# mcgillmrl/prob_mbrl

Measured on AMD Instinct MI355X. Metric: particle_rollouts_per_sec, higher is better.
Workload: dtype f32 via split fp16 (fwd, 2 pieces) / bf16 (adjoint, 2 pieces) MFMA, fp32 accumulate

## Files before the change

include/pmbrl.h:

```cpp
#ifndef PMBRL_H
#define PMBRL_H

#include <stddef.h>
#include <stdint.h>

#ifdef __cplusplus
extern "C" {
#endif

#define PMBRL_MAX_LAYERS 8
#define PMBRL_MAX_ANGLE 8
#define PMBRL_MAX_TIP 8
#define PMBRL_MAX_DIM 64

#define PMBRL_FLAG_MM_STATES 1
#define PMBRL_FLAG_MM_REWARDS 2
#define PMBRL_FLAG_INFER_NS 4
#define PMBRL_FLAG_FORCE_GENERIC 16
#define PMBRL_FLAG_NO_SHAPED 32
#define PMBRL_FLAG_POL_MASKS_PER_STEP 64
#define PMBRL_FLAG_DYN_MASKS_PER_STEP 128
#define PMBRL_FLAG_GMM_EXACT_NOISE_GRAD 256
#define PMBRL_MAX_COMP 8
#define PMBRL_FLAG_ZMM_PER_STEP 8
// ... 18 lines not shown

typedef struct pmbrl_reward {
  int32_t kind;
  int32_t expand;
  int32_t n_angle;
  int32_t angle_dims[PMBRL_MAX_ANGLE];
  int32_t k;
  float C[PMBRL_MAX_TIP * PMBRL_MAX_DIM];
  float tip_target[PMBRL_MAX_TIP];
  float norm;
  float w;
  float Q[PMBRL_MAX_TIP * PMBRL_MAX_TIP];
  float R[PMBRL_MAX_DIM * PMBRL_MAX_DIM];
} pmbrl_reward;

typedef struct pmbrl_config {
  int32_t B, D, U, H;
  int32_t B_global, row_offset;
  int32_t flags;
  int32_t mm_groups;
  float max_log_std_pol;
  float max_log_std_dyn;
  pmbrl_mlp pol;
  pmbrl_mlp dyn;
  pmbrl_reward reward;
  int32_t rows_per_wg_hint;
  int32_t precision;
  int32_t n_pol_angle;
  int32_t pol_angle_dims[PMBRL_MAX_ANGLE];
  int32_t n_dyn_angle;
  int32_t dyn_angle_dims[PMBRL_MAX_ANGLE];
  int32_t dyn_components;
  int32_t mm_span_rows, mm_span_offset;
  int32_t mm_span_ranks, mm_span_rank;
  int32_t pol_act, dyn_act;
} pmbrl_config;


typedef struct pmbrl_plan pmbrl_plan;

enum {
  PMBRL_INFO_ROWS_PER_WG = 0,
  PMBRL_INFO_N_WG = 1,
  PMBRL_INFO_ROW_TILES = 2,
  PMBRL_INFO_LDS_BYTES = 3,
  PMBRL_INFO_N_POL_PARAMS = 4,
  PMBRL_INFO_N_DYN_PARAMS = 5,
  PMBRL_INFO_DW_SPLITS = 6,
  PMBRL_INFO_MM_MODE = 7,
  PMBRL_INFO_LD = 8,
  PMBRL_INFO_DW_BLOCKS = 9,
  PMBRL_INFO_FAST = 10,
  PMBRL_INFO_STAGES = 11,
  PMBRL_INFO_MM_GRID = 12,
  PMBRL_INFO_PRECISION = 13,
  PMBRL_INFO_DW_PIPE = 14,
  PMBRL_INFO_MM_PARTS = 15,
  PMBRL_INFO_REG = 16,
  PMBRL_INFO_REPLAY = 17,
  PMBRL_INFO_INPLACE = 18,
  PMBRL_INFO_REG_FWD_CALLS = 19,
  PMBRL_INFO_REG_BWD_CALLS = 20,
  PMBRL_INFO_TAIL_CALLS = 21,
  PMBRL_INFO_COUNT = 22
};

const char* pmbrl_last_error(void);
int pmbrl_version(void);
const char* pmbrl_build_id(void);

typedef struct pmbrl_graph pmbrl_graph;
int pmbrl_graph_capture_begin(void* stream);
int pmbrl_graph_capture_end(void* stream, pmbrl_graph** graph_out);
int pmbrl_graph_launch(pmbrl_graph* graph, void* stream);
int pmbrl_graph_num_nodes(pmbrl_graph* graph, int64_t* n_out);
void pmbrl_graph_destroy(pmbrl_graph* graph);

int pmbrl_plan_create(const pmbrl_config* cfg, int device, pmbrl_plan** out);
void pmbrl_plan_destroy(pmbrl_plan* plan);
size_t pmbrl_plan_workspace_bytes(const pmbrl_plan* plan);
int pmbrl_plan_info(const pmbrl_plan* plan, int32_t* info );
#define PMBRL_SWEEP_REG 4
int pmbrl_plan_sweep_kernel(const pmbrl_plan* plan, int variant, int adjoint, const char** name);

int pmbrl_pack_mask(void* stream, const float* mask_d, int32_t B, int32_t h,
                    int32_t src_ld, uint16_t* bits_d);

int pmbrl_draw_masks(void* stream, int32_t kind, uint64_t seed, uint64_t offset, const float* param_d,
                     int32_t param_len, float temp, int32_t rows, int32_t h, const float* u_d, const float* v_d,
                     uint16_t* bits_d, int32_t aux_row0, int32_t aux_rows, float* u_out_d, float* hard_out_d,
                     float* probs_out_d);

typedef struct pmbrl_inputs {
  const float* x0_d;
  const float* pol_params_d;
  const float* dyn_params_d;
  const float* mx_d;
  const float* iSx_d;
  const float* my_d;
  const float* Sy_d;
  const float* pol_scale_d;
  const float* pol_bias_d;
  const uint16_t* pol_mask_bits_d[PMBRL_MAX_LAYERS];
  const uint16_t* dyn_mask_bits_d[PMBRL_MAX_LAYERS];
  const float* z_pol_d;
  const float* z_dyn_d;
  int64_t z_pol_step_stride;
  int64_t z_dyn_step_stride;
  const float* z_mm_d;
  const float* z_rr_d;
  const float* z_pi_d;
  const float* u_cat_d;
} pmbrl_inputs;

int pmbrl_rollout_fwd(pmbrl_plan* plan, void* stream, void* workspace_d,
                      const pmbrl_inputs* in, float* states_d, float* actions_d,
                      float* rewards_d, int32_t* status_d);

int pmbrl_rollout_bwd(pmbrl_plan* plan, void* stream, void* workspace_d,
                      const pmbrl_inputs* in, const float* states_d,
                      const float* actions_d, const float* rewards_d,
                      const float* grad_rewards_d, const float* grad_states_d,
                      const float* grad_actions_d, float* grad_pol_flat_d,
                      float* grad_x0_d, float* action_grad_norms_d, int32_t* status_d);

int pmbrl_weighted_sum(void* stream, const float* a_d, const float* w_d,
                       int64_t n, float* out_d);
int pmbrl_weighted_sum_steps(void* stream, const float* a_d, const float* w_d,
                             int64_t n_per_step, int32_t n_steps, const int32_t* status_d,
                             float* out_d);

int pmbrl_clip_adam(void* stream, float* params_d, float* grads_d,
                    float* exp_avg_d, float* exp_avg_sq_d, int64_t n,
                    int64_t step, double lr, double beta1, double beta2, double eps,
                    double max_norm, float* norm_out_d);

int pmbrl_clip_adam_guarded(void* stream, float* params_d, float* grads_d,
                            float* exp_avg_d, float* exp_avg_sq_d, int64_t n,
                            int64_t* step_d, double lr, double beta1, double beta2,
                            double eps, double max_norm, float* norm_out_d,
                            const int32_t* status_d, int32_t expect);

typedef struct pmbrl_adam {
  float* params_d;
  float* exp_avg_d;
  float* exp_avg_sq_d;
  int64_t* step_d;
  double lr, beta1, beta2, eps, max_norm;
  float* norm_out_d;
  int32_t expect_steps;
  float* loss_out_d;
} pmbrl_adam;
int pmbrl_plan_set_loss(pmbrl_plan* plan, const float* loss_weights_d, float* loss_out_d);
int pmbrl_rollout_bwd_adam(pmbrl_plan* plan, void* stream, void* workspace_d, const pmbrl_inputs* in,
                           const float* states_d, const float* actions_d, const float* rewards_d,
                           const float* grad_rewards_d, const float* grad_states_d, const float* grad_actions_d,
                           float* grad_pol_flat_d, float* grad_x0_d, float* action_grad_norms_d, int32_t* status_d,
                           const pmbrl_adam* opt);

#define PMBRL_COMM_ID_BYTES 128
typedef struct pmbrl_comm pmbrl_comm;
int pmbrl_comm_unique_id(void* id_out );
int pmbrl_comm_init(const void* id , int32_t rank, int32_t nranks,
                    int32_t device, pmbrl_comm** out);
int pmbrl_allreduce_sum(pmbrl_comm* comm, void* stream, float* buf_d, int64_t n);
int pmbrl_comm_count(pmbrl_comm* comm, int32_t* nranks_out);
// ... 114 lines not shown
```

prob_mbrl_amd/_lib.py:

```python
import ctypes as C
import os

_HERE = os.path.dirname(os.path.abspath(__file__))
LIB_PATH = os.environ.get('PMBRL_LIB_PATH', os.path.join(_HERE, 'csrc', 'libpmbrl_hip.so'))

MAX_LAYERS = 8
MAX_ANGLE = 8
MAX_TIP = 8
MAX_DIM = 64
FLAG_MM_STATES, FLAG_MM_REWARDS, FLAG_INFER_NS, FLAG_ZMM_PER_STEP = 1, 2, 4, 8
FLAG_FORCE_GENERIC = 16
FLAG_NO_SHAPED = 32
FLAG_POL_MASKS_PER_STEP, FLAG_DYN_MASKS_PER_STEP = 64, 128
FLAG_GMM_EXACT_NOISE_GRAD = 256
MAX_COMP = 8
REWARD_EXP, REWARD_NEG, REWARD_LEARNED = 0, 1, 2
PREC_F32, PREC_SPLIT, PREC_SPLIT_F16 = 0, 1, 2
ACT_RELU, ACT_TANH, ACT_SILU = 0, 1, 2
DROP_BY_TEMPERATURE, DROP_BERNOULLI = 0, 1
(INFO_ROWS_PER_WG, INFO_N_WG, INFO_ROW_TILES, INFO_LDS_BYTES, INFO_N_POL_PARAMS, INFO_N_DYN_PARAMS, INFO_DW_SPLITS,
 INFO_MM_MODE, INFO_LD, INFO_DW_BLOCKS, INFO_FAST, INFO_STAGES, INFO_MM_GRID, INFO_PRECISION, INFO_DW_PIPE, INFO_MM_PARTS,
 INFO_REG, INFO_REPLAY, INFO_INPLACE, INFO_REG_FWD_CALLS, INFO_REG_BWD_CALLS, INFO_TAIL_CALLS, INFO_COUNT) = range(23)
SWEEP_VARIANTS = ('lean', 'ext', 'mm', 'mmg', 'reg')
TIMER_COUNT = 8
TIMER_NAMES = ['pack', 'fwd', 'bwd', 'dw', 'dw_reduce', 'reward']


class MLP(C.Structure):
    _fields_ = [('n_layers', C.c_int32),
                ('dims', C.c_int32 * (MAX_LAYERS + 1)),
                ('keep', C.c_float * MAX_LAYERS)]


class MlpCall(C.Structure):
    _fields_ = [('B', C.c_int32), ('net', MLP), ('max_log_std', C.c_float), ('act', C.c_int32)]


class BnnConfig(C.Structure):
    _fields_ = [('M', C.c_int32), ('N', C.c_int32), ('net', MLP), ('max_log_std', C.c_float),
                ('temperature', C.c_float * MAX_LAYERS), ('reg_scale', C.c_float * MAX_LAYERS),
                ('drop_reg', C.c_float * MAX_LAYERS), ('reg_weight', C.c_float), ('loss_kind', C.c_int32),
                ('n_components', C.c_int32), ('act', C.c_int32),
                ('drop_kind', C.c_int32 * MAX_LAYERS), ('bern_keep', C.c_float * MAX_LAYERS)]


class Reward(C.Structure):
    _fields_ = [('kind', C.c_int32), ('expand', C.c_int32),
                ('n_angle', C.c_int32), ('angle_dims', C.c_int32 * MAX_ANGLE),
                ('k', C.c_int32), ('C', C.c_float * (MAX_TIP * MAX_DIM)),
                ('tip_target', C.c_float * MAX_TIP), ('norm', C.c_float),
                ('w', C.c_float), ('Q', C.c_float * (MAX_TIP * MAX_TIP)),
                ('R', C.c_float * (MAX_DIM * MAX_DIM))]


class Config(C.Structure):
    _fields_ = [('B', C.c_int32), ('D', C.c_int32), ('U', C.c_int32),
                ('H', C.c_int32), ('B_global', C.c_int32),
                ('row_offset', C.c_int32), ('flags', C.c_int32),
                ('mm_groups', C.c_int32), ('max_log_std_pol', C.c_float),
                ('max_log_std_dyn', C.c_float), ('pol', MLP), ('dyn', MLP),
                ('reward', Reward), ('rows_per_wg_hint', C.c_int32), ('precision', C.c_int32),
                ('n_pol_angle', C.c_int32), ('pol_angle_dims', C.c_int32 * MAX_ANGLE),
                ('n_dyn_angle', C.c_int32), ('dyn_angle_dims', C.c_int32 * MAX_ANGLE),
                ('dyn_components', C.c_int32),
                ('mm_span_rows', C.c_int32), ('mm_span_offset', C.c_int32),
                ('mm_span_ranks', C.c_int32), ('mm_span_rank', C.c_int32),
                ('pol_act', C.c_int32), ('dyn_act', C.c_int32)]


COLLECTIVE_FN = C.CFUNCTYPE(C.c_int, C.c_void_p, C.c_void_p, C.c_void_p, C.c_int64)


class Inputs(C.Structure):
    _fields_ = [('x0', C.c_void_p), ('pol_params', C.c_void_p),
                ('dyn_params', C.c_void_p), ('mx', C.c_void_p),
                ('iSx', C.c_void_p), ('my', C.c_void_p), ('Sy', C.c_void_p),
                ('pol_scale', C.c_void_p), ('pol_bias', C.c_void_p),
                ('pol_mask_bits', C.c_void_p * MAX_LAYERS),
                ('dyn_mask_bits', C.c_void_p * MAX_LAYERS),
                ('z_pol', C.c_void_p), ('z_dyn', C.c_void_p),
                ('z_pol_step_stride', C.c_int64), ('z_dyn_step_stride', C.c_int64),
                ('z_mm', C.c_void_p), ('z_rr', C.c_void_p),
                ('z_pi', C.c_void_p), ('u_cat', C.c_void_p)]


EXPORTS = [
    'pmbrl_last_error', 'pmbrl_version', 'pmbrl_build_id', 'pmbrl_plan_create',
    'pmbrl_graph_capture_begin', 'pmbrl_graph_capture_end', 'pmbrl_graph_launch', 'pmbrl_graph_num_nodes', 'pmbrl_graph_destroy',
    'pmbrl_plan_destroy', 'pmbrl_plan_workspace_bytes', 'pmbrl_plan_info', 'pmbrl_plan_sweep_kernel',
    'pmbrl_pack_mask', 'pmbrl_draw_masks', 'pmbrl_rollout_fwd', 'pmbrl_rollout_bwd', 'pmbrl_rollout_bwd_adam',
    'pmbrl_plan_set_loss',
    'pmbrl_weighted_sum', 'pmbrl_weighted_sum_steps', 'pmbrl_clip_adam', 'pmbrl_clip_adam_guarded', 'pmbrl_debug_linear',
    'pmbrl_plan_set_timing', 'pmbrl_plan_read_timing', 'pmbrl_plan_set_prof', 'pmbrl_plan_set_replay', 'pmbrl_plan_replay_count',
    'pmbrl_mlp_workspace_bytes', 'pmbrl_mlp_forward', 'pmbrl_mlp_grad_input',
    'pmbrl_bnn_plan_create', 'pmbrl_bnn_plan_destroy', 'pmbrl_bnn_plan_workspace_bytes',
    'pmbrl_bnn_plan_n_params', 'pmbrl_bnn_plan_set_unit_keep', 'pmbrl_bnn_loss_grad', 'pmbrl_bnn_loss_grad_ex', 'pmbrl_bnn_train_steps',
    'pmbrl_comm_unique_id', 'pmbrl_comm_init', 'pmbrl_allreduce_sum', 'pmbrl_comm_count', 'pmbrl_comm_destroy',
    'pmbrl_plan_set_comm', 'pmbrl_plan_set_collective',
    'pmbrl_p2p_create', 'pmbrl_p2p_handle', 'pmbrl_p2p_open', 'pmbrl_p2p_allreduce_f32', 'pmbrl_p2p_allreduce_f64',
    'pmbrl_plan_set_p2p', 'pmbrl_p2p_error', 'pmbrl_p2p_destroy', 'pmbrl_plan_set_grad_comm',
]

class Adam(C.Structure):
    _fields_ = [('params_d', C.c_void_p), ('exp_avg_d', C.c_void_p), ('exp_avg_sq_d', C.c_void_p),
                ('step_d', C.c_void_p), ('lr', C.c_double), ('beta1', C.c_double), ('beta2', C.c_double),
                ('eps', C.c_double), ('max_norm', C.c_double), ('norm_out_d', C.c_void_p), ('expect_steps', C.c_int32),
                ('loss_out_d', C.c_void_p)]


_lib = None


def load():
    global _lib
    if _lib is not None:
        return _lib
    if not os.path.exists(LIB_PATH):
        raise RuntimeError(
            'prob_mbrl_amd: %s is missing -- build the HIP extension first '
            '(python -c "import __graft_entry__ as g; g.build()"). There is no '
            'CPU fallback for the rollout hot path.' % LIB_PATH)
    lib = C.CDLL(LIB_PATH)
    vp, i32, i64, f32 = C.c_void_p, C.c_int32, C.c_int64, C.c_float
    lib.pmbrl_last_error.restype = C.c_char_p
    lib.pmbrl_last_error.argtypes = []
    lib.pmbrl_version.restype = C.c_int
    lib.pmbrl_build_id.restype = C.c_char_p
    lib.pmbrl_build_id.argtypes = []
    lib.pmbrl_graph_capture_begin.restype = C.c_int
    lib.pmbrl_graph_capture_begin.argtypes = [vp]
    lib.pmbrl_graph_capture_end.restype = C.c_int
    lib.pmbrl_graph_capture_end.argtypes = [vp, C.POINTER(vp)]
    lib.pmbrl_graph_launch.restype = C.c_int
    lib.pmbrl_graph_launch.argtypes = [vp, vp]
    lib.pmbrl_graph_num_nodes.restype = C.c_int
    lib.pmbrl_graph_num_nodes.argtypes = [vp, C.POINTER(C.c_int64)]
    lib.pmbrl_graph_destroy.restype = None
    lib.pmbrl_graph_destroy.argtypes = [vp]
    lib.pmbrl_plan_create.restype = C.c_int
    lib.pmbrl_plan_create.argtypes = [C.POINTER(Config), C.c_int, C.POINTER(vp)]
    lib.pmbrl_plan_destroy.restype = None
    lib.pmbrl_plan_destroy.argtypes = [vp]
    lib.pmbrl_plan_workspace_bytes.restype = C.c_size_t
    lib.pmbrl_plan_workspace_bytes.argtypes = [vp]
    lib.pmbrl_plan_info.restype = C.c_int
    lib.pmbrl_plan_info.argtypes = [vp, C.POINTER(i32)]
    lib.pmbrl_plan_sweep_kernel.restype = C.c_int
    lib.pmbrl_plan_sweep_kernel.argtypes = [vp, C.c_int, C.c_int, C.POINTER(C.c_char_p)]
    lib.pmbrl_pack_mask.restype = C.c_int
    lib.pmbrl_pack_mask.argtypes = [vp, vp, i32, i32, i32, vp]
    lib.pmbrl_rollout_fwd.restype = C.c_int
    lib.pmbrl_rollout_fwd.argtypes = [vp, vp, vp, C.POINTER(Inputs), vp, vp, vp, vp]
    lib.pmbrl_rollout_bwd.restype = C.c_int
    lib.pmbrl_rollout_bwd.argtypes = [vp, vp, vp, C.POINTER(Inputs), vp, vp, vp,
                                      vp, vp, vp, vp, vp, vp, vp]
    lib.pmbrl_weighted_sum.restype = C.c_int
    lib.pmbrl_weighted_sum.argtypes = [vp, vp, vp, i64, vp]
    lib.pmbrl_weighted_sum_steps.restype = C.c_int
    lib.pmbrl_weighted_sum_steps.argtypes = [vp, vp, vp, i64, i32, vp, vp]
    lib.pmbrl_clip_adam.restype = C.c_int
    f64 = C.c_double
    lib.pmbrl_clip_adam.argtypes = [vp, vp, vp, vp, vp, i64, i64, f64, f64, f64,
                                    f64, f64, vp]
    lib.pmbrl_clip_adam_guarded.restype = C.c_int
    lib.pmbrl_clip_adam_guarded.argtypes = [vp, vp, vp, vp, vp, i64, vp, f64, f64, f64, f64, f64, vp, vp, i32]
    lib.pmbrl_mlp_workspace_bytes.restype = C.c_size_t
    lib.pmbrl_mlp_workspace_bytes.argtypes = [C.POINTER(MlpCall)]
    lib.pmbrl_mlp_forward.restype = C.c_int
    lib.pmbrl_mlp_forward.argtypes = [vp, C.POINTER(MlpCall), vp, vp, vp, C.POINTER(vp)] + [vp] * 10
    lib.pmbrl_mlp_grad_input.restype = C.c_int
    lib.pmbrl_mlp_grad_input.argtypes = [vp, C.POINTER(MlpCall), vp, vp, vp, C.POINTER(vp)] + [vp] * 11
    lib.pmbrl_bnn_plan_create.restype = C.c_int
    lib.pmbrl_bnn_plan_create.argtypes = [C.POINTER(BnnConfig), C.c_int, C.POINTER(vp)]
    lib.pmbrl_bnn_plan_destroy.restype = None
    lib.pmbrl_bnn_plan_destroy.argtypes = [vp]
    lib.pmbrl_bnn_plan_workspace_bytes.restype = C.c_size_t
    lib.pmbrl_bnn_plan_workspace_bytes.argtypes = [vp]
    lib.pmbrl_bnn_plan_n_params.restype = C.c_int64
    lib.pmbrl_bnn_plan_n_params.argtypes = [vp]
    lib.pmbrl_bnn_plan_set_unit_keep.restype = C.c_int
    lib.pmbrl_bnn_plan_set_unit_keep.argtypes = [vp, i32, C.POINTER(f32), i32]
    lib.pmbrl_bnn_loss_grad.restype = C.c_int
    lib.pmbrl_bnn_loss_grad.argtypes = [vp] * 11
    lib.pmbrl_bnn_loss_grad_ex.restype = C.c_int
    lib.pmbrl_bnn_loss_grad_ex.argtypes = [vp] * 13 + [i32]
    lib.pmbrl_bnn_train_steps.restype = C.c_int
    lib.pmbrl_bnn_train_steps.argtypes = ([vp] * 6 + [i32] + [vp] * 4 + [C.c_double] * 4 + [C.c_uint64] * 2 + [vp] * 4)
    lib.pmbrl_debug_linear.restype = C.c_int
    lib.pmbrl_debug_linear.argtypes = [vp, vp, vp, vp, i32, i32, i32, i32, vp, vp]
    lib.pmbrl_plan_set_replay.restype = C.c_int
    lib.pmbrl_plan_set_replay.argtypes = [vp, C.c_int]
    lib.pmbrl_plan_replay_count.restype = C.c_int
    lib.pmbrl_plan_replay_count.argtypes = [vp, C.POINTER(C.c_int64)]
    lib.pmbrl_plan_set_timing.restype = C.c_int
    lib.pmbrl_plan_set_timing.argtypes = [vp, C.c_int]
    lib.pmbrl_plan_read_timing.restype = C.c_int
    lib.pmbrl_plan_read_timing.argtypes = [vp, C.POINTER(C.c_float)]
    lib.pmbrl_plan_set_prof.restype = C.c_int
    lib.pmbrl_plan_set_prof.argtypes = [vp, vp, vp]
    lib.pmbrl_comm_unique_id.restype = C.c_int
    lib.pmbrl_comm_unique_id.argtypes = [vp]
    lib.pmbrl_comm_init.restype = C.c_int
    lib.pmbrl_comm_init.argtypes = [vp, i32, i32, i32, C.POINTER(vp)]
    lib.pmbrl_allreduce_sum.restype = C.c_int
    lib.pmbrl_allreduce_sum.argtypes = [vp, vp, vp, i64]
    lib.pmbrl_plan_set_loss.restype = C.c_int
    lib.pmbrl_plan_set_loss.argtypes = [vp, vp, vp]
    lib.pmbrl_rollout_bwd_adam.restype = C.c_int
    lib.pmbrl_rollout_bwd_adam.argtypes = [vp, vp, vp, C.POINTER(Inputs)] + [vp] * 10 + [C.POINTER(Adam)]
    lib.pmbrl_draw_masks.restype = C.c_int
    lib.pmbrl_draw_masks.argtypes = [vp, i32, C.c_uint64, C.c_uint64, vp, i32, C.c_float, i32, i32, vp, vp, vp, i32, i32, vp, vp, vp]
    lib.pmbrl_comm_count.restype = C.c_int
    lib.pmbrl_comm_count.argtypes = [vp, C.POINTER(i32)]
    lib.pmbrl_comm_destroy.restype = None
    lib.pmbrl_comm_destroy.argtypes = [vp]
    lib.pmbrl_plan_set_comm.restype = C.c_int
    lib.pmbrl_plan_set_comm.argtypes = [vp, vp]
    lib.pmbrl_p2p_create.restype = C.c_int
    lib.pmbrl_p2p_create.argtypes = [i32, i32, i32, i64, C.POINTER(vp)]
    lib.pmbrl_p2p_handle.restype = C.c_int
    lib.pmbrl_p2p_handle.argtypes = [vp, vp]
    lib.pmbrl_p2p_open.restype = C.c_int
    lib.pmbrl_p2p_open.argtypes = [vp, i32, vp]
    for fn in (lib.pmbrl_p2p_allreduce_f32, lib.pmbrl_p2p_allreduce_f64):
        fn.restype = C.c_int
        fn.argtypes = [vp, vp, vp, i64]
    lib.pmbrl_plan_set_p2p.restype = C.c_int
    lib.pmbrl_plan_set_p2p.argtypes = [vp, vp]
    lib.pmbrl_p2p_error.restype = C.c_int
    lib.pmbrl_p2p_error.argtypes = [vp, C.POINTER(i32)]
    lib.pmbrl_p2p_destroy.restype = None
# ... 22 lines not shown
```

prob_mbrl_amd/csrc/pmbrl.hip:

```cpp
#include <hip/hip_runtime.h>
#include <math.h>
#include <stdio.h>
#include <string.h>

#include <algorithm>
#include <memory>
#include <string>
#include <vector>

#include "pmbrl_host.h"
#include "pmbrl_mm.h"
#include "pmbrl_rollout.h"
#include "pmbrl_mmx.h"
#include "pmbrl_mm_wide.h"
#include "pmbrl_fast.h"
#include "pmbrl_reward.h"

static thread_local std::string g_err;
int pm_fail(int code, const std::string& msg) {
  g_err = msg;
  return code;
}

extern "C" const char* pmbrl_last_error(void) { return g_err.c_str(); }
// ... 265 lines not shown
  const int gi = blockIdx.x, r0 = gi * A.M;
  if (A.nvalid && t >= *A.nvalid) return;
  const int zrow0 = pm_zrow0(t, A.row_off + r0, A.flags);
  const float* zmm = pm_zbase(A.zmm, A.D, t, A.Bg, A.flags);
  const float* s = A.xt + ((size_t)t * A.B + r0) * A.D;
  float* g = A.gx_carry + (size_t)r0 * A.D;
  const double* fac = fac_all + ((size_t)t * gridDim.x + gi) * pm_mmw_fac_doubles(A.D);
  pm_mmw_bwd(s, A.M, A.D, zmm, zrow0, A.Bg, g, g, fac, mmscr);
}

static size_t align_up(size_t x, size_t a) { return (x + a - 1) / a * a; }

static int net_plan(const pmbrl_mlp& m, int act, NetPlan& n, int in_expect, int out_expect,
                    const char* name) {
  if (m.n_layers < 1 || m.n_layers > PM_MAXL)
    return fail(-2, std::string(name) + ": n_layers out of range");
  n.nl = m.n_layers;
  size_t off = 0;
  for (int i = 0; i <= n.nl; ++i) {
    if (m.dims[i] < 1 || m.dims[i] > 4096) return fail(-2, std::string(name) + ": bad layer width");
    n.dim[i] = m.dims[i];
    n.nt[i] = (m.dims[i] + 15) / 16;
  }
  if (n.dim[0] != in_expect || n.dim[n.nl] != out_expect)
    return fail(-2, std::string(name) + ": input/output width does not match D/U");
  if (act != PMBRL_ACT_RELU && act != PMBRL_ACT_TANH && act != PMBRL_ACT_SILU)
    return fail(-2, std::string(name) + ": unknown activation (PMBRL_ACT_RELU, PMBRL_ACT_TANH, PMBRL_ACT_SILU are offered)");
  n.act = act;
  for (int l = 0; l < n.nl; ++l) {
    n.keep[l] = (l < n.nl - 1) ? m.keep[l] : 1.f;
    if (l < n.nl - 1 && !(n.keep[l] > 0.f)) return fail(-2, std::string(name) + ": keep must be > 0");
    n.w_off[l] = off;
    off += (size_t)n.dim[l + 1] * n.dim[l];
    n.b_off[l] = off;
    off += n.dim[l + 1];
  }
  n.n_params = off;
  return 0;
}

#define PM_INST(RT, CA, CB, VAR, D, U, LD, NL, NT, TREE) \
  {reinterpret_cast<const void*>(&pm_rollout_fwd<RT>), reinterpret_cast<const void*>(&pm_rollout_bwd<RT>)},
static const PmInst general_f32_fns[] = {PM_GENERAL_F32_INSTANCES};
#undef PM_INST
static_assert(sizeof(general_f32_fns) / sizeof(general_f32_fns[0]) == pm_general_f32_n, "one kernel pair per key");

static constexpr size_t PM_LDS_CAP = 160 * 1024;

static bool env_set(const char* name) { return getenv(name) != nullptr; }
static bool env_on(const char* name) {
  const char* e = getenv(name);
  return !(e && atoi(e) == 0);
}
static PlanSwitches read_switches() {
  PlanSwitches s{};
  s.mm_perstep = env_set("PMBRL_MM_PERSTEP");
  s.mm_mode2 = env_set("PMBRL_MM_MODE2");
  s.mm_no_batch = env_set("PMBRL_MM_NO_BATCH");
  s.dw_no_wide = env_set("PMBRL_DW_NO_WIDE");
  s.reg_debug = env_set("PMBRL_REG_DEBUG");
  s.lds_tiles = env_on("PMBRL_LDS_TILES");
  s.mm_xch = env_on("PMBRL_MM_XCH");
  s.mm_tree = env_on("PMBRL_MM_TREE");
  s.reg = env_on("PMBRL_REG");
  s.reg_mm = env_on("PMBRL_REG_MM");
  s.reg_tree = env_on("PMBRL_REG_TREE");
  s.reg_bwd = env_on("PMBRL_REG_BWD");
  s.fuse_loss = env_on("PMBRL_FUSE_LOSS");
  s.ztab_merge = env_on("PMBRL_ZTAB_MERGE");
  s.wide = env_on("PMBRL_WIDE");
  if (const char* e = getenv("PMBRL_MM_PARTS")) { s.mm_parts_set = true; s.mm_parts = atoi(e); }
  s.replay = 1;
  if (const char* e = getenv("PMBRL_REPLAY")) s.replay = std::max(0, std::min(2, atoi(e)));
  if (const char* e = getenv("PMBRL_DW_PIPE")) {
    s.dw_pipe_off = !strcmp(e, "off");
    s.dw_pipe_ranges = e[0] >= '0' && e[0] <= '9';
    for (const char* q = e; s.dw_pipe_ranges && *q;) {
      const int v = atoi(q);
      if (v > 0) s.dw_pipe.push_back(v);
      while (*q && *q != ',') ++q;
      if (*q == ',') ++q;
    }
  }
  return s;
}

static int plan_nets(pmbrl_plan* p) {
  const pmbrl_config& c = p->cfg;
  if (c.n_pol_angle < 0 || c.n_pol_angle > PMBRL_MAX_ANGLE || c.n_dyn_angle < 0 || c.n_dyn_angle > PMBRL_MAX_ANGLE)
    return fail(-2, "n_pol_angle / n_dyn_angle out of range");
  if (c.dyn_components < 0 || c.dyn_components > PMBRL_MAX_COMP)
    return fail(-2, "dyn_components out of range (<= PMBRL_MAX_COMP)");
  const bool gmm = c.dyn_components > 1;
  if (c.reward.kind != PMBRL_REWARD_EXP && c.reward.kind != PMBRL_REWARD_NEG && c.reward.kind != PMBRL_REWARD_LEARNED)
    return fail(-2, "unknown reward kind");
  p->learned = c.reward.kind == PMBRL_REWARD_LEARNED;
  if (p->learned && gmm)
    return fail(-2, "learned reward head: not offered with the mixture head (dyn_components > 1)");
  if (p->learned && c.mm_span_rows > 0)
    return fail(-2, "learned reward head: not offered with moment-matching groups spread over ranks (mm_span_rows > 0)");
  if (p->learned && c.D + 1 > PMBRL_MAX_DIM) return fail(-2, "learned reward head: D + 1 exceeds PMBRL_MAX_DIM");
  int rc = net_plan(c.pol, c.pol_act, p->pol, c.D + c.n_pol_angle, 2 * c.U, "policy");
  if (rc == 0)
    rc = net_plan(c.dyn, c.dyn_act, p->dyn, c.D + c.U + c.n_dyn_angle,
                  gmm ? (2 * c.D + 1) * c.dyn_components + 1 : 2 * (c.D + p->learned), "dynamics");
  p->act = rc == 0 && (p->pol.act != PMBRL_ACT_RELU || p->dyn.act != PMBRL_ACT_RELU);
  return rc;
}

struct LayoutCalc {
  const pmbrl_plan* p;
  int maxnt;
  bool gsplit;
  bool want_split;
  bool rt4_split;
  int ld_generic() const { return gsplit ? (maxnt * 16 + 31) / 32 * 32 + 16 : maxnt * 16 + 8; }
  int prec(int RT) const {
    if (!p->fast) return gsplit ? (int)PMBRL_PREC_SPLIT_F16 : 0;
    return (want_split && (RT <= 2 || rt4_split)) ? (int)p->cfg.precision : 0;
  }
  long stream_work(int m, int kdiv) const {
    long w = 0;
    for (const NetPlan* n : {&p->pol, &p->dyn})
      for (int l = 1; l <= n->nl - 2; ++l) {
        const int ki = (n->nt[l] + kdiv - 1) / kdiv, ko = (n->nt[l + 1] + kdiv - 1) / kdiv;
        w += (long)n->nt[l + 1] * ((ki + m - 1) / m * m) + (long)n->nt[l] * ((ko + m - 1) / m * m);
      }
    return w;
  }
  StagePair stages(int RT) const {
    const int pr = prec(RT);
    return pm_inst_best_stages(pm_fast_keys(pr), pr && !p->fast ? std::min(RT, 2) : RT,
                               [&](int m) { return stream_work(m, pr ? 2 : 1); });
  }
  int ldb(int RT) const {
    if (!prec(RT)) return 0;
    if (!p->fast) return ld_generic();
    const StagePair sp = stages(RT);
    const int m = sp.ca + sp.cb;
    return ((maxnt + 1) / 2 + m - 1) / m * m * 32 + 16;
  }
  int ld(int RT) const {
    if (!p->fast) return ld_generic();
    if (prec(RT))
      return ((prec(RT) == PMBRL_PREC_SPLIT_F16 ? 2 : 3) * ldb(RT) / 2 + 3) / 4 * 4;
    const StagePair sp = stages(RT);
    const int m = sp.ca + sp.cb;
    return (maxnt + m - 1) / m * m * 16 + 8;
  }
  size_t lds(int RT, int mmd, int parts = 1, bool inplace = false) const {
    const pmbrl_config& c = p->cfg;
    if (p->fast) {
      const int mw = parts > 1 ? 1 : (mmd && p->M <= 16 * RT) ? std::min(PF_NW, std::max(1, 16 * RT / p->M)) : PF_NW;
      return pm_fast_lds_floats(16 * RT, ld(RT), c.D, c.U, RT, p->pol.nt, p->pol.nl, p->dyn.nt, p->dyn.nl, mmd, prec(RT),
                                mw, parts > 1 ? (parts > 8 ? 16 : p->M) : 0, parts > 1 ? c.H : 0) * sizeof(float);
    }
    return pm_lds_floats(16 * RT, ld(RT), c.D, c.U, RT, mmd, inplace) * sizeof(float);
  }
};

static int plan_groups(pmbrl_plan* p, LayoutCalc& L, int cus) {
  const pmbrl_config& c = p->cfg;
  const PlanSwitches& sw = p->sw;
  p->G = c.mm_groups > 0 ? c.mm_groups : 1;
  if (c.B % p->G) return fail(-2, "B must be divisible by mm_groups");
  p->M = c.B / p->G;
// ... 319 lines not shown
      for (int l = 0; l < p->pol.nl; ++l) {
        if (p->dw_narrow[l]) { wide[l] = true; continue; }
        p->dw_pre_mask |= 1u << l;
        for (int m0 = 0; m0 < 512; m0 += PM_DWP_TM)
          for (int n0 = 0; n0 < 512; n0 += PM_DWP_TN) pre.push_back(DwUnit{(int16_t)l, (int16_t)m0, (int16_t)n0, 0});
      }
      units = pre;
    } else {
      for (int l = 0; l < PM_MAXL; ++l) p->dw_narrow[l] = 0;
    }
  }
  p->n_dw_units = (int)units.size();
  if (p->n_dw_units) {
    HIPCHK(hipMalloc(&p->dw_units_d, units.size() * sizeof(DwUnit)));
    HIPCHK(hipMemcpy(p->dw_units_d, units.data(), units.size() * sizeof(DwUnit), hipMemcpyHostToDevice));
  }
  if (int rc = pm_dw_set_attr(p)) return rc;
  p->n_dw_blocks = build_dw_blocks(p->pol.nl, p->pol.nt, blocks, p->dw_wave_first, p->dw_split ? PM_DW_TN_S : PM_DW_TN, wide);
  p->dw_n_chunks = c.H * p->nwg * p->RT;
  int nsplit = std::min(256, p->dw_n_chunks);
  p->dw_chunks_per_split = (p->dw_n_chunks + nsplit - 1) / nsplit;
  if (p->dw_split) p->dw_chunks_per_split = (p->dw_chunks_per_split + 1) & ~1;
  p->dw_nsplit = (p->dw_n_chunks + p->dw_chunks_per_split - 1) / p->dw_chunks_per_split;
  HIPCHK(hipMalloc(&p->dw_blocks_d, std::max<size_t>(1, blocks.size()) * sizeof(DwBlock)));
  if (!blocks.empty())
    HIPCHK(hipMemcpy(p->dw_blocks_d, blocks.data(), blocks.size() * sizeof(DwBlock), hipMemcpyHostToDevice));
  DwArgs& W = p->dw_args;
  memset(&W, 0, sizeof(W));
  W.nl = p->pol.nl;
  W.nsplit = p->dw_nsplit;
  W.n_chunks = p->dw_n_chunks;
  W.chunks_per_split = p->dw_chunks_per_split;
  W.RT = p->RT;
  W.Rw = 16 * p->RT;
  W.n_params = (int)p->pol.n_params;
  W.part_stride = (W.n_params + 3) / 4 * 4;
  for (int i = 0; i <= p->pol.nl; ++i) { W.dim[i] = p->pol.dim[i]; W.nt[i] = p->pol.nt[i]; }
  for (int l = 0; l < p->pol.nl; ++l) { W.w_off[l] = (int)p->pol.w_off[l]; W.b_off[l] = (int)p->pol.b_off[l]; }
  W.blocks = p->dw_blocks_d;
  for (int w = 0; w <= PM_DW_NW; ++w) W.wave_first[w] = p->dw_wave_first[w];
  W.chunks_per_step = p->nwg * p->RT;
  W.split_prec = p->dw_split;
  return 0;
}

static int plan_dw_pipe(pmbrl_plan* p, int cus) {
  const pmbrl_config& c = p->cfg;
  const PlanSwitches& sw = p->sw;
  p->pipe_K = 1;
  const bool no_pipe_pre = p->dw_pre_mask != 0;
  const int n_free = cus >= 64 && cus % 8 == 0 ? 8 * (cus / 8 - (p->nwg + 7) / 8) : 0;
  const bool single = sweep_form(p) == SweepForm::Whole && p->mm_parts <= 1;
  const bool long_steps = (long long)p->RT * (long long)(p->pol.n_params + p->dyn.n_params) >= 256 * 1024 && c.H >= 16;
  if (!single || no_pipe_pre || n_free < cus / 8 || c.H < 2 || sw.dw_pipe_off || !(long_steps || sw.dw_pipe_ranges))
    return 0;
  std::vector<int> cnt;
  if (sw.dw_pipe_ranges) {
    cnt = sw.dw_pipe;
    int sum = 0;
    for (int v : cnt) sum += v;
    if (sum != c.H || (int)cnt.size() > PM_PIPE_MAX) cnt.clear();
  }
  if (cnt.empty() && long_steps) {
    const int a3 = std::max(2, c.H / 10), a2 = a3 + std::max(2, c.H / 5), a1 = a2 + std::max(2, (3 * c.H) / 10);
    cnt = {c.H - a1, a1 - a2, a2 - a3, a3};
  }
  int K = 0, lo = c.H;
  for (size_t k = 0; k < cnt.size() && lo > 0; ++k) {
    lo = k + 1 == cnt.size() ? 0 : std::max(0, lo - cnt[k]);
    if (p->dw_split && ((p->nwg * p->RT) & 1) && (lo & 1)) lo -= 1;
    if (K > 0 && lo >= p->pipe_lo[K - 1]) continue;
    p->pipe_lo[K++] = lo;
  }
  if (K >= 2 && p->pipe_lo[K - 1] == 0) {
    p->pipe_K = K;
    p->pipe_grid = n_free;
    p->pipe_rows = std::max(n_free, cus);
    HIPCHK(hipStreamCreateWithFlags(&p->pipe_stream, hipStreamNonBlocking));
    for (int k = 0; k < p->pipe_K; ++k) HIPCHK(hipEventCreateWithFlags(&p->pipe_ev[k], hipEventDisableTiming));
  }
  return 0;
}

static int plan_workspace(pmbrl_plan* p) {
  const pmbrl_config& c = p->cfg;
  p->reg = pm_reg_plan_ok(p) ? 1 : 0;
  p->reg_mm = pm_reg_mm_width(p);
  size_t off = 0;
  auto take = [&](size_t bytes) {
    const size_t o = off;
    off = align_up(off + bytes, 256);
    return o;
  };
  for (NetPlan* n : {&p->pol, &p->dyn}) {
    for (int l = 0; l < n->nl; ++l) {
      const size_t fr = (size_t)(n->nt[l + 1] + 15) * (n->nt[l] + 15) * 256 * sizeof(float);
      n->wf[l] = take(fr);
      n->wb[l] = take(fr);
      n->bias[l] = take((size_t)n->nt[l + 1] * 16 * sizeof(float));
      if (l < n->nl - 1)
        n->abits[l] = take((size_t)c.H * c.B * n->nt[l + 1] * (p->act ? 16 * sizeof(float) : 4) + 256);
    }
  }
  const bool gmm = c.dyn_components > 1;
  const size_t Rw = 16 * p->RT;
  for (int l = 0; l < p->pol.nl; ++l) {
    p->off_actT[l] = take((size_t)c.H * p->nwg * p->pol.nt[l] * 16 * Rw * sizeof(float));
    p->off_gT[l] = take((size_t)c.H * p->nwg * p->pol.nt[l + 1] * 16 * Rw * sizeof(float));
  }
  p->off_Tp = take((size_t)c.H * c.B * c.U * sizeof(float));
  p->off_Td = take((size_t)c.H * c.B * c.D * sizeof(float));
  p->off_gmm_c = take(gmm ? (size_t)c.H * c.B * (c.dyn_components + 1) * c.D * sizeof(float) : 0);
  p->off_gmm_k = take(gmm ? (size_t)c.H * c.B * sizeof(int) : 0);
  p->off_xt = take((size_t)c.H * c.B * c.D * sizeof(float));
  p->off_rt = take((size_t)c.H * c.B * sizeof(float));
  p->off_mmfac = take(p->mm_mode == 1 ? (size_t)c.H * (c.B / p->M) * pm_mm_fac_doubles(c.D) * sizeof(double)
                      : p->mm_wide    ? (size_t)c.H * p->G * pm_mmw_fac_doubles(c.D) * sizeof(double)
                                      : 0);
  p->off_Jx = take((size_t)c.H * c.B * c.D * sizeof(float));
  p->off_Ja = take((size_t)c.H * c.B * c.U * sizeof(float));
  p->off_gxc = take((size_t)c.B * c.D * sizeof(float));
  p->off_gxc2 = take((size_t)c.B * c.D * sizeof(float));
  p->off_gsync = take(2 * 1024 * sizeof(unsigned));
  if (p->mm_parts > 1 && p->sw.mm_xch) {
    p->xch_bytes = (size_t)(p->mm_parts > 8 ? 2 : 1) * p->nwg * PM_XCH_WG_WORDS(2) * sizeof(unsigned long long);
    p->off_xch = take(p->xch_bytes);
  }
  p->off_ztab = take((p->mm_fan || p->reg_mm) ? (size_t)c.H * p->G * 2 * c.D * sizeof(double) : 0);
  p->off_reg_linv = take(p->reg_mm ? (size_t)c.H * p->G * c.D * c.D * sizeof(double) : 0);
  p->off_grt = take((size_t)c.H * c.B * sizeof(float));
  const size_t n_s = (size_t)p->G * pm_mmx_slot_doubles(c.D), n_r = (size_t)c.H * p->G * pm_mmx_slot_doubles(1);
  p->off_mmx_buf = take(p->span ? (size_t)c.mm_span_ranks * std::max(n_s * PM_MMX_NB, n_r) * sizeof(double) : 0);
  p->off_mmx_fac = take(p->span ? (size_t)c.H * p->G * pm_mm_fac_doubles(c.D) * sizeof(double) : 0);
  p->off_mmx_rfac = take(p->span ? (size_t)c.H * p->G * pm_mm_fac_doubles(1) * sizeof(double) : 0);
  p->off_reg_pack = take(p->reg ? pm_reg_pack_bytes() : 0);
  for (int n = 0; n < 2; ++n)
    for (int l = 0; l < 2; ++l) p->off_reg_ab[n][l] = take(p->reg ? (size_t)c.H * p->nwg * 1024 : 0);
  p->off_part = take((size_t)std::max(p->dw_nsplit, p->pipe_K > 1 ? p->pipe_rows : 0) *
                     ((p->pol.n_params + 3) / 4 * 4) * sizeof(float));
  p->ws_bytes = off;
  if (p->ws_bytes >= ((size_t)1 << 32)) p->reg = p->reg_mm = 0;
  return 0;
}

static PmInstTable sweep_table(const pmbrl_plan* p) {
  if (p->fast)
    return p->prec == PMBRL_PREC_SPLIT_F16 ? pm_fast_split2_instances() : p->prec ? pm_fast_split1_instances() : pm_fast_f32_instances();
  if (p->act) return pm_general_act_instances();
  return p->prec ? pm_general_split_instances() : PmInstTable{pm_general_f32_keys, general_f32_fns, pm_general_f32_n};
}
static bool lds_tiles_row(const pmbrl_plan* p, const PmInstKey& k) {
  return p->prec == PMBRL_PREC_SPLIT_F16 && p->RT == 1 && p->CA + p->CB == 7 && k.var != PF_VAR_MMG && k.nl == 3 && k.nt > 8;
}
static int resolve_sweeps(pmbrl_plan* p) {
  const pmbrl_config& c = p->cfg;
  const PmInstTable T = sweep_table(p);
  auto take = [&](int slot, const PmInstKey& k) {
    const int i = pm_inst_find(T, k);
    if (i >= 0) { p->sweep[slot] = T.fn[i]; p->sweep_key[slot] = k; }
    return i >= 0;
  };
  if (!p->fast) {
    const int wide_form = (p->inplace == 2 && p->dw_pre_mask) ? 3 : p->inplace;
    const PmInstKey k = pm_general_key(p->RT, p->act ? (p->prec ? 2 : 0) : p->prec ? wide_form : 0);
    return take(0, k) ? 0 : fail(-3, "no general-family instance for " + pm_inst_name(k));
  }
  const bool shaped_ok = !(c.flags & PMBRL_FLAG_NO_SHAPED) && !(p->mm_parts > 1 && !p->xch_bytes);
  for (int var = 0; var < PF_VAR_COUNT; ++var) {
    const bool mm_in = p->mm_mode == 1 || p->mm_mode == 3;
    const bool needed = var == PF_VAR_MMG ? p->mm_grid != 0 : (var == PF_VAR_MM) == mm_in;
    PmInstKey k = {p->RT, p->CA, p->CB, var, c.D, c.U, p->LD, 3, hidden_tiles_3l(p), 0};
    k.tree = var == PF_VAR_MM && p->mm_mode == 1 && p->mm_parts > 8;
    if (shaped_ok && (!lds_tiles_row(p, k) || p->wlds_off > 0) && take(var, k)) continue;
    if (k.tree) return fail(-3, "no instance for a moment-matching group split over more than 8 workgroups: " + pm_inst_name(k));
    k = PmInstKey{p->RT, p->CA, p->CB, var, 0, 0, 0, 0, 0, 0};
    if (!take(var, k) && needed) return fail(-3, "no latency-optimised instance for " + pm_inst_name(k));
  }
  return 0;
}
static int plan_attrs(pmbrl_plan* p, int cus) {
  const pmbrl_config& c = p->cfg;
  if (int rc = resolve_sweeps(p)) return rc;
  const PmInstTable T = sweep_table(p);
  for (int i = 0; i < T.n; ++i) {
    const PmInstKey& k = T.key[i];
    if (p->fast ? k.rt != p->RT || k.ca != p->CA || k.cb != p->CB : T.fn[i].fwd != p->sweep[0].fwd) continue;
    HIPCHK(hipFuncSetAttribute(T.fn[i].fwd, hipFuncAttributeMaxDynamicSharedMemorySize, (int)p->lds_bytes));
    HIPCHK(hipFuncSetAttribute(T.fn[i].bwd, hipFuncAttributeMaxDynamicSharedMemorySize, (int)p->lds_bytes));
  }
  if (p->mm_wide) {
    const int smem = (int)pm_mmw_lds_bytes(p->M, c.D, true);
    if (smem > 64 * 1024 &&
        (hipFuncSetAttribute(reinterpret_cast<const void*>(&pm_mmw_fwd_kernel), hipFuncAttributeMaxDynamicSharedMemorySize,
                             smem) != hipSuccess ||
         hipFuncSetAttribute(reinterpret_cast<const void*>(&pm_mmw_bwd_kernel), hipFuncAttributeMaxDynamicSharedMemorySize,
                             smem) != hipSuccess)) {
      (void)hipGetLastError();
      return fail(-3, "hipFuncSetAttribute(wide moment-matching kernels) failed");
    }
  }
  if (p->mm_mode == 2 || p->mm_mode == 3) {
    const int smem = (int)(pm_mm_kernel_doubles(c.D) * sizeof(double));
    if (smem > (int)PM_LDS_CAP) return fail(-3, "moment-matching scratch exceeds the LDS");
    if (smem > 64 * 1024 &&
        (hipFuncSetAttribute(reinterpret_cast<const void*>(&pm_mm_fwd_kernel), hipFuncAttributeMaxDynamicSharedMemorySize,
                             smem) != hipSuccess ||
         hipFuncSetAttribute(reinterpret_cast<const void*>(&pm_mm_bwd_kernel), hipFuncAttributeMaxDynamicSharedMemorySize,
                             smem) != hipSuccess)) {
      (void)hipGetLastError();
      return fail(-3, "hipFuncSetAttribute(moment-matching kernels) failed");
    }
  }
  if (p->reg)
    if (int rc = pm_reg_resolve(p)) return rc;
  if (p->mm_grid) {
    const int i = pm_inst_find(T, {1, p->CA, p->CB, PF_VAR_MMG, 0, 0, 0, 0, 0, 0});
    int a = 0, b = 0;
    if (i < 0 || hipOccupancyMaxActiveBlocksPerMultiprocessor(&a, T.fn[i].fwd, PF_NT, p->lds_bytes) != hipSuccess ||
        hipOccupancyMaxActiveBlocksPerMultiprocessor(&b, T.fn[i].bwd, PF_NT, p->lds_bytes) != hipSuccess)
      a = b = 0;
    if (std::min(a, b) < 1 || p->nwg > cus) p->mm_grid = 0;
  }
  return 0;
}

extern "C" int pmbrl_plan_create(const pmbrl_config* cfg, int device, pmbrl_plan** out) {
  if (!cfg || !out) return fail(-1, "null argument");
  const pmbrl_config& c = *cfg;
  if (c.B < 1 || c.D < 1 || c.U < 1 || c.H < 1) return fail(-2, "B, D, U, H must be >= 1");
  if (c.D > 32 || c.U > 16) return fail(-2, "supported widths: D <= 32, U <= 16");
  if (c.reward.kind != PMBRL_REWARD_LEARNED && (c.reward.k < 1 || c.reward.k > PMBRL_MAX_TIP))
    return fail(-2, "reward.k out of range");
  std::unique_ptr<pmbrl_plan, void (*)(pmbrl_plan*)> p(new pmbrl_plan(), pmbrl_plan_destroy);
  p->cfg = c;
  if (p->cfg.B_global <= 0) p->cfg.B_global = c.B;
  p->device = device;
  p->sw = read_switches();
  p->replay = p->sw.replay;
  if (int rc = plan_nets(p.get())) return rc;
  int cus = 0;
  (void)hipDeviceGetAttribute(&cus, hipDeviceAttributeMultiprocessorCount, device);
  if (int rc = plan_layout(p.get(), cus)) return rc;
  if (int rc = plan_reward(p.get())) return rc;
  if (int rc = plan_angles(p.get())) return rc;
  if (int rc = plan_dw(p.get())) return rc;
  if (int rc = plan_dw_pipe(p.get(), cus)) return rc;
  if (int rc = plan_workspace(p.get())) return rc;
  if (int rc = plan_attrs(p.get(), cus)) return rc;
  *out = p.release();
  return 0;
}

static bool per_step_launches(const pmbrl_plan* p) {
  const SweepForm f = sweep_form(p);
  return (f == SweepForm::StepExternal || f == SweepForm::StepInSweep) && p->cfg.H >= 4;
}
static bool replay_wanted(const pmbrl_plan* p) {
  if (p->replay == 0 || p->span || p->coll) return false;
  return p->replay >= 2 || per_step_launches(p);
}
struct ReplayKey {
  unsigned long long h = 1469598103934665603ull;
  std::vector<unsigned char> bytes;
  void add(const void* q, size_t n) {
    const unsigned char* b = static_cast<const unsigned char*>(q);
    for (size_t i = 0; i < n; ++i) { h ^= b[i]; h *= 1099511628211ull; }
    bytes.insert(bytes.end(), b, b + n);
  }
  template <class T> void val(const T& v) { add(&v, sizeof(T)); }
};
static bool pm_stream_recording(hipStream_t s) {
  hipStreamCaptureStatus cs = hipStreamCaptureStatusNone;
  if (!s) return false;
  if (hipStreamIsCapturing(s, &cs) != hipSuccess) { (void)hipGetLastError(); return false; }
  return cs != hipStreamCaptureStatusNone;
}
template <class Body>
static int replay_call(pmbrl_plan* p, int slot, const ReplayKey& K, hipStream_t s, Body body) {
  const unsigned long long key = K.h;
  pmbrl_plan::ReplaySlot& R = p->rp[slot];
  hipStreamCaptureStatus cs = hipStreamCaptureStatusNone;
  const bool usable = replay_wanted(p) && !p->timing && !p->prof_fwd && !p->prof_bwd && !R.dead &&
                      (!s || (hipStreamIsCapturing(s, &cs) == hipSuccess && cs == hipStreamCaptureStatusNone));
  if (!usable) {
    if (R.exec || R.seen) replay_drop(p, slot);
    return body(s);
  }
  const bool same = R.key == key && R.bytes == K.bytes;
  if (R.exec && same) {
    HIPCHK(hipGraphLaunch(R.exec, s));
    ++R.launches;
    if (slot == 0) { p->old_pack_stale = R.aux & 1; p->abits_packed = (R.aux >> 1) & 1; }
    else p->dw_g1_rebuilt = (R.aux >> 2) & 1;
    return 0;
  }
  if (!same || R.seen == 0) {
    replay_drop(p, slot);
    R.key = key;
    R.bytes = K.bytes;
    R.seen = 1;
    return body(s);
  }
  hipGraph_t g = nullptr;
  if (!p->cap_stream && hipStreamCreateWithFlags(&p->cap_stream, hipStreamNonBlocking) != hipSuccess) p->cap_stream = nullptr;
  if (!p->cap_stream || hipStreamBeginCapture(p->cap_stream, hipStreamCaptureModeThreadLocal) != hipSuccess) {
    (void)hipGetLastError();
    R.dead = 1;
    return body(s);
  }
  const int rc = body(p->cap_stream);
  const hipError_t e = hipStreamEndCapture(p->cap_stream, &g);
  if (rc != 0 || e != hipSuccess || !g) {
    (void)hipGetLastError();
    if (g) (void)hipGraphDestroy(g);
    R.dead = 1;
    replay_drop(p, slot);
    return rc != 0 ? rc : body(s);
  }
  hipGraphExec_t ex = nullptr;
  const hipError_t ei = hipGraphInstantiate(&ex, g, nullptr, nullptr, 0);
  (void)hipGraphDestroy(g);
  if (ei != hipSuccess || !ex) {
    (void)hipGetLastError();
    R.dead = 1;
    replay_drop(p, slot);
    return body(s);
  }
  R.exec = ex;
  R.aux = (p->old_pack_stale & 1) | ((p->abits_packed & 1) << 1) | ((p->dw_g1_rebuilt & 1) << 2);
  HIPCHK(hipGraphLaunch(R.exec, s));
  ++R.launches;
  return 0;
}

extern "C" int pmbrl_plan_set_replay(pmbrl_plan* p, int on) {
  if (!p || on < 0 || on > 2) return fail(-1, "bad argument");
  p->replay = on;
  for (int k = 0; k < 2; ++k) { replay_drop(p, k); p->rp[k].dead = 0; }
  return 0;
}

extern "C" int pmbrl_plan_replay_count(const pmbrl_plan* p, int64_t* n_out) {
  if (!p || !n_out) return fail(-1, "null argument");
  for (int k = 0; k < 2; ++k) n_out[k] = p->rp[k].launches;
  return 0;
}

extern "C" int pmbrl_plan_set_prof(pmbrl_plan* p, long long* fwd_d, long long* bwd_d) {
  if (!p) return fail(-1, "null argument");
  p->prof_fwd = fwd_d;
  p->prof_bwd = bwd_d;
  return 0;
}

extern "C" int pmbrl_plan_set_timing(pmbrl_plan* p, int on) {
  if (!p) return fail(-1, "null argument");
  if (on && !p->ev[0][0]) {
    for (int i = 0; i < PMBRL_TIMER_COUNT; ++i)
      for (int j = 0; j < 2; ++j) HIPCHK(hipEventCreate(&p->ev[i][j]));
  }
  p->timing = on ? 1 : 0;
  for (int i = 0; i < PMBRL_TIMER_COUNT; ++i) p->ev_set[i] = false;
  return 0;
}

extern "C" int pmbrl_plan_read_timing(pmbrl_plan* p, float* ms) {
  if (!p || !ms) return fail(-1, "null argument");
  for (int i = 0; i < PMBRL_TIMER_COUNT; ++i) {
    ms[i] = -1.f;
    if (p->timing && p->ev_set[i]) {
      HIPCHK(hipEventSynchronize(p->ev[i][1]));
      HIPCHK(hipEventElapsedTime(&ms[i], p->ev[i][0], p->ev[i][1]));
    }
  }
  return 0;
}

extern "C" void pmbrl_plan_destroy(pmbrl_plan* p) {
  if (!p) return;
  if (p->ev[0][0])
    for (int i = 0; i < PMBRL_TIMER_COUNT; ++i)
      for (int j = 0; j < 2; ++j) (void)hipEventDestroy(p->ev[i][j]);
  for (int k = 0; k < 2; ++k) replay_drop(p, k);
  if (p->cap_stream) (void)hipStreamDestroy(p->cap_stream);
  if (p->rew_d) (void)hipFree(p->rew_d);
  if (p->wflag_d) (void)hipFree(p->wflag_d);
  if (p->ang_d) (void)hipFree(p->ang_d);
  if (p->dw_blocks_d) (void)hipFree(p->dw_blocks_d);
  if (p->dw_units_d) (void)hipFree(p->dw_units_d);
  if (p->tail_buf_d) (void)hipFree(p->tail_buf_d);
  if (p->pipe_stream) {
    (void)hipStreamDestroy(p->pipe_stream);
    for (int k = 0; k < p->pipe_K; ++k) (void)hipEventDestroy(p->pipe_ev[k]);
  }
  delete p;
}

extern "C" int pmbrl_plan_sweep_kernel(const pmbrl_plan* p, int variant, int adjoint, const char** name) {
  if (!p || !name) return fail(-1, "null argument");
  PmInst k{};
  if (variant == PMBRL_SWEEP_REG) k = p->reg ? p->reg_k[0] : k;
  else if (!p->fast) k = p->sweep[0];
  else if (variant >= 0 && variant < PF_VAR_COUNT) k = p->sweep[variant];
  else return fail(-1, "variant out of range");
  const void* f = adjoint ? k.bwd : k.fwd;
  *name = f ? hipKernelNameRefByPtr(f, nullptr) : "";
  if (!*name) *name = "";
  return 0;
}

extern "C" size_t pmbrl_plan_workspace_bytes(const pmbrl_plan* p) { return p ? p->ws_bytes : 0; }

extern "C" int pmbrl_plan_info(const pmbrl_plan* p, int32_t* info) {
  if (!p || !info) return fail(-1, "null argument");
  memset(info, 0, sizeof(int32_t) * PMBRL_INFO_COUNT);
  info[PMBRL_INFO_ROWS_PER_WG] = p->rows_per_wg;
  info[PMBRL_INFO_N_WG] = p->nwg;
  info[PMBRL_INFO_ROW_TILES] = p->RT;
  info[PMBRL_INFO_LDS_BYTES] = (int32_t)p->lds_bytes;
  info[PMBRL_INFO_N_POL_PARAMS] = (int32_t)p->pol.n_params;
  info[PMBRL_INFO_N_DYN_PARAMS] = (int32_t)p->dyn.n_params;
  info[PMBRL_INFO_DW_SPLITS] = p->dw_nsplit;
  info[PMBRL_INFO_MM_MODE] = p->mm_mode;
  info[PMBRL_INFO_LD] = p->LD;
  info[PMBRL_INFO_DW_BLOCKS] = p->n_dw_blocks;
  info[PMBRL_INFO_FAST] = p->fast;
  info[PMBRL_INFO_STAGES] = p->CA * 16 + p->CB;
  info[PMBRL_INFO_MM_GRID] = p->mm_grid;
  info[PMBRL_INFO_PRECISION] = p->prec;
  info[PMBRL_INFO_DW_PIPE] = p->pipe_K;
  info[PMBRL_INFO_MM_PARTS] = p->mm_parts;
  info[PMBRL_INFO_REG] = p->reg;
  info[PMBRL_INFO_REPLAY] = replay_wanted(p) ? 1 : 0;
  info[PMBRL_INFO_INPLACE] = p->inplace;
  info[PMBRL_INFO_REG_FWD_CALLS] = p->reg_calls[0];
  info[PMBRL_INFO_REG_BWD_CALLS] = p->reg_calls[1];
  info[PMBRL_INFO_TAIL_CALLS] = p->tail_calls;
  return 0;
}


static void fill_net(const NetPlan& n, char* ws, const uint16_t* const* masks, NetDev& d) {
  d.nl = n.nl;
  for (int i = 0; i <= n.nl; ++i) {
    d.dim[i] = n.dim[i];
    d.nt[i] = n.nt[i];
  }
  for (int l = 0; l < n.nl; ++l) {
    d.keep[l] = n.keep[l];
    d.inv_keep[l] = 1.f / n.keep[l];
    d.wf[l] = reinterpret_cast<const float*>(ws + n.wf[l]);
    d.wb[l] = reinterpret_cast<const float*>(ws + n.wb[l]);
    d.bias[l] = reinterpret_cast<const float*>(ws + n.bias[l]);
    d.mask[l] = (l < n.nl - 1) ? masks[l] : nullptr;
    d.abits[l] = (l < n.nl - 1) ? reinterpret_cast<uint16_t*>(ws + n.abits[l]) : nullptr;
  }
}

static int fill_args(const pmbrl_plan* p, void* workspace, const pmbrl_inputs* in, RolloutArgs& A) {
  const pmbrl_config& c = p->cfg;
  char* ws = static_cast<char*>(workspace);
  memset(&A, 0, sizeof(A));
  A.B = c.B; A.D = c.D; A.U = c.U; A.H = c.H;
  A.Bg = c.B_global; A.row_off = c.row_offset; A.flags = c.flags;
  A.flags |= (p->pol.act << PM_ACT_POL_SHIFT) | (p->dyn.act << PM_ACT_DYN_SHIFT);
  A.G = p->G; A.M = p->M; A.mm_mode = p->mm_mode;
  A.t0 = 0; A.t1 = c.H;
  A.rows_per_wg = p->rows_per_wg; A.nwg = p->nwg; A.Rw = 16 * p->RT; A.LD = p->LD; A.LDB = p->LDB;
  A.mls_pol = c.max_log_std_pol; A.mls_dyn = c.max_log_std_dyn;
  for (int l = 0; l < p->pol.nl - 1; ++l)
    if (!in->pol_mask_bits_d[l]) return fail(-1, "missing policy mask bits");
  for (int l = 0; l < p->dyn.nl - 1; ++l)
    if (!in->dyn_mask_bits_d[l]) return fail(-1, "missing dynamics mask bits");
  fill_net(p->pol, ws, in->pol_mask_bits_d, A.pol);
  fill_net(p->dyn, ws, in->dyn_mask_bits_d, A.dyn);
  A.rew = p->rew_d;
  A.ang = p->ang_d;
  A.x0 = in->x0_d; A.mx = in->mx_d; A.iSx = in->iSx_d; A.my = in->my_d; A.Sy = in->Sy_d;
  A.pscale = in->pol_scale_d; A.pbias = in->pol_bias_d;
  A.zpol = in->z_pol_d; A.zdyn = in->z_dyn_d; A.zmm = in->z_mm_d; A.zrr = in->z_rr_d;
  A.zpol_ss = in->z_pol_step_stride; A.zdyn_ss = in->z_dyn_step_stride;
  if (!A.x0 || !A.mx || !A.iSx || !A.my || !A.Sy || !A.pscale || !A.pbias || !A.zpol || !A.zdyn)
    return fail(-1, "null input pointer");
  if ((c.flags & PMBRL_FLAG_MM_STATES) && !A.zmm) return fail(-1, "mm_states needs z_mm");
  if ((c.flags & PMBRL_FLAG_MM_REWARDS) && !A.zrr) return fail(-1, "mm_rewards needs z_rr");
  for (int l = 0; l < p->pol.nl; ++l) {
    A.actT[l] = reinterpret_cast<float*>(ws + p->off_actT[l]);
    A.gT[l] = reinterpret_cast<float*>(ws + p->off_gT[l]);
  }
  A.Tp = reinterpret_cast<float*>(ws + p->off_Tp);
  A.Td = reinterpret_cast<float*>(ws + p->off_Td);
  A.gmm_n = p->cfg.dyn_components > 1 ? p->cfg.dyn_components : 0;
  A.zpi = A.ucat = A.zdyn_grad = nullptr;
  A.gmm_k = nullptr;
// ... 381 lines not shown
  if (!p || (loss_weights_d && !loss_out_d)) return fail(-1, "bad argument");
  p->loss_w = loss_weights_d;
  p->loss_out = loss_weights_d ? loss_out_d : nullptr;
  return 0;
}

static int tail_allreduce(pmbrl_plan* p, hipStream_t s, float* buf_d, int64_t n) {
  if (p->grad_p2p) return pmbrl_p2p_allreduce_f32(p->grad_p2p, s, buf_d, n);
  return pmbrl_allreduce_sum(p->grad_comm, s, buf_d, n);
}

struct BwdCall {
  hipStream_t stream;
  void* workspace;
  const pmbrl_inputs* in;
  const float *states, *actions, *rewards;
  const float *grad_rewards, *grad_states, *grad_actions;
  float *grad_pol_flat, *grad_x0, *action_grad_norms;
  int32_t* status;
  const pmbrl_adam* opt;
};
static bool bwd_tail(const pmbrl_plan* p, const BwdCall& C) { return C.opt && (p->grad_comm || p->grad_p2p); }
static int expect_steps(const pmbrl_plan* p, const pmbrl_adam* opt) {
  return opt ? (opt->expect_steps > 0 ? opt->expect_steps : p->cfg.H) : 0;
}

static int check_bwd(const pmbrl_plan* p, const BwdCall& C, bool reg_bwd) {
  if (bwd_tail(p, C) && p->span && p->cfg.mm_span_ranks > 1)
    return fail(-3, "pmbrl_rollout_bwd_adam with a gradient transport: moment-matching groups spread over ranks are not offered");
  if (p->reg && p->old_pack_stale && !reg_bwd && (!C.in->pol_params_d || !C.in->dyn_params_d)) return fail(-1, "null parameter pointer");
  if (int rc = check_collective(p)) return rc;
  const SweepForm form = sweep_form(p);
  if (C.grad_states && (form == SweepForm::Barrier || form == SweepForm::StepInSweep))
    return fail(-3, "grad_states with moment-matching groups spanning workgroups: not offered");
  if (C.grad_states && form == SweepForm::StepExternal) return fail(-3, "grad_states with external moment matching: not offered");
  return 0;
}

static int bwd_args(const pmbrl_plan* p, const BwdCall& C, RolloutArgs& A) {
  if (int rc = fill_args(p, C.workspace, C.in, A)) return rc;
  A.states = const_cast<float*>(C.states);
  A.actions = const_cast<float*>(C.actions);
  A.rewards = const_cast<float*>(C.rewards);
  A.grad_rewards = C.grad_rewards;
  A.grad_states = C.grad_states;
  A.grad_actions = C.grad_actions;
  A.grad_x0 = C.grad_x0;
  A.agn = C.action_grad_norms;
  A.prof = p->prof_bwd;
  A.nvalid = C.status;
  A.status = C.status ? C.status + 1 : nullptr;
  if (!p->fast) A.ext_reward = 1;
  return 0;
}

static int bwd_agree_horizon(pmbrl_plan* p, const BwdCall& C) {
  hipStream_t s = C.stream;
  float* hvec = p->tail_buf_d + ((size_t)p->pol.n_params + 2 + 3) / 4 * 4;
  pm_tail_hvec_launch(s, hvec, p->tail_world, p->tail_rank, C.status, p->cfg.H);
  if (int rc = tail_allreduce(p, s, hvec, p->tail_world)) return rc;
  pm_tail_hmin_launch(s, hvec, p->tail_world, C.status, p->cfg.H);
  return 0;
}

static void bwd_convert_family(pmbrl_plan* p, const BwdCall& C) {
  char* ws = static_cast<char*>(C.workspace);
  if (p->old_pack_stale) launch_pack_all(p, ws, C.in, C.stream, nullptr);
  if (p->abits_packed) pm_reg_unpack_abits(p, ws, C.stream);
}

static int bwd_reward_adjoint(pmbrl_plan* p, const BwdCall& C, RolloutArgs& A, float* grt) {
  if (p->cfg.flags & PMBRL_FLAG_MM_REWARDS) {
    if (p->span) {
      if (int rc = mmx_bwd(p, static_cast<char*>(C.workspace), A, true, 0, grt, C.stream)) return rc;
    } else {
      hipLaunchKernelGGL(pm_mm_rewards_bwd_kernel, dim3(p->cfg.H * p->G), dim3(64), pm_mmr_lds_bytes(p->M, 3), C.stream, A, grt);
    }
    A.grad_rewards = grt;
  }
  if (!p->fast) A.flags &= ~PMBRL_FLAG_MM_REWARDS;
  return 0;
}

static DwArgs dw_call_args(const pmbrl_plan* p, const BwdCall& C, const RolloutArgs& A) {
  DwArgs W = p->dw_args;
  for (int l = 0; l < p->pol.nl; ++l) { W.actT[l] = A.actT[l]; W.gT[l] = A.gT[l]; }
  W.part = reinterpret_cast<float*>(static_cast<char*>(C.workspace) + p->off_part);
  W.nvalid = C.status;
  if (p->dw_g1_rebuilt) {
    pm_reg_dw_rebuild_args(p, static_cast<char*>(C.workspace), W);
    W.rc_inv_keep = A.pol.inv_keep[1];
  }
  return W;
}
static int bwd_sweep_barrier(pmbrl_plan* p, const BwdCall& C, RolloutArgs A) {
  hipStream_t s = C.stream;
  HIPCHK(hipMemsetAsync(A.gx_carry, 0, (size_t)p->cfg.B * p->cfg.D * sizeof(float), s));
  A.gx_from_carry = 1;
  A.gsync += 1024;
  HIPCHK(hipMemsetAsync(A.gsync, 0, 1024 * sizeof(unsigned), s));
  A.gx_carry_out = reinterpret_cast<float*>(static_cast<char*>(C.workspace) + p->off_gxc2);
  A.t0 = 0; A.t1 = p->cfg.H;
  launch_bwd_rt(p, A, s);
  return 0;
}
static int bwd_sweep_steps(pmbrl_plan* p, const BwdCall& C, RolloutArgs A) {
  hipStream_t s = C.stream;
  float* cbuf[2] = {A.gx_carry, reinterpret_cast<float*>(static_cast<char*>(C.workspace) + p->off_gxc2)};
  HIPCHK(hipMemsetAsync(cbuf[0], 0, (size_t)p->cfg.B * p->cfg.D * sizeof(float), s));
  A.gx_from_carry = 1;
  for (int t = p->cfg.H - 1, k = 0; t >= 0; --t, k ^= 1) {
    A.gx_carry = cbuf[k];
    A.gx_carry_out = cbuf[k ^ 1];
    A.t0 = t; A.t1 = t + 1;
    launch_bwd_rt(p, A, s);
  }
  return 0;
}
static int bwd_sweep_whole(pmbrl_plan* p, const BwdCall& C, RolloutArgs A, const DwArgs& W, bool reg_bwd, int K, const int* lo) {
  hipStream_t s = C.stream;
  char* ws = static_cast<char*>(C.workspace);
  if (p->mm_parts > 1) {
    A.gsync += 1024;
    A.gx_carry_out = reinterpret_cast<float*>(ws + p->off_gxc2);
    if (int rc = xch_prepare(p, A, reg_bwd, s)) return rc;
  }
  for (int k = 0; k < K; ++k) {
    A.t0 = lo[k];
    A.t1 = k ? lo[k - 1] : p->cfg.H;
    A.gx_from_carry = k > 0;
    if (reg_bwd) pm_reg_launch(p, ws, A, C.in->pol_params_d, C.in->dyn_params_d, s, false);
    else launch_bwd_rt(p, A, s);
    if (k + 1 < K) {
      HIPCHK(hipEventRecord(p->pipe_ev[k], s));
      HIPCHK(hipStreamWaitEvent(p->pipe_stream, p->pipe_ev[k], 0));
      pm_dw_launch_range(p, W, k, p->pipe_stream);
    }
  }
  return 0;
}
static int bwd_sweep_external(pmbrl_plan* p, const BwdCall& C, RolloutArgs A, float* grt) {
  hipStream_t s = C.stream;
  char* ws = static_cast<char*>(C.workspace);
  const size_t smem = pm_mm_kernel_doubles(p->cfg.D) * sizeof(double);
  HIPCHK(hipMemsetAsync(A.gx_carry, 0, (size_t)p->cfg.B * p->cfg.D * sizeof(float), s));
  RolloutArgs Am = A;
  Am.flags &= ~PMBRL_FLAG_MM_REWARDS;
  A.gx_from_carry = 1;
  for (int t = p->cfg.H - 1; t >= 0; --t) {
    if (p->mm_wide) {
      hipLaunchKernelGGL(pm_mmw_bwd_kernel, dim3(p->G), dim3(PM_MMW_NT), pm_mmw_lds_bytes(p->M, p->cfg.D, true), s, Am, t,
                         reinterpret_cast<const double*>(ws + p->off_mmfac));
    } else if (!p->span) {
      hipLaunchKernelGGL(pm_mm_bwd_kernel, dim3(p->G), dim3(PM_MM_NW * 64), smem, s, Am, t, grt);
    } else if (p->cfg.flags & PMBRL_FLAG_MM_STATES) {
      if (int rc = mmx_bwd(p, ws, Am, false, t, nullptr, s)) return rc;
    }
    A.t0 = t; A.t1 = t + 1;
    launch_bwd_rt(p, A, s);
  }
  return 0;
}

static int bwd_dw(pmbrl_plan* p, const BwdCall& C, const DwArgs& W, bool piped) {
  ScopedTimer tm(p, PMBRL_TIMER_DW, C.stream);
  if (!piped) {
    pm_dw_launch(p, W, C.stream);
    return 0;
  }
  HIPCHK(hipEventRecord(p->pipe_ev[p->pipe_K - 1], p->pipe_stream));
  HIPCHK(hipStreamWaitEvent(C.stream, p->pipe_ev[p->pipe_K - 1], 0));
  pm_dw_launch_range(p, W, p->pipe_K - 1, C.stream);
  return 0;
}

static int rollout_bwd(pmbrl_plan* p, const BwdCall& C, const RolloutArgs& A0, bool reg_bwd) {
  hipStream_t s = C.stream;
  RolloutArgs A = A0;
  if (int rc = check_bwd(p, C, reg_bwd)) return rc;
  p->dw_g1_rebuilt = reg_bwd ? 1 : 0;
  const pmbrl_adam* opt = C.opt;
  const bool tail = bwd_tail(p, C);
  float* const xb = p->tail_buf_d;
  if (tail)
    if (int rc = bwd_agree_horizon(p, C)) return rc;
  if (p->reg && !reg_bwd) bwd_convert_family(p, C);
  float* grt = reinterpret_cast<float*>(static_cast<char*>(C.workspace) + p->off_grt);
  if (int rc = bwd_reward_adjoint(p, C, A, grt)) return rc;
  const DwArgs W = dw_call_args(p, C, A);
  const SweepForm form = sweep_form(p);
  const bool piped = form == SweepForm::Whole && p->pipe_K > 1 && !p->prof_bwd;
  {
    ScopedTimer tm(p, PMBRL_TIMER_BWD, s);
    static const int whole[1] = {0};
    int rc = 0;
    switch (form) {
      case SweepForm::Barrier: rc = bwd_sweep_barrier(p, C, A); break;
      case SweepForm::StepInSweep: rc = bwd_sweep_steps(p, C, A); break;
      case SweepForm::Whole: rc = bwd_sweep_whole(p, C, A, W, reg_bwd, piped ? p->pipe_K : 1, piped ? p->pipe_lo : whole); break;
      case SweepForm::StepExternal: rc = bwd_sweep_external(p, C, A, grt); break;
    }
    if (rc) return rc;
  }
  if (int rc = bwd_dw(p, C, W, piped)) return rc;
  const int n = (int)p->pol.n_params;
  const int expect = expect_steps(p, opt);
  const bool part_ok = opt && !piped && (n + 255) / 256 <= PM_NORM_MAXB;
  const bool norm_fused = part_ok && !tail;
  const bool loss_fused = part_ok && opt->loss_out_d && p->sw.fuse_loss;
  const int n_loss_part = loss_fused ? (n + 255) / 256 : 0;
  float* const red_out = tail ? xb : C.grad_pol_flat;
  {
    ScopedTimer tm(p, PMBRL_TIMER_DW_REDUCE, s);
    if (piped)
      pm_dw_reduce_launch(s, W.part, p->pipe_rows, n, W.part_stride, red_out, (const int*)nullptr, 0, 1);
    else
      pm_dw_reduce_launch(s, W.part, p->dw_nsplit, n, W.part_stride, red_out, (const int*)C.status, W.chunks_per_step,
                          W.chunks_per_split, norm_fused ? 1 : 0, (const int*)C.status, expect,
                          opt ? reinterpret_cast<long long*>(opt->step_d) : (long long*)nullptr,
                          loss_fused ? C.rewards : (const float*)nullptr, C.grad_rewards, (long long)p->cfg.H * p->cfg.B,
                          (long long)p->cfg.B);
  }
  if (opt && opt->loss_out_d && !loss_fused)
    launch_weighted_sum(s, C.rewards, C.grad_rewards, (long long)p->cfg.H * p->cfg.B, tail ? xb + n : opt->loss_out_d, C.status,
                        p->cfg.B);
  HIPCHK(hipGetLastError());
  if (!opt) return 0;
  if (tail) {
    pm_tail_pack_launch(s, xb, n, n_loss_part, opt->loss_out_d && !loss_fused ? 1 : 0, C.status, p->tail_err_d);
    if (int rc = tail_allreduce(p, s, xb, (int64_t)n + 2)) return rc;
    pm_tail_finish_launch(s, xb, C.grad_pol_flat, n, C.status, expect, reinterpret_cast<long long*>(opt->step_d), p->tail_err_d);
    HIPCHK(hipGetLastError());
  }
  return clip_adam_guarded_impl(s, opt->params_d, C.grad_pol_flat, opt->exp_avg_d, opt->exp_avg_sq_d, n, opt->step_d, opt->lr,
                                opt->beta1, opt->beta2, opt->eps, opt->max_norm, opt->norm_out_d, C.status, expect,
                                tail || norm_fused, tail || loss_fused ? opt->loss_out_d : nullptr,
                                tail ? (opt->loss_out_d ? 1 : 0) : n_loss_part);
}

static ReplayKey bwd_key(const pmbrl_plan* p, const BwdCall& C, bool reg_bwd) {
  const pmbrl_adam* opt = C.opt;
  ReplayKey K;
  K.val(C.stream); K.val(C.workspace); K.add(C.in, sizeof(*C.in));
  K.val(C.states); K.val(C.actions); K.val(C.rewards); K.val(C.grad_rewards); K.val(C.grad_states); K.val(C.grad_actions);
  K.val(C.grad_pol_flat); K.val(C.grad_x0); K.val(C.action_grad_norms); K.val(C.status);
  const int has_opt = opt ? 1 : 0;
  K.val(has_opt);
  if (opt) {
    K.val(opt->params_d); K.val(opt->exp_avg_d); K.val(opt->exp_avg_sq_d); K.val(opt->step_d);
    K.val(opt->lr); K.val(opt->beta1); K.val(opt->beta2); K.val(opt->eps); K.val(opt->max_norm);
    K.val(opt->norm_out_d); K.val(opt->expect_steps);
  }
  if (bwd_tail(p, C)) {
    K.val(p->grad_comm); K.val(p->tail_buf_d); K.val(opt->loss_out_d);
  }
  K.val(p->old_pack_stale); K.val(p->abits_packed);
  const int g1_rebuilt = reg_bwd ? 1 : 0;
  K.val(g1_rebuilt);
  return K;
}

static int rollout_bwd_replay(pmbrl_plan* p, const BwdCall& C) {
  if (!p || !C.workspace || !C.in || !C.states || !C.actions || !C.rewards || !C.grad_rewards || !C.grad_pol_flat)
    return fail(-1, "null argument");
  HIPCHK(hipSetDevice(p->device));
  RolloutArgs A;
  if (int rc = bwd_args(p, C, A)) return rc;
  const bool reg_bwd = pm_reg_can_run(p, A, false);
  const bool tail = bwd_tail(p, C);
  if (tail) ++p->tail_calls;
  if (tail && p->grad_p2p) {
    if (p->rp[1].exec || p->rp[1].seen) replay_drop(p, 1);
    return rollout_bwd(p, C, A, reg_bwd);
  }
  return replay_call(p, 1, bwd_key(p, C, reg_bwd), C.stream, [&](hipStream_t on) {
    BwdCall Con = C;
    Con.stream = on;
    return rollout_bwd(p, Con, A, reg_bwd);
  });
}

extern "C" int pmbrl_rollout_bwd(pmbrl_plan* p, void* stream, void* workspace, const pmbrl_inputs* in,
                                 const float* states_d, const float* actions_d,
                                 const float* rewards_d, const float* grad_rewards_d,
                                 const float* grad_states_d, const float* grad_actions_d,
                                 float* grad_pol_flat_d, float* grad_x0_d,
                                 float* action_grad_norms_d, int32_t* status_d) {
  return rollout_bwd_replay(p, BwdCall{(hipStream_t)stream, workspace, in, states_d, actions_d, rewards_d, grad_rewards_d,
                                       grad_states_d, grad_actions_d, grad_pol_flat_d, grad_x0_d, action_grad_norms_d,
                                       status_d, nullptr});
}

extern "C" int pmbrl_rollout_bwd_adam(pmbrl_plan* p, void* stream, void* workspace, const pmbrl_inputs* in,
                                      const float* states_d, const float* actions_d,
                                      const float* rewards_d, const float* grad_rewards_d,
                                      const float* grad_states_d, const float* grad_actions_d,
                                      float* grad_pol_flat_d, float* grad_x0_d,
                                      float* action_grad_norms_d, int32_t* status_d, const pmbrl_adam* opt) {
  if (!opt || !status_d || !opt->params_d || !opt->exp_avg_d || !opt->exp_avg_sq_d || !opt->step_d)
    return fail(-1, "null argument");
  return rollout_bwd_replay(p, BwdCall{(hipStream_t)stream, workspace, in, states_d, actions_d, rewards_d, grad_rewards_d,
                                       grad_states_d, grad_actions_d, grad_pol_flat_d, grad_x0_d, action_grad_norms_d,
                                       status_d, opt});
}

template <int RT>
__global__ __launch_bounds__(PM_NT, 1) void pm_debug_linear_kernel(const float* x, const float* wf,
                                                                  const float* bias, int R, int K,
                                                                  int O, int LD, int narrow,
                                                                  float* y) {
  extern __shared__ __attribute__((aligned(16))) float smem[];
  const int tid = threadIdx.x, lane = tid & 63, wid = tid >> 6;
  constexpr int RR = 16 * RT;
  float* X = smem;
  float* Y = X + RR * LD;
  float* part = pm_part_alias_ok(RR, LD, RT) ? nullptr : Y + RR * LD;
  const int n_kb = (K + 15) / 16, n_ot = (O + 15) / 16;
  for (int i = tid; i < RR * LD; i += PM_NT) {
    const int r = i / LD, k = i - r * LD;
    X[i] = (r < R && k < K) ? x[(size_t)r * K + k] : 0.f;
  }
  __syncthreads();
  if (narrow) {
    gemm_narrow<RT>(wf, n_ot, n_kb, bias, X, Y, LD, part, wid, lane, tid);
  } else {
    EpiPlain e{bias, Y, LD, lane};
    gemm_tiles<RT>(wf, n_ot, n_kb, X, LD, wid, lane, e);
    __syncthreads();
  }
  for (int i = tid; i < R * O; i += PM_NT) {
    const int r = i / O, o = i - r * O;
    y[i] = Y[r * LD + o];
  }
}

extern "C" int pmbrl_debug_linear(void* stream, const float* x_d, const float* W_d, const float* b_d,
                                  int32_t R, int32_t K, int32_t O, int32_t transpose_w, float* y_d,
                                  float* scratch_d) {
  if (R < 1 || R > 64 || K < 1 || O < 1) return fail(-1, "bad argument");
  hipStream_t s = (hipStream_t)stream;
  const int n_kb = (K + 15) / 16, n_ot = (O + 15) / 16;
// ... 39 lines not shown
```

prob_mbrl_amd/csrc/pmbrl_dw.h:

```cpp
#pragma once
#include "pmbrl_dev.h"

#define PM_DW_NW 8
#define PM_DW_NT (PM_DW_NW * 64)
#define PM_DW_TM 4
#define PM_DW_TN 7
#define PM_DW_MAXBLK 256
#define PM_DW_TN_S 4

struct DwBlock {
  int16_t layer, ot0, it0, n_ot, n_it, pad;
};
struct DwUnit {
  int16_t layer, m0, n0, pad;
};
#define PM_DWW_TM 128
#define PM_DWW_TN 128
#define PM_DWW_LDK 40
#define PM_DWW_STAGE ((PM_DWW_TM + PM_DWW_TN) * 2 * PM_DWW_LDK)
#define PM_DWW_LDS_BYTES (2 * PM_DWW_STAGE * 2)

struct DwArgs {
  int nl, nsplit, n_chunks, chunks_per_split;
  int RT, Rw, n_params;
  int part_stride;
  int dim[PM_MAXL + 1], nt[PM_MAXL + 1];
  int w_off[PM_MAXL], b_off[PM_MAXL];
  const float* actT[PM_MAXL];
  const float* gT[PM_MAXL];
  const int* nvalid;
  int chunks_per_step;
  const DwBlock* blocks;
  int wave_first[PM_DW_NW + 1];
  float* part;
  int split_prec;
  int pipe;
  int pipe_k;
  int c_begin, c_end;
  int rows_before;
  const unsigned* rc_abits;
  const float* rc_head;
  float rc_inv_keep;
  int rc_D, rc_U;
};

#define PM_DWP_TM 256
#define PM_DWP_TN 256
#define PM_DWL_NT 13
```

prob_mbrl_amd/csrc/pmbrl_dw.hip:

```cpp
#include <hip/hip_runtime.h>

#include <algorithm>
#include <cassert>
#include <vector>

#include "pmbrl_host.h"
#include "pmbrl_dw_kernels.h"

int build_dw_blocks(int nl, const int* nt, std::vector<DwBlock>& blocks, int* wave_first, int tn_max,
                           const bool* skip) {
  blocks.clear();
  auto split = [](int n, int maxsz, std::vector<std::pair<int, int>>& out) {
    const int parts = (n + maxsz - 1) / maxsz;
    int lo = 0;
    for (int i = 0; i < parts; ++i) {
      const int sz = n / parts + (i < n % parts ? 1 : 0);
      out.push_back({lo, sz});
      lo += sz;
    }
  };
  for (int l = 0; l < nl; ++l) {
    if (skip && skip[l]) continue;
    std::vector<std::pair<int, int>> os, is;
    split(nt[l + 1], PM_DW_TM, os);
    split(nt[l], tn_max, is);
    for (auto& o : os)
      for (auto& i : is) {
        DwBlock b;
        b.layer = (int16_t)l;
        b.ot0 = (int16_t)o.first;
        b.n_ot = (int16_t)o.second;
        b.it0 = (int16_t)i.first;
        b.n_it = (int16_t)i.second;
        b.pad = 0;
        blocks.push_back(b);
      }
  }
  const int n_blocks = (int)blocks.size();
  auto cost = [tn_max](const DwBlock& b) {
    const int ni = b.n_ot <= 1 ? 1 : (b.n_ot <= 3 ? 3 : 4);
    const int nj = b.n_it <= 1 ? 1 : (b.n_it <= 4 ? 4 : (b.n_it <= 6 ? 6 : 7));
    return ni * (tn_max <= 4 && nj > 1 ? 4 : nj);
  };
  std::stable_sort(blocks.begin(), blocks.end(),
                   [&](const DwBlock& a, const DwBlock& b) { return cost(a) > cost(b); });
  std::vector<DwBlock> per_wave[PM_DW_NW];
  long wave_load[PM_DW_NW] = {0};
  for (const DwBlock& b : blocks) {
    int best_simd = 0;
    for (int sm = 1; sm < 4; ++sm)
      if (wave_load[sm] + wave_load[sm + 4] < wave_load[best_simd] + wave_load[best_simd + 4]) best_simd = sm;
    const int w = wave_load[best_simd] <= wave_load[best_simd + 4] ? best_simd : best_simd + 4;
    per_wave[w].push_back(b);
    wave_load[w] += cost(b);
  }
  blocks.clear();
  for (int w = 0; w < PM_DW_NW; ++w) {
    wave_first[w] = (int)blocks.size();
    if (w >= 4) std::reverse(per_wave[w].begin(), per_wave[w].end());
    for (const DwBlock& b : per_wave[w]) blocks.push_back(b);
  }
  wave_first[PM_DW_NW] = (int)blocks.size();
  return n_blocks;
}

int pm_dw_set_attr(const pmbrl_plan* p) {
  if (p->dw_layer13 >= 0) {
    HIPCHK(hipFuncSetAttribute(reinterpret_cast<const void*>(&pm_dw_layer_kernel),
                               hipFuncAttributeMaxDynamicSharedMemorySize, PM_DWL_LDS_BYTES));
    HIPCHK(hipFuncSetAttribute(reinterpret_cast<const void*>(&pm_dw_layer_rc_kernel),
                               hipFuncAttributeMaxDynamicSharedMemorySize, PM_DWL_LDS_BYTES));
  }
  if (p->dw_pre_mask) {
    HIPCHK(hipFuncSetAttribute(reinterpret_cast<const void*>(&pm_dw_narrow_pre_kernel<1>),
                               hipFuncAttributeMaxDynamicSharedMemorySize, PM_DWP_LDS_BYTES));
    HIPCHK(hipFuncSetAttribute(reinterpret_cast<const void*>(&pm_dw_narrow_pre_kernel<2>),
                               hipFuncAttributeMaxDynamicSharedMemorySize, PM_DWP_LDS_BYTES));
  }
  if (p->n_dw_units) {
    HIPCHK(hipFuncSetAttribute(reinterpret_cast<const void*>(&pm_dw_wide_kernel),
                               hipFuncAttributeMaxDynamicSharedMemorySize, PM_DWW_LDS_BYTES));
    if (p->dw_pre_mask)
      HIPCHK(hipFuncSetAttribute(reinterpret_cast<const void*>(&pm_dw_wide_pre_kernel),
                                 hipFuncAttributeMaxDynamicSharedMemorySize, PM_DWP_LDS_BYTES));
  }
  return 0;
}

static DwArgs dw_range_args(const pmbrl_plan* p, const DwArgs& W, int k) {
  DwArgs Wk = W;
  const int cps = W.chunks_per_step;
  Wk.pipe = 1;
  Wk.pipe_k = k;
  Wk.nsplit = k + 1 == p->pipe_K ? p->pipe_rows : p->pipe_grid;
  Wk.rows_before = p->pipe_grid;
  Wk.c_begin = p->pipe_lo[k] * cps;
  Wk.c_end = (k ? p->pipe_lo[k - 1] : p->cfg.H) * cps;
  Wk.chunks_per_split = (Wk.c_end - Wk.c_begin + Wk.nsplit - 1) / Wk.nsplit;
  if (p->dw_split) Wk.chunks_per_split = (Wk.chunks_per_split + 1) & ~1;
  return Wk;
}
void pm_dw_launch(const pmbrl_plan* p, const DwArgs& W, hipStream_t s) {
  const dim3 rows(W.nsplit), units((W.nsplit + 7) / 8 * 8 * p->n_dw_units);
  if (p->n_dw_blocks == 0) {}
  else if (p->dw_split) hipLaunchKernelGGL(pm_dw_kernel_s, rows, dim3(PM_DW_NT), 0, s, W);
  else hipLaunchKernelGGL(pm_dw_kernel, rows, dim3(PM_DW_NT), 0, s, W);
  if (p->dw_pre_mask)
    for (int l = 0; l < p->pol.nl; ++l) {
      if (!p->dw_narrow[l]) continue;
      const int g_wide = p->dw_narrow[l] == 1 ? 1 : 0, nt_n = g_wide ? p->pol.nt[l] : p->pol.nt[l + 1];
      if (nt_n <= 1) hipLaunchKernelGGL(pm_dw_narrow_pre_kernel<1>, rows, dim3(PM_DWP_NT), PM_DWP_LDS_BYTES, s, W, l, g_wide);
      else hipLaunchKernelGGL(pm_dw_narrow_pre_kernel<2>, rows, dim3(PM_DWP_NT), PM_DWP_LDS_BYTES, s, W, l, g_wide);
    }
  if (p->n_dw_units && p->dw_pre_mask)
    hipLaunchKernelGGL(pm_dw_wide_pre_kernel, units, dim3(PM_DWP_NT), PM_DWP_LDS_BYTES, s, W, p->dw_units_d, p->n_dw_units);
  else if (p->n_dw_units)
    hipLaunchKernelGGL(pm_dw_wide_kernel, units, dim3(PM_DW_NT), PM_DWW_LDS_BYTES, s, W, p->dw_units_d, p->n_dw_units);
  const bool rebuild = W.rc_abits != nullptr;
  assert(!rebuild || (W.RT == 1 && p->dw_layer13 == PM_REG_DW_LAYER));
  if (p->dw_layer13 >= 0 && rebuild)
    hipLaunchKernelGGL(pm_dw_layer_rc_kernel, rows, dim3(PM_DW_NT), PM_DWL_LDS_BYTES, s, W, p->dw_layer13);
  else if (p->dw_layer13 >= 0)
    hipLaunchKernelGGL(pm_dw_layer_kernel, rows, dim3(PM_DW_NT), PM_DWL_LDS_BYTES, s, W, p->dw_layer13);
}
void pm_dw_launch_range(const pmbrl_plan* p, const DwArgs& W, int k, hipStream_t s) { pm_dw_launch(p, dw_range_args(p, W, k), s); }
void pm_dw_blocks_launch(const DwArgs& W, hipStream_t s) {
  hipLaunchKernelGGL(pm_dw_kernel, dim3(W.nsplit), dim3(PM_DW_NT), 0, s, W);
}
```

prob_mbrl_amd/csrc/pmbrl_dw_kernels.h:

```cpp
#pragma once
#include "pmbrl_dw.h"
#include "pmbrl_split.h"
#include "pmbrl_reg_head.h"

#include <utility>
#include <type_traits>
template <class F, int... I>
__device__ __forceinline__ void pr_for_dw_impl(F&& f, std::integer_sequence<int, I...>) { (f(std::integral_constant<int, I>{}), ...); }
template <int N, class F>
__device__ __forceinline__ void pr_for_dw(F&& f) { pr_for_dw_impl(static_cast<F&&>(f), std::make_integer_sequence<int, N>{}); }
typedef unsigned pr_u32x4_dw __attribute__((ext_vector_type(4)));
typedef unsigned long long pr_u64x2_dw __attribute__((ext_vector_type(2)));

struct PmTrue { static constexpr bool value = true; };
struct PmFalse { static constexpr bool value = false; };

struct DwRange {
  int c_lo, c_hi;
  bool add;
  bool zero;
};

__device__ __forceinline__ void pm_dw_ld(f32x4& d, unsigned voff, const float* sbase) {
#ifdef PM_EXP_DW_NOLOAD
  asm volatile("" : "=v"(d) : "v"(voff), "s"(sbase));
#else
  asm volatile("global_load_dwordx4 %0, %1, %2" : "=&v"(d) : "v"(voff), "s"(sbase));
#endif
}

__device__ __forceinline__ bool pm_dw_range(const DwArgs& A, int row, DwRange& r) {
  long long nv = 0x7fffffffll;
  if (A.nvalid) nv = max(0, __builtin_amdgcn_readfirstlane(*A.nvalid));
  const int n_chunks = A.nvalid ? (int)min((long long)A.n_chunks, nv * A.chunks_per_step) : A.n_chunks;
  r.add = r.zero = false;
  if (!A.pipe) {
    r.c_lo = row * A.chunks_per_split;
    r.c_hi = min(n_chunks, r.c_lo + A.chunks_per_split);
    return r.c_lo < r.c_hi;
  }
  const long long first_valid = max(nv, 1ll) * A.chunks_per_step;
  r.add = A.pipe_k > 0 && (long long)A.c_end < first_valid && row < A.rows_before;
  r.c_lo = A.c_begin + row * A.chunks_per_split;
  r.c_hi = min(min(A.c_end, n_chunks), r.c_lo + A.chunks_per_split);
  if (r.c_lo < r.c_hi) return true;
  r.zero = !r.add && (long long)A.c_begin < first_valid;
  return r.zero;
}
__device__ __forceinline__ void pm_dw_put(float* q, float v, bool add) { *q = add ? *q + v : v; }

template <int NI, int NJ>
__device__ __forceinline__ void pm_dw_block(const DwArgs& A, const DwBlock& blk, int c_lo, int c_hi,
                                            float* part, int lane, bool add) {
  const int g = lane >> 4, c16 = lane & 15;
  const int l = blk.layer;
  const int Fo16 = A.nt[l + 1] * 16, Fi16 = A.nt[l] * 16;
  const float* gbase = A.gT[l];
  const float* abase = A.actT[l];
  const size_t gblk = (size_t)Fo16 * A.Rw, ablk = (size_t)Fi16 * A.Rw;
  unsigned goff[NI], aoff[NJ];
#pragma unroll
  for (int i = 0; i < NI; ++i) {
    const int ot = blk.ot0 + (i < blk.n_ot ? i : blk.n_ot - 1);
    goff[i] = (unsigned)(((ot * 16 + c16) * A.Rw + 4 * g) * 4);
  }
#pragma unroll
  for (int j = 0; j < NJ; ++j) {
    const int it = blk.it0 + (j < blk.n_it ? j : blk.n_it - 1);
    aoff[j] = (unsigned)(((it * 16 + c16) * A.Rw + 4 * g) * 4);
  }

  f32x4 acc[NI][NJ];
  float bsum[NI];
#pragma unroll
  for (int i = 0; i < NI; ++i) {
    bsum[i] = 0.f;
#pragma unroll
    for (int j = 0; j < NJ; ++j) acc[i][j] = f32x4{0.f, 0.f, 0.f, 0.f};
  }
  const bool do_bias = blk.it0 == 0;
  f32x4 ga[2][NI], aa[2][NJ];
  auto load = [&](int buf, int c) {
    const int cc = c < c_hi ? c : c_hi - 1;
    const int b = cc / A.RT, rt = cc - b * A.RT;
    const float* gp = gbase + (size_t)b * gblk + rt * 16;
    const float* ap = abase + (size_t)b * ablk + rt * 16;
#pragma unroll
    for (int i = 0; i < NI; ++i) pm_dw_ld(ga[buf][i], goff[i], gp);
#pragma unroll
    for (int j = 0; j < NJ; ++j) pm_dw_ld(aa[buf][j], aoff[j], ap);
  };
  auto wait = [&](int buf) {
    asm volatile("s_waitcnt vmcnt(%0)" ::"n"(NI + NJ));
#pragma unroll
    for (int i = 0; i < NI; ++i) asm volatile("" : "+v"(ga[buf][i]));
#pragma unroll
    for (int j = 0; j < NJ; ++j) asm volatile("" : "+v"(aa[buf][j]));
  };
  auto compute = [&](int buf) {
#pragma unroll
    for (int kk = 0; kk < 4; ++kk)
#pragma unroll
      for (int i = 0; i < NI; ++i)
#pragma unroll
        for (int j = 0; j < NJ; ++j) {
#ifdef PM_EXP_DW_NOMFMA
          if (kk == 0) acc[i][j][0] += ga[buf][i][0] * aa[buf][j][0];
#else
          acc[i][j] = mfma4(ga[buf][i][kk], aa[buf][j][kk], acc[i][j]);
#endif
        }
    if (do_bias) {
#pragma unroll
      for (int i = 0; i < NI; ++i)
        bsum[i] += (ga[buf][i][0] + ga[buf][i][1]) + (ga[buf][i][2] + ga[buf][i][3]);
    }
  };
  load(0, c_lo);
  for (int c = c_lo; c < c_hi; c += 2) {
    load(1, c + 1);
    wait(0);
    compute(0);
    load(0, c + 2);
    wait(1);
    if (c + 1 < c_hi) compute(1);
  }
  asm volatile("s_waitcnt vmcnt(0)");
#pragma unroll
  for (int i = 0; i < NI; ++i) asm volatile("" : "+v"(ga[0][i]));
#pragma unroll
  for (int j = 0; j < NJ; ++j) asm volatile("" : "+v"(aa[0][j]));
  const int O = A.dim[l + 1], K = A.dim[l];
// ... 726 lines not shown
      ab_off[i] = (unsigned)((tr == PR_XT ? pr_xwave(0) : (tr & (PR_NW - 1))) * 64 + lane);
      ab_sh[i] = tr == PR_XT ? 4u * PR_SLOTS : 4u * (unsigned)(tr >> 2);
#pragma unroll
      for (int r = 0; r < 4; ++r) rbs[i][r] = 0.f;
    }
#pragma unroll
    for (int s = 0; s < 2; ++s) {
      const int j = 2 * g + s - A.rc_D;
      hok[s] = j >= 0 && j < A.rc_U;
      hoff_m[s] = (unsigned)((hok[s] ? j : 0) * 16 + c16);
      hoff_l[s] = (unsigned)((A.rc_U + (hok[s] ? j : 0)) * 16 + c16);
    }
  }
  __device__ __forceinline__ void fetch(const DwArgs& A, int l, int c, bool second) {
#pragma unroll
    for (int h = 0; h < 2; ++h) {
      const bool live = h == 0 || second;
      const float* hb = A.gT[l + 1] + (size_t)(c + h) * hblk;
      const unsigned* ap = A.rc_abits + (size_t)(c + h) * (PR_NW * 64);
#pragma unroll
      for (int s = 0; s < 2; ++s) {
        hgm[h][s] = (live && hok[s]) ? hb[hoff_m[s]] : 0.f;
        hgl[h][s] = (live && hok[s]) ? hb[hoff_l[s]] : 0.f;
      }
#pragma unroll
      for (int i = 0; i < 2; ++i) abw[h][i] = live ? ap[ab_off[i]] : 0u;
    }
  }
  __device__ __forceinline__ void stage(unsigned short* sa, float inv_keep, int lane) {
    const int g = lane >> 4, c16 = lane & 15;
    f32x4 bf[2][2], dl[2][2];
#pragma unroll
    for (int h = 0; h < 2; ++h) { PR_HEAD_BFRAGS(hgm[h], hgl[h], bf[h]) }
    pr_mfma_open();
#pragma unroll
    for (int h = 0; h < 2; ++h)
#pragma unroll
      for (int i = 0; i < 2; ++i) pr_mfma0<false, false, true>(dl[h][i], hw[i][0], bf[h][0]);
#pragma unroll
    for (int h = 0; h < 2; ++h)
#pragma unroll
      for (int i = 0; i < 2; ++i) pr_mfma<false, false, true>(dl[h][i], hw[i][1], bf[h][1]);
    asm volatile("s_nop 7\n\ts_nop 7" : "+v"(dl[0][0]), "+v"(dl[0][1]), "+v"(dl[1][0]), "+v"(dl[1][1]));
#pragma unroll
    for (int i = 0; i < 2; ++i)
      if (i == 0 || two) {
#pragma unroll
        for (int h = 0; h < 2; ++h) {
          f32x4 gq = dl[h][i] * pr_nibble_mult((abw[h][i] >> ab_sh[i]) & 15u, inv_keep);
          asm volatile("" : "+v"(gq));
#pragma unroll
          for (int r = 0; r < 4; ++r) rbs[i][r] += gq[r];
          pm_u32x2 pc[2];
          pm_split4<2, false>(gq, pc);
          unsigned short* q = sa + (row0 + 128 * i + 4 * g) * PM_DWW_LDK + 16 * h + c16;
#pragma unroll
          for (int pz = 0; pz < 2; ++pz, q += PM_DWL_F * PM_DWW_LDK) {
            q[0] = (unsigned short)(pc[pz][0] & 0xffffu);
            q[PM_DWW_LDK] = (unsigned short)(pc[pz][0] >> 16);
            q[2 * PM_DWW_LDK] = (unsigned short)(pc[pz][1] & 0xffffu);
            q[3 * PM_DWW_LDK] = (unsigned short)(pc[pz][1] >> 16);
          }
        }
      }
  }
  __device__ __forceinline__ void bias_out(float* pb, int O, int lane, bool add) {
    const int g = lane >> 4, c16 = lane & 15;
#pragma unroll
    for (int i = 0; i < 2; ++i)
      if (i == 0 || two) {
#pragma unroll
        for (int r = 0; r < 4; ++r) {
          float v = rbs[i][r];
          v += __shfl_xor(v, 1);
          v += __shfl_xor(v, 2);
          v += __shfl_xor(v, 4);
          v += __shfl_xor(v, 8);
          const int o = row0 + 128 * i + 4 * g + r;
          if (c16 == 0 && o < O) pm_dw_put(pb + o, v, add);
        }
      }
  }
};
template <bool RC>
__device__ __forceinline__ void pm_dw_layer_body(const DwArgs& A, int l) {
  extern __shared__ __attribute__((aligned(16))) unsigned short dww_lds[];
  const int tid = threadIdx.x, lane = tid & 63;
  const int wid = __builtin_amdgcn_readfirstlane(tid >> 6);
  const int row = blockIdx.x;
  DwRange R;
  if (!pm_dw_range(A, row, R)) return;
  const int Fo16 = A.nt[l + 1] * 16, Fi16 = A.nt[l] * 16;
  const int O = A.dim[l + 1], K = A.dim[l];
  float* part = A.part + (size_t)row * A.part_stride;
  const int g = lane >> 4, c16 = lane & 15;
  if (R.zero) {
    for (int e = tid; e < O * K; e += PM_DW_NT) part[A.w_off[l] + e] = 0.f;
    for (int e = tid; e < O; e += PM_DW_NT) part[A.b_off[l] + e] = 0.f;
    return;
  }
  const float* gbase = A.gT[l];
  const float* abase = A.actT[l];
  const size_t gblk = (size_t)Fo16 * A.Rw, ablk = (size_t)Fi16 * A.Rw;
  f32x4 rb[PM_DWL_Q];
  std::conditional_t<RC, PmDwNone, PmDwFetched> cl;
  std::conditional_t<RC, PmDwRc, PmDwNone> rc;
  if constexpr (RC) rc.init(A, l, wid, lane);
  else {
#pragma unroll
    for (int j = 0; j < PM_DWL_Q; ++j) cl.bs[j] = 0.f;
  }
  auto fetch1 = [&](f32x4& dst, const float* base, size_t blk, int F16, int idx, int c, bool second) {
    const int f = idx >> 3, kq = idx & 7;
    const float* p;
    bool live = f < F16;
    if (A.RT >= 2) {
      const int b = c / A.RT, rt = c - b * A.RT;
      p = base + (size_t)b * blk + (size_t)f * A.Rw + rt * 16 + kq * 4;
    } else {
      p = base + (size_t)(c + (kq >> 2)) * blk + (size_t)f * 16 + (kq & 3) * 4;
      live = live && (kq < 4 || second);
    }
    dst = live ? *reinterpret_cast<const f32x4*>(p) : f32x4{0.f, 0.f, 0.f, 0.f};
  };
  const bool pow2 = (A.RT & (A.RT - 1)) == 0;
  const int rt_sh = A.RT >= 4 ? 2 : (A.RT >= 2 ? 1 : 0);
  unsigned offB[PM_DWL_Q];
#pragma unroll
  for (int j = 0; j < PM_DWL_Q; ++j) {
    const int idx = tid + PM_DW_NT * j, f = idx >> 3, kq = idx & 7;
    const int fa = min(f, Fo16 - 1), fb = min(f, Fi16 - 1);
    if (A.RT >= 2) {
      if constexpr (!RC) cl.offA[j] = (unsigned)(fa * A.Rw + kq * 4);
      offB[j] = (unsigned)(fb * A.Rw + kq * 4);
    } else {
      if constexpr (!RC) cl.offA[j] = (unsigned)((kq >> 2) * (int)gblk + fa * 16 + (kq & 3) * 4);
      offB[j] = (unsigned)((kq >> 2) * (int)ablk + fb * 16 + (kq & 3) * 4);
    }
  }
  auto fetch = [&](int c) {
    const bool second = c + 1 < R.c_hi;
    if constexpr (RC) rc.fetch(A, l, c, second);
    if (second && pow2) {
      const int b = A.RT >= 2 ? c >> rt_sh : c, rt = A.RT >= 2 ? (c & (A.RT - 1)) : 0;
      const float* pg = gbase + (size_t)b * gblk + rt * 16;
      const float* pa = abase + (size_t)b * ablk + rt * 16;
      if constexpr (!RC) {
#pragma unroll
        for (int j = 0; j < PM_DWL_Q; ++j) cl.ra[j] = *reinterpret_cast<const f32x4*>(pg + cl.offA[j]);
      }
#pragma unroll
      for (int j = 0; j < PM_DWL_Q; ++j) rb[j] = *reinterpret_cast<const f32x4*>(pa + offB[j]);
      return;
    }
#pragma unroll
    for (int j = 0; j < PM_DWL_Q; ++j) {
      const int idx = tid + PM_DW_NT * j;
      if constexpr (!RC) fetch1(cl.ra[j], gbase, gblk, Fo16, idx, c, second);
      fetch1(rb[j], abase, ablk, Fi16, idx, c, second);
    }
  };
  auto put = [&](unsigned short* plane, int f, int kq, const f32x4& v) {
    const unsigned h0 = pm_pk_bf16(v[0], v[1]), h1 = pm_pk_bf16(v[2], v[3]);
    const unsigned l0 = pm_pk_bf16(v[0] - pm_bf_lo(h0), v[1] - pm_bf_hi(h0));
    const unsigned l1 = pm_pk_bf16(v[2] - pm_bf_lo(h1), v[3] - pm_bf_hi(h1));
    unsigned short* q = plane + f * PM_DWW_LDK + kq * 4;
    *reinterpret_cast<uint2*>(q) = uint2{h0, h1};
    *reinterpret_cast<uint2*>(q + PM_DWL_F * PM_DWW_LDK) = uint2{l0, l1};
  };
  auto stage = [&](int st) {
    unsigned short* sa = dww_lds + st * PM_DWL_STAGE;
    unsigned short* sb = sa + 2 * PM_DWL_F * PM_DWW_LDK;
#pragma unroll
    for (int j = 0; j < PM_DWL_Q; ++j) {
      const int idx = tid + PM_DW_NT * j;
      if (idx < PM_DWL_F * 8) {
        if constexpr (!RC) put(sa, idx >> 3, idx & 7, cl.ra[j]);
        put(sb, idx >> 3, idx & 7, rb[j]);
        if constexpr (!RC) cl.bs[j] += (cl.ra[j][0] + cl.ra[j][1]) + (cl.ra[j][2] + cl.ra[j][3]);
      }
    }
    if constexpr (RC) rc.stage(sa, A.rc_inv_keep, lane);
  };
  f32x4 acc[2][PM_DWL_NT];
#pragma unroll
  for (int i = 0; i < 2; ++i)
#pragma unroll
    for (int j = 0; j < PM_DWL_NT; ++j) acc[i][j] = f32x4{0.f, 0.f, 0.f, 0.f};
  const bool two = wid + 8 < PM_DWL_NT;
  auto mfmas = [&](int st) {
    const unsigned short* sa = dww_lds + st * PM_DWL_STAGE;
    const unsigned short* sb = sa + 2 * PM_DWL_F * PM_DWW_LDK;
    f32x4 ah[2], al[2];
#pragma unroll
    for (int i = 0; i < 2; ++i) {
      const int tr = (i == 0 || two) ? wid + 8 * i : wid;
      const unsigned short* q = sa + (tr * 16 + c16) * PM_DWW_LDK + g * 8;
      ah[i] = *reinterpret_cast<const f32x4*>(q);
      al[i] = *reinterpret_cast<const f32x4*>(q + PM_DWL_F * PM_DWW_LDK);
    }
#pragma unroll
    for (int j = 0; j < PM_DWL_NT; ++j) {
      const unsigned short* q = sb + (j * 16 + c16) * PM_DWW_LDK + g * 8;
      const f32x4 bh = *reinterpret_cast<const f32x4*>(q);
      const f32x4 bl = *reinterpret_cast<const f32x4*>(q + PM_DWL_F * PM_DWW_LDK);
      acc[0][j] = pm_mfma_bf<false>(al[0], bh, acc[0][j]);
      if (two) acc[1][j] = pm_mfma_bf<false>(al[1], bh, acc[1][j]);
      acc[0][j] = pm_mfma_bf<false>(ah[0], bl, acc[0][j]);
      if (two) acc[1][j] = pm_mfma_bf<false>(ah[1], bl, acc[1][j]);
      acc[0][j] = pm_mfma_bf<false>(ah[0], bh, acc[0][j]);
      if (two) acc[1][j] = pm_mfma_bf<false>(ah[1], bh, acc[1][j]);
    }
  };
  fetch(R.c_lo);
  stage(0);
  __syncthreads();
  int st = 0;
  for (int c = R.c_lo; c < R.c_hi; c += 2, st ^= 1) {
    const bool more = c + 2 < R.c_hi;
    if (more) fetch(c + 2);
    mfmas(st);
    if (more) stage(st ^ 1);
    __syncthreads();
  }
  {
    constexpr int LDE = PM_DWL_F + 4;
    float* ep = reinterpret_cast<float*>(dww_lds);
    float* wpart = part + A.w_off[l];
    const bool vec4 = (K & 3) == 0 && (A.w_off[l] & 3) == 0;
    __syncthreads();
#pragma unroll
    for (int half = 0; half < 2; ++half) {
      const int tr0 = 7 * half;
#pragma unroll
      for (int i = 0; i < 2; ++i) {
        const int tr = wid + 8 * i;
        if ((i == 0 || two) && (half == 0 ? tr < 7 : tr >= 7)) {
#pragma unroll
          for (int j = 0; j < PM_DWL_NT; ++j)
#pragma unroll
            for (int r = 0; r < 4; ++r) ep[((tr - tr0) * 16 + 4 * g + r) * LDE + j * 16 + c16] = acc[i][j][r];
        }
      }
      __syncthreads();
      const int o0 = tr0 * 16, nro = min(half == 0 ? 7 * 16 : 6 * 16, max(0, O - o0));
      if (vec4) {
        const int K4 = K >> 2;
        for (int e = tid; e < nro * K4; e += PM_DW_NT) {
          const int ro = e / K4, kq = e - ro * K4;
          const f32x4 v = *reinterpret_cast<const f32x4*>(ep + ro * LDE + 4 * kq);
          f32x4* q = reinterpret_cast<f32x4*>(wpart + (size_t)(o0 + ro) * K + 4 * kq);
          *q = R.add ? *q + v : v;
        }
      } else {
        for (int e = tid; e < nro * K; e += PM_DW_NT) {
          const int ro = e / K, k = e - ro * K;
          pm_dw_put(wpart + (size_t)(o0 + ro) * K + k, ep[ro * LDE + k], R.add);
        }
      }
      __syncthreads();
    }
  }
  if constexpr (RC) {
    rc.bias_out(part + A.b_off[l], O, lane, R.add);
  } else {
#pragma unroll
    for (int j = 0; j < PM_DWL_Q; ++j) {
      float v = cl.bs[j];
      v += __shfl_xor(v, 1);
      v += __shfl_xor(v, 2);
      v += __shfl_xor(v, 4);
      const int idx = tid + PM_DW_NT * j, o = idx >> 3;
      if ((idx & 7) == 0 && o < O) pm_dw_put(part + A.b_off[l] + o, v, R.add);
    }
  }
}
__global__ __launch_bounds__(PM_DW_NT, 2) void pm_dw_layer_kernel(const DwArgs A, int l) { pm_dw_layer_body<false>(A, l); }
__global__ __launch_bounds__(PM_DW_NT, 2) void pm_dw_layer_rc_kernel(const DwArgs A, int l) { pm_dw_layer_body<true>(A, l); }
```

prob_mbrl_amd/csrc/pmbrl_host.h:

```cpp
#pragma once
#include <hip/hip_runtime.h>

#include <string>
#include <vector>

#include "pmbrl.h"
#include "pmbrl_dev.h"
#include "pmbrl_dw.h"
#include "pmbrl_instances.h"

int pm_fail(int code, const std::string& msg);
static inline int fail(int code, const std::string& msg) { return pm_fail(code, msg); }
#define HIPCHK(expr)                                                               \
  do {                                                                             \
    hipError_t _e = (expr);                                                        \
    if (_e != hipSuccess)                                                          \
      return pm_fail(-100 - (int)_e, std::string(#expr) + ": " + hipGetErrorString(_e)); \
  } while (0)

struct NetPlan {
  int nl;
  int dim[PM_MAXL + 1], nt[PM_MAXL + 1];
  float keep[PM_MAXL];
  int act;
  size_t w_off[PM_MAXL], b_off[PM_MAXL];
  size_t n_params;
  size_t wf[PM_MAXL], wb[PM_MAXL], bias[PM_MAXL], abits[PM_MAXL];
};

struct PlanSwitches {
  bool mm_perstep, mm_mode2, mm_no_batch, dw_no_wide, reg_debug;
  bool lds_tiles, mm_xch, mm_tree, reg, reg_mm, reg_tree, reg_bwd, fuse_loss, ztab_merge, wide;
  bool mm_parts_set;
  int mm_parts;
  int replay;
  bool dw_pipe_off, dw_pipe_ranges;
  std::vector<int> dw_pipe;
};

#define PM_PIPE_MAX 8
struct pmbrl_plan {
  pmbrl_config cfg;
  PlanSwitches sw;
  int device;
  int RT, rows_per_wg, nwg, LD, mm_mode, G, M, fast, CA, CB;
  int prec, LDB;
  size_t lds_bytes;
  NetPlan pol, dyn;
  RewardDev* rew_d;
  int act;
  int learned;
  int rew_k = PMBRL_MAX_TIP;
  int* wflag_d;
  int wgen;
  int dw_split;
  AngleDev* ang_d;
  DwBlock* dw_blocks_d;
  DwUnit* dw_units_d;
  int n_dw_units;
  int dw_narrow[PM_MAXL];
  unsigned dw_pre_mask;
  int dw_layer13;
  int n_dw_blocks, dw_nsplit, dw_chunks_per_split, dw_n_chunks;
  DwArgs dw_args;
  int pipe_K, pipe_lo[PM_PIPE_MAX], pipe_rows, pipe_grid;
  hipStream_t pipe_stream;
  hipEvent_t pipe_ev[PM_PIPE_MAX];
  int dw_wave_first[PM_DW_NW + 1];
  size_t off_actT[PM_MAXL], off_gT[PM_MAXL], off_Tp, off_Td, off_xt, off_rt, off_part, off_mmfac,
      off_gxc, off_gxc2, off_gsync, off_xch, xch_bytes, off_grt, off_Jx, off_Ja, off_gmm_c, off_gmm_k, ws_bytes;
  int wlds_off, lds_last_lanes;
  const float* loss_w;
  float* loss_out;

  int mm_grid;
  int span;
  size_t off_mmx_buf, off_mmx_fac, off_mmx_rfac;
  int (*coll)(void* ctx, void* stream, double* buf_d, int64_t n);
  void* coll_ctx;
  int inplace;
  int mm_wide;
  int mm_parts;
  int xch_zeroed;
  mutable unsigned xch_gen;
  int mm_gpb;
  int mm_fan;
  size_t off_ztab;
  PmInst sweep[PF_VAR_COUNT];
  PmInstKey sweep_key[PF_VAR_COUNT];
  PmInst reg_k[2];
  int reg;
  mutable int reg_calls[2];
  int reg_mm;
  size_t off_reg_linv;
  size_t off_reg_pack;
  size_t off_reg_ab[2][2];
  int abits_packed;
  int old_pack_stale;
  int dw_g1_rebuilt;
  int replay;
  hipStream_t cap_stream;
  struct ReplaySlot { unsigned long long key; std::vector<unsigned char> bytes; int seen, dead, aux; hipGraphExec_t exec; long long launches; } rp[2];
  pmbrl_comm* grad_comm;
  pmbrl_p2p* grad_p2p;
  int tail_rank, tail_world;
  float* tail_buf_d;
  int* tail_err_d;
  mutable int tail_calls;
  long long* prof_fwd;
  long long* prof_bwd;
  int timing;
  hipEvent_t ev[PMBRL_TIMER_COUNT][2];
  bool ev_set[PMBRL_TIMER_COUNT];
};

enum class SweepForm {
  Barrier,
  StepInSweep,
  Whole,
  StepExternal
};
static inline SweepForm sweep_form(const pmbrl_plan* p) {
  if (p->mm_mode == 3) return p->mm_grid ? SweepForm::Barrier : SweepForm::StepInSweep;
  return p->mm_mode == 2 ? SweepForm::StepExternal : SweepForm::Whole;
}

static inline void replay_drop(pmbrl_plan* p, int slot) {
  if (p->rp[slot].exec) (void)hipGraphExecDestroy(p->rp[slot].exec);
  p->rp[slot].exec = nullptr;
  p->rp[slot].seen = 0;
}

struct ScopedTimer {
  pmbrl_plan* p; int slot; hipStream_t s;
  ScopedTimer(pmbrl_plan* p_, int slot_, hipStream_t s_) : p(p_), slot(slot_), s(s_) {
    if (p->timing) (void)hipEventRecord(p->ev[slot][0], s);
  }
  ~ScopedTimer() {
    if (p->timing) { (void)hipEventRecord(p->ev[slot][1], s); p->ev_set[slot] = true; }
  }
};

static inline std::string pm_inst_name(const PmInstKey& k) {
  std::string s;
  for (int v : {k.rt, k.ca, k.cb, k.var, k.d, k.u, k.ld, k.nl, k.nt, k.tree}) s += (s.empty() ? "(" : ", ") + std::to_string(v);
  return s + ") [row tiles, stage pair, variant, D, U, LD, layers, hidden tiles, tree]";
}

static inline int hidden_tiles_3l(const pmbrl_plan* p) {
  if (p->pol.nl != 3 || p->dyn.nl != 3) return -1;
  const int nt = p->pol.nt[1];
  return p->pol.nt[2] == nt && p->dyn.nt[1] == nt && p->dyn.nt[2] == nt ? nt : -1;
}
static inline int fast_variant(int RT, const RolloutArgs& A) {
  const bool mm = A.mm_mode == 1 || A.mm_mode == 3;
  const bool ext = A.prof || A.grad_states || A.grad_actions || A.agn || A.zpol_ss != 0 || A.zdyn_ss != 0 ||
                   (A.flags & PMBRL_FLAG_MM_STATES) || A.t0 != 0 || A.t1 != A.H || A.gx_from_carry;
  const bool mmg = RT == 1 && A.mm_mode == 3 && A.mm_grid;
  return mmg ? PF_VAR_MMG : mm ? PF_VAR_MM : (ext ? PF_VAR_EXT : PF_VAR_LEAN);
}

struct PackJob {
  const float* src;
  float* dst;
  int O, K, transpose, mult, is_bias;
  int planes;
  int f16;
};
struct PackArgs {
  int n;
  int* wflag;
  int gen;
  int* status;
  PackJob job[6 * PM_MAXL];
};
void pm_pack_all_launch(const PackArgs& PK, hipStream_t s);

int build_dw_blocks(int nl, const int* nt, std::vector<DwBlock>& blocks, int* wave_first, int tn_max = PM_DW_TN,
                    const bool* skip = nullptr);
int pm_dw_set_attr(const pmbrl_plan* p);
void pm_dw_launch(const pmbrl_plan* p, const DwArgs& W, hipStream_t s);
void pm_dw_launch_range(const pmbrl_plan* p, const DwArgs& W, int k, hipStream_t s);
void pm_dw_blocks_launch(const DwArgs& W, hipStream_t s);
#define PM_NORM_MAXB 8192
void pm_dw_reduce_launch(hipStream_t s, const float* part, int nsplit, int n, int stride, float* grad,
                         const int* nvalid = nullptr, int chunks_per_step = 0, int chunks_per_split = 1, int norm_on = 0,
                         const int* status = nullptr, int expect = 0, long long* step = nullptr, const float* loss_r = nullptr,
                         const float* loss_w = nullptr, long long loss_n = 0, long long loss_per_step = 0);
void launch_weighted_sum(hipStream_t s, const float* a, const float* w, long long n, float* out, const int* nvalid,
                         long long n_per_step);
int clip_adam_guarded_impl(void* stream, float* params_d, float* grads_d, float* exp_avg_d, float* exp_avg_sq_d, int64_t n,
                           int64_t* step_d, double lr, double beta1, double beta2, double eps, double max_norm,
                           float* norm_out_d, const int32_t* status_d, int32_t expect, bool norm_done,
                           float* loss_out_d = nullptr, int n_loss_part = 0);
void pm_tail_hvec_launch(hipStream_t s, float* hvec, int world, int rank, const int* status, int H);
void pm_tail_hmin_launch(hipStream_t s, const float* hvec, int world, int* status, int H);
void pm_tail_pack_launch(hipStream_t s, float* xb, int n, int n_loss_part, int loss_here, const int* status, const int* err);
void pm_tail_finish_launch(hipStream_t s, const float* xb, float* g, long long n, int* status, int expect, long long* step,
                           const int* err);
void pm_p2p_describe(const pmbrl_p2p* p, int* rank, int* nranks, size_t* cap_bytes, int** err_d);
bool pm_reg_plan_ok(const pmbrl_plan* p);
bool pm_reg_shape_ok(const pmbrl_plan* p, int prec1);
bool pm_reg_mm_shape_ok(const pmbrl_plan* p, int prec1);
int pm_reg_mm_width(const pmbrl_plan* p);
size_t pm_reg_pack_bytes();
int pm_reg_resolve(pmbrl_plan* p);
bool pm_reg_can_run(const pmbrl_plan* p, const RolloutArgs& A, bool fwd);
struct ZtabArgs;
void pm_reg_pack_launch(const pmbrl_plan* p, char* ws, const float* pol_params, const float* dyn_params, int* wflag, int gen,
                        hipStream_t s, int* status_reset, const ZtabArgs* ztab);
void pm_reg_unpack_abits(const pmbrl_plan* p, char* ws, hipStream_t s);
#define PM_REG_DW_LAYER 1
void pm_reg_dw_rebuild_args(const pmbrl_plan* p, char* ws, DwArgs& W);
void pm_reg_launch(const pmbrl_plan* p, char* ws, const RolloutArgs& A, const float* pol_params, const float* dyn_params,
                   hipStream_t s, bool fwd);
PmInstTable pm_fast_f32_instances();
PmInstTable pm_fast_split1_instances();
PmInstTable pm_fast_split2_instances();
PmInstTable pm_general_split_instances();
PmInstTable pm_general_act_instances();
```

prob_mbrl_amd/csrc/pmbrl_reg.h:

```cpp
#pragma once
#include <cstddef>
#include <type_traits>
#include <utility>
#include "pmbrl_dev.h"
#include "pmbrl_split.h"
#include "pmbrl_reg_head.h"
#include "pmbrl_reg_mm.h"

#define PR_NTHR (PR_NW * 64)
#define PR_NT 13
#define PR_KB 7
#define PM_GLOBAL_ __attribute__((address_space(1)))
typedef float f32x2 __attribute__((ext_vector_type(2)));

#define PR_RES_FLOATS (PR_NW * PR_SLOTS * PR_KB * 2 * PR_FRAG)
#define PR_XT_FLOATS (PR_KB * 2 * PR_FRAG)
#define PR_L0P_FLOATS (PR_NT * 2 * PR_FRAG)
#define PR_L0_FLOATS (PR_NT * PR_FRAG)
#define PR_HEAD_FLOATS (PR_NW * 2 * 2 * PR_FRAG)
#define PR_NET_FLOATS (PR_RES_FLOATS + PR_XT_FLOATS + PR_L0P_FLOATS + PR_HEAD_FLOATS)
#define PR_OFF_RES 0
#define PR_OFF_XT (PR_RES_FLOATS)
#define PR_OFF_L0 (PR_RES_FLOATS + PR_XT_FLOATS)
#define PR_OFF_HEAD (PR_RES_FLOATS + PR_XT_FLOATS + PR_L0P_FLOATS)
#define PR_PACK_FLOATS (4 * PR_NET_FLOATS)

#define PR_LDS_ACT 0
#define PR_LDS_PART (PR_LDS_ACT + PR_KB * 2 * PR_FRAG)
#define PR_LDS_L0(net) (PR_LDS_PART + PR_NW * PR_FRAG + (net) * (PR_L0_FLOATS + PR_XT_FLOATS + PR_HEAD_FLOATS))
#define PR_LDS_XT(net) (PR_LDS_L0(net) + PR_L0_FLOATS)
#define PR_LDS_HEAD(net) (PR_LDS_XT(net) + PR_XT_FLOATS)
#define PR_LDS_MF (PR_LDS_L0(2))
#define PR_LDS_MFX (PR_LDS_MF + PR_NW * 2 * 2 * PR_SLOTS * PR_FRAG)
#define PR_LDS_FLAG (PR_LDS_MFX + 2 * 2 * PR_FRAG)
#define PR_LDS_XB (PR_LDS_FLAG + 16)
#define PR_LDS_ZH (PR_LDS_XB + 128)
#define PR_LDS_REC (PR_LDS_ZH + 2 * PR_MM_ZH_DOUBLES(6))
#define PR_LDS_FLOATS (PR_LDS_REC + 2 * PR_MM_REC_DOUBLES)
static_assert(PR_LDS_FLOATS * 4 <= 160 * 1024, "forward sweep: LDS");

struct RegNet {
  int w_off[3], b_off[3];
  int n_in, n_out;
  const uint16_t* mask[2];
  unsigned abits[2];
  float inv_keep[2];
};

struct RegArgs {
  int B, H, D, U, nwg, hid;
  float mls_pol, mls_dyn;
  RegNet pol, dyn;
  const float* packed;
  const float *pol_params, *dyn_params;
  const float *x0, *mx, *iSx, *my, *Sy, *pscale, *pbias, *zpol, *zdyn;
  float *states, *actions;
  char* ws;
  unsigned Tp, Td;
  unsigned actT[3];
  unsigned gT[3];
  unsigned Jx, Ja;
  int* status;
  const int* wflag;
  int wgen;
  const float* grad_rewards;
  float* grad_x0;
  const int* nvalid;
  int t0, t1;
  const float* gx_in;
  float* gx_out;
  long long* prof;
  RegMM mm;
  int wg0;
};
typedef __attribute__((address_space(4))) const RegMM* pr_mm_kptr;
__device__ __forceinline__ pr_mm_kptr pr_mm_args() {
  typedef __attribute__((address_space(4))) const char* kcp;
  return (pr_mm_kptr)((kcp)__builtin_amdgcn_kernarg_segment_ptr() + offsetof(RegArgs, mm));
}
__device__ __forceinline__ RegMM pr_mm_load(pr_mm_kptr p) {
#if defined(__HIP_DEVICE_COMPILE__)
  return *p;
#else
  (void)p;
  return RegMM{};
#endif
}
__device__ __forceinline__ int pr_wg(const RegArgs& A) {
  const int hw = (int)blockIdx.x + A.wg0;
  if (!A.mm.on || !A.mm.xcd) return hw;
  if (A.mm.xcd == 2) {
    const int per = 2 * A.mm.fan, pw = (hw & 7) * per + (hw >> 3);
    return pw < A.mm.parts ? pw : -1;
  }
  const int P = A.mm.parts, blk = hw / (8 * P), r = hw - blk * (8 * P);
  const int gi = blk * 8 + (r & 7);
  return gi < A.mm.groups ? gi * P + (r >> 3) : -1;
}
__device__ __forceinline__ void pr_rows(const RegArgs& A, int wg, int& row0, int& nvalid) {
  if (A.mm.on) {
    const int gi = wg / A.mm.parts, me = wg - gi * A.mm.parts;
    row0 = gi * A.mm.M + me * A.mm.rpw;
    nvalid = min(A.mm.rpw, A.mm.M - me * A.mm.rpw);
  } else {
    row0 = wg * 16;
    nvalid = min(16, A.B - row0);
  }
}

template <int N, class F, int... I>
__device__ __forceinline__ void pr_for_impl(F&& f, std::integer_sequence<int, I...>) {
  (f(std::integral_constant<int, I>{}), ...);
}
template <int N, class F>
__device__ __forceinline__ void pr_for(F&& f) {
  pr_for_impl<N>(static_cast<F&&>(f), std::make_integer_sequence<int, N>{});
}

__host__ __device__ constexpr int pr_hid_feature(int kb, int g, int j) { return 16 * (2 * kb + (j >> 2)) + 4 * g + (j & 3); }

__host__ __device__ inline int pr_head_row(int net, int D, int U, int m) {
  const int i = 2 * (m >> 2) + ((m >> 1) & 1), kind = m & 1;
  if (net == 0) {
    const int j = i - D;
    return (j >= 0 && j < U) ? (kind ? U + j : j) : -1;
  }
  return i < D ? (kind ? D + i : i) : -1;
}

struct RegPackArgs {
  const float* par[2];
  int w_off[2][3], b_off[2][3];
  int n_in[2], n_out[2];
  int D, U, hid;
  float* out;
  int* wflag;
  int gen;
  int* status;
  int n_pack_blocks;
  ZtabArgs zt;
};

__device__ __forceinline__ unsigned short pr_f16_bits(float v) { return __builtin_bit_cast(unsigned short, (_Float16)v); }
__device__ __forceinline__ unsigned short pr_bf16_bits(float v) { return (unsigned short)(pm_pk_bf16(v, 0.f) & 0xffffu); }
__device__ __forceinline__ unsigned short pr_piece(float v, int p, bool f16) {
  if (f16) {
    const _Float16 h = (_Float16)v;
    return p == 0 ? __builtin_bit_cast(unsigned short, h) : pr_f16_bits((v - (float)h) * PM_F16_LO_SCALE);
  }
  const unsigned a = pm_pk_bf16(v, 0.f) & 0xffffu;
  return p == 0 ? (unsigned short)a : pr_bf16_bits(v - pm_bf_lo(a));
}

template <bool ZT>
__global__ __launch_bounds__(256) void pm_reg_pack_kernel(const RegPackArgs P) {
  if constexpr (ZT) {
// ... 1020 lines not shown
      asm volatile("" : "+v"(ln));
      pr_mm_kptr Qp = pr_mm_args();
      asm volatile("" : "+s"(Qp));
      const RegMM Q = pr_mm_load(Qp);
      if (PROF && wg == 0 && tid == 0) A.prof[(size_t)t * 32 + 6] = (long long)__builtin_readcyclecounter();
      if (wid == 1 && t > T0) {
        pr_mm_bwd_prep_noise<MMDc>(Q, t - 1, mm_gi, mm_g0, row0, nvalid, ln, mm_bop + ((t - 1) & 1) * PR_MM_BOP_DOUBLES);
        if (PROF && wg == 0 && lane == 0) A.prof[(size_t)t * 32 + 13] = (long long)__builtin_readcyclecounter();
      } else if (wid == 2 && t > T0) {
        pr_mm_bwd_prep_factor<MMDc>(Q, B, t - 1, mm_gi, row0, nvalid, ln, mm_yop + ((t - 1) & 1) * PR_MM_YOP_DOUBLES(MMDc));
        if (PROF && wg == 0 && lane == 0) A.prof[(size_t)t * 32 + 14] = (long long)__builtin_readcyclecounter();
      }
      if (do_chain) {
        double* const xh = reinterpret_cast<double*>(smem + PRB_LDS_XH);
        volatile unsigned* const xtag = reinterpret_cast<volatile unsigned*>(smem + PRB_LDS_XTAG);
        if constexpr (TREE) {
          if (wid != 0) {
            const bool okh = pm_xch_tree_help<PR_MM_NVX(MMDc), 4>(Q.xch, Q.nwg, mm_gi * Q.parts, Q.parts, Q.fan, mm_me, Q.tag0 + (unsigned)(T1 - t), wid, xh,
                                                    xtag, ln);
            if (!okh && lane == 0 && A.status) atomicMax(A.status, 1);
          }
        }
        if (wid == 0) {
          float go[(MMDc + 3) / 4];
          const bool ok = pr_mm_bwd_chain<MMDc, TREE>(Q, Q.tag0 + (unsigned)(T1 - t), mm_me, mm_gi * Q.parts, nvalid, ln, gx,
                                                 mm_bop + (t & 1) * PR_MM_BOP_DOUBLES, mm_yop + (t & 1) * PR_MM_YOP_DOUBLES(MMDc), go,
                                                 xh, xtag, (PROF && wg <= 1) ? A.prof + (size_t)t * 32 + 8 * wg : nullptr);
          if (!ok && lane == 0 && A.status) atomicMax(A.status, 1);
#pragma unroll
          for (int rr = 0; rr < (MMDc + 3) / 4; ++rr) smem[PRB_LDS_XB + row * 8 + g + 4 * rr] = go[rr];
        }
        pr_barrier();
        const f32x2 gm = *reinterpret_cast<const f32x2*>(smem + PRB_LDS_XB + row * 8 + 2 * g);
#pragma unroll
        for (int s = 0; s < 2; ++s) gx[s] = ok_x[s] ? gm[s] : 0.f;
        if (PROF && wg == 0 && tid == 0) A.prof[(size_t)t * 32 + 7] = (long long)__builtin_readcyclecounter();
      }
    }
    if (t > T0) {
#pragma unroll
      for (int k = 0; k < 2; ++k) sp[k] -= sstep[k];
      so_abp -= abp_step;
    }
    stage_load();
    ab_load(abn);
    float gxn[2], gm[2], gl[2];
#pragma unroll
    for (int s = 0; s < 2; ++s) {
      const float gg = gx[s] + In.gr * In.jx[s];
      gxn[s] = gg;
      gm[s] = gg * c_sy[s];
      gl[s] = gg * In.td[s];
    }
    head_adjoint(std::integral_constant<int, 1>{}, gm, gl, abc[0]);
    pr_barrier();
    if (PROF && wg == 0 && tid == 0) A.prof[(size_t)t * 32 + 1] = (long long)__builtin_readcyclecounter();
    f32x4 o;
    hidden_adjoint_and_tail(std::integral_constant<int, 1>{}, abc[1], 0, o, []() {});
    if (PROF && wg == 0 && tid == 0) A.prof[(size_t)t * 32 + 2] = (long long)__builtin_readcyclecounter();
    float pm_[2], pl_[2];
    {
      const f32x2 ja = *reinterpret_cast<const f32x2*>(st_row + 2 + 2 * g), tp = *reinterpret_cast<const f32x2*>(st_row + 10 + 2 * g),
                  ac = *reinterpret_cast<const f32x2*>(st_row + 18 + 2 * g);
#pragma unroll
      for (int s = 0; s < 2; ++s) {
        const float tail = o[2 * s] * c_isx[s];
        gxn[s] += ok_x[s] ? tail : 0.f;
        const float ga = In.gr * (ok_a[s] ? ja[s] : 0.f) + tail;
        const float th = ((ok_a[s] ? ac[s] : c_pbi[s]) - c_pbi[s]) * pr_rcp(c_psc[s]);
        const float gu = ok_a[s] ? ga * c_psc[s] * (1.f - th * th) : 0.f;
        pm_[s] = gu;
        pl_[s] = ok_a[s] ? gu * tp[s] : 0.f;
      }
    }
    if (wid == 2) {
#pragma unroll
      for (int s = 0; s < 2; ++s) {
        const int j = 2 * g + s - D;
        if (j >= 0 && j < U) {
          __builtin_amdgcn_raw_buffer_store_b32(__float_as_uint(pm_[s]), srd, (j * 16 + row) * 4, pr_uni(so_g2), 0);
          __builtin_amdgcn_raw_buffer_store_b32(__float_as_uint(pl_[s]), srd, ((U + j) * 16 + row) * 4, pr_uni(so_g2), 0);
        }
      }
    } else if (wid == 3) {
      for (int k = 2 * U * 16 + lane; k < 256; k += 64) __builtin_amdgcn_raw_buffer_store_b32(0u, srd, k * 4, pr_uni(so_g2), 0);
    }
    head_adjoint(std::integral_constant<int, 0>{}, pm_, pl_, abc[2]);
    pr_barrier();
    if (PROF && wg == 0 && tid == 0) A.prof[(size_t)t * 32 + 3] = (long long)__builtin_readcyclecounter();
    hidden_adjoint_and_tail(std::integral_constant<int, 0>{}, abc[3], so_g0, o, [&]() {
      stage_landed(std::integral_constant<int, 4>{}, sv);
      stage_park();
    });
    if (PROF && wg == 0 && tid == 0) A.prof[(size_t)t * 32 + 4] = (long long)__builtin_readcyclecounter();
#pragma unroll
    for (int s = 0; s < 2; ++s) gx[s] = ok_x[s] ? gxn[s] + o[2 * s] : 0.f;
    so_g0 -= st_step; so_g2 -= st_step2;
#ifdef PR_EXP_NOSTASH
    ab_landed(std::integral_constant<int, 0>{}, abn);
#else
    ab_landed(std::integral_constant<int, 12>{}, abn);
#endif
#pragma unroll
    for (int k = 0; k < 4; ++k) abc[k] = abn[k];
    if (PROF && wg == 0 && tid == 0) A.prof[(size_t)t * 32 + 5] = (long long)__builtin_readcyclecounter();
  }
  if (PROF && wg == 0 && tid == 0) {
    A.prof[31] = (long long)__builtin_readcyclecounter();
    A.prof[29] = (long long)__builtin_amdgcn_s_memrealtime();
  }
  if (wid == 0) {
#pragma unroll
    for (int s = 0; s < 2; ++s) {
      if (A.grad_x0 && T0 == 0 && ok_x[s]) *(gf32*)((PM_GLOBAL_ char*)A.grad_x0 + so_x[s]) = gx[s];
      if (A.gx_out && ok_x[s]) *(gf32*)((PM_GLOBAL_ char*)A.gx_out + so_x[s]) = gx[s];
    }
  }
}
```

prob_mbrl_amd/csrc/pmbrl_reg.hip:

```cpp
#include <algorithm>
#include <cstdio>
#include <cstdlib>
#include <cstring>
#include "pmbrl_host.h"
#include "pmbrl_reg.h"

bool pm_reg_shape_ok(const pmbrl_plan* p, int prec1) {
  const pmbrl_config& c = p->cfg;
  if (!p->sw.reg || !p->fast || prec1 != PMBRL_PREC_SPLIT_F16 || (c.flags & PMBRL_FLAG_NO_SHAPED)) return false;
  if (hidden_tiles_3l(p) != PR_NT) return false;
  const int hid = p->pol.dim[1];
  if (p->pol.dim[2] != hid || p->dyn.dim[1] != hid || p->dyn.dim[2] != hid) return false;
  if (c.D + c.U > 8 || p->pol.dim[0] != c.D || p->dyn.dim[0] != c.D + c.U) return false;
  if (p->pol.dim[3] != 2 * c.U || p->dyn.dim[3] != 2 * c.D) return false;
  return true;
}
bool pm_reg_mm_shape_ok(const pmbrl_plan* p, int prec1) {
  const pmbrl_config& c = p->cfg;
  if (!pm_reg_shape_ok(p, prec1)) return false;
  if (!(c.flags & PMBRL_FLAG_MM_STATES) || (c.flags & PMBRL_FLAG_INFER_NS) || c.D < 4 || c.D > 6) return false;
  if (!p->sw.mm_xch || !p->sw.reg_mm) return false;
  return true;
}

// ... 62 lines not shown
  R.states = A.states; R.actions = A.actions;
  R.ws = ws; R.Tp = (unsigned)p->off_Tp; R.Td = (unsigned)p->off_Td; R.Jx = (unsigned)p->off_Jx; R.Ja = (unsigned)p->off_Ja;
  for (int l = 0; l < 3; ++l) { R.actT[l] = (unsigned)p->off_actT[l]; R.gT[l] = (unsigned)p->off_gT[l]; }
  R.status = A.status;
  R.wflag = A.wflag; R.wgen = A.wgen;
  R.grad_rewards = A.grad_rewards; R.grad_x0 = A.grad_x0; R.nvalid = A.nvalid;
  R.t0 = A.t0; R.t1 = A.t1;
  R.gx_in = A.gx_from_carry ? A.gx_carry : nullptr;
  R.gx_out = (A.gx_carry && A.t0 > 0) ? A.gx_carry : nullptr;
  R.prof = A.prof;
  memset(&R.mm, 0, sizeof(R.mm));
  if (p->reg_mm) {
    R.mm.on = 1;
    R.mm.M = p->M; R.mm.parts = p->mm_parts; R.mm.rpw = p->rows_per_wg; R.mm.groups = p->G;
    R.mm.Bg = A.Bg; R.mm.row_off = A.row_off; R.mm.flags = A.flags;
    R.mm.zmm = A.zmm;
    R.mm.ztab = A.mm_ztab;
    R.mm.mmfac = A.mmfac;
    R.mm.linv = reinterpret_cast<double*>(ws + p->off_reg_linv);
    R.mm.xt = A.xt;
    R.mm.xt_off = (unsigned)p->off_xt;
    R.mm.xch = A.xch;
    R.mm.fan = p->mm_fan; R.mm.nwg = p->nwg;
    R.mm.xcd = p->mm_parts > 1 ? (p->mm_fan ? (pm_reg_tree_xcd(p) ? 2 : 0) : 1) : 0;
    R.mm.tag0 = (++p->xch_gen) << 12;
    R.mm.inv_m = 1.0 / (double)p->M;
    R.mm.inv_m1 = 1.0 / (double)(p->M - 1);
  }
}

bool pm_reg_can_run(const pmbrl_plan* p, const RolloutArgs& A, bool fwd) {
  if (!p->reg || (A.mm_mode != 0) != (p->reg_mm != 0)) return false;
  if (!fwd && !p->sw.reg_bwd) return false;
  if (!fwd && p->dw_layer13 != PM_REG_DW_LAYER) return false;
  const bool ext = A.grad_states || A.grad_actions || A.agn || A.zpol_ss != 0 || A.zdyn_ss != 0 ||
                   (((A.flags & PMBRL_FLAG_MM_STATES) != 0) != (p->reg_mm != 0)) || A.t0 != 0 || A.t1 != A.H || A.gx_from_carry;
  if (p->reg_mm && p->mm_parts > 1 && !A.xch) return false;
  return !ext;
}

void pm_reg_pack_launch(const pmbrl_plan* p, char* ws, const float* pol_params, const float* dyn_params, int* wflag, int gen,
                        hipStream_t s, int* status_reset, const ZtabArgs* ztab) {
  RegPackArgs P;
  memset(&P, 0, sizeof(P));
  P.par[0] = pol_params; P.par[1] = dyn_params;
  const NetPlan* nets[2] = {&p->pol, &p->dyn};
  for (int n = 0; n < 2; ++n) {
    for (int l = 0; l < 3; ++l) { P.w_off[n][l] = (int)nets[n]->w_off[l]; P.b_off[n][l] = (int)nets[n]->b_off[l]; }
    P.n_in[n] = nets[n]->dim[0];
    P.n_out[n] = nets[n]->dim[3];
  }
  P.D = p->cfg.D; P.U = p->cfg.U; P.hid = p->pol.dim[1];
  P.out = reinterpret_cast<float*>(ws + p->off_reg_pack);
  P.wflag = wflag; P.gen = gen;
  P.status = status_reset;
  const int total = 4 * (PR_NET_FLOATS / PR_FRAG) * 64;
  P.n_pack_blocks = (total + 255) / 256;
  if (ztab) P.zt = *ztab;
  if (P.zt.n_blocks > 0) hipLaunchKernelGGL(pm_reg_pack_kernel<true>, dim3(P.n_pack_blocks + P.zt.n_blocks), dim3(256), 0, s, P);
  else hipLaunchKernelGGL(pm_reg_pack_kernel<false>, dim3(P.n_pack_blocks), dim3(256), 0, s, P);
}

void pm_reg_unpack_abits(const pmbrl_plan* p, char* ws, hipStream_t s) {
  RegUnpackArgs U;
  U.B = p->cfg.B; U.H = p->cfg.H; U.nwg = p->nwg;
  U.mm_on = p->reg_mm ? 1 : 0; U.M = p->M; U.parts = p->mm_parts; U.rpw = p->rows_per_wg;
  const NetPlan* nets[2] = {&p->pol, &p->dyn};
  for (int n = 0; n < 2; ++n)
    for (int l = 0; l < 2; ++l) {
      U.src[n][l] = reinterpret_cast<const unsigned*>(ws + p->off_reg_ab[n][l]);
      U.dst[n][l] = reinterpret_cast<unsigned char*>(ws + nets[n]->abits[l]);
    }
  hipLaunchKernelGGL(pm_reg_unpack_abits_kernel, dim3(p->nwg, p->cfg.H), dim3(PR_NTHR), 0, s, U);
}

void pm_reg_dw_rebuild_args(const pmbrl_plan* p, char* ws, DwArgs& W) {
  W.rc_abits = reinterpret_cast<const unsigned*>(ws + p->off_reg_ab[0][1]);
  W.rc_head = reinterpret_cast<const float*>(ws + p->off_reg_pack) + (size_t)2 * PR_NET_FLOATS + PR_OFF_L0;
  W.rc_D = p->cfg.D;
  W.rc_U = p->cfg.U;
}

void pm_reg_launch(const pmbrl_plan* p, char* ws, const RolloutArgs& A, const float* pol_params, const float* dyn_params,
                   hipStream_t s, bool fwd) {
  ++p->reg_calls[fwd ? 0 : 1];
  RegArgs R;
  reg_args(p, ws, A, reinterpret_cast<const float*>(ws + p->off_reg_pack), pol_params, dyn_params, R);
  if (p->sw.reg_debug)
    fprintf(stderr, "pm_reg_launch %s: off_mmfac %zu off_reg_pack %zu gT %zu %zu %zu actT %zu %zu %zu abits %zu %zu %zu %zu ws_bytes %zu\n", fwd ? "fwd" : "bwd",
            p->off_mmfac, p->off_reg_pack, p->off_gT[0], p->off_gT[1], p->off_gT[2], p->off_actT[0], p->off_actT[1], p->off_actT[2],
            p->off_reg_ab[0][0], p->off_reg_ab[0][1], p->off_reg_ab[1][0], p->off_reg_ab[1][1], p->ws_bytes);
  const int total = R.mm.xcd == 2 ? 8 * 2 * p->mm_fan : R.mm.xcd ? (p->G + 7) / 8 * 8 * p->mm_parts : p->nwg;
  int per = (p->reg_mm && p->mm_gpb > 0) ? p->mm_gpb * p->mm_parts : total;
  if (R.mm.xcd == 1 && per < total) per = (p->mm_gpb + 7) / 8 * 8 * p->mm_parts;
  const PmInst& K = p->reg_k[R.prof ? 1 : 0];
  for (int w0 = 0; w0 < total; w0 += per) {
    R.wg0 = w0;
    void* args[] = {&R};
    (void)hipLaunchKernel(fwd ? K.fwd : K.bwd, dim3(std::min(per, total - w0)), dim3(PR_NTHR), args,
                          (fwd ? PR_LDS_FLOATS : PRB_LDS_FLOATS) * sizeof(float), s);
  }
}
```

prob_mbrl_amd/engine.py:

```python
import ctypes as C
import math

import numpy as np
import torch

from . import _lib

LOG_MAX_STD = math.log(5.0)

_PRECISIONS = {'f32': _lib.PREC_F32, 'split': _lib.PREC_SPLIT, 'split_f16': _lib.PREC_SPLIT_F16}
_default_precision = [None]


def set_precision(name):
    assert name in _PRECISIONS, name
    _default_precision[0] = name


def get_precision():
    import os
    return _default_precision[0] or os.environ.get('PMBRL_PRECISION', 'split_f16')


def safe_precision(name):
# ... 539 lines not shown
        s = int(self.status[0].item())
        return self.H if s >= self.H else s

    def sweep_failed(self):
        return int(self.status[1].item()) != 0

    def set_loss(self, weights, out=None):
        if weights is None:
            _lib.check(self.lib.pmbrl_plan_set_loss(self.plan, None, None), 'pmbrl_plan_set_loss')
            self._loss = None
            return None
        w = _f32c(weights.reshape(self.H, self.B), self.device)
        out = out if out is not None else torch.zeros(1, dtype=torch.float32, device=self.device)
        _lib.check(self.lib.pmbrl_plan_set_loss(self.plan, _ptr(w), _ptr(out)), 'pmbrl_plan_set_loss')
        self._loss = (w, out)
        return out

    def backward(self, grad_rewards, grad_states=None, grad_actions=None, want_x0=False,
                 want_agn=False, adam=None):
        assert self._inputs is not None, 'forward() first'
        dev = self.device
        gr = _f32c(grad_rewards.reshape(self.H, self.B), dev)
        gs = _f32c(grad_states, dev) if grad_states is not None else None
        ga = _f32c(grad_actions, dev) if grad_actions is not None else None
        if gs is not None:
            assert gs.shape == (self.H + 1, self.B, self.D)
        if ga is not None:
            assert ga.shape == (self.H, self.B, self.U)
        gx0 = torch.empty((self.B, self.D), dtype=torch.float32, device=dev) if want_x0 else None
        agn = torch.empty((self.H, self.B), dtype=torch.float32, device=dev) if want_agn else None
        S, A, R = self._traj
        if adam is not None:
            for k in ('params', 'exp_avg', 'exp_avg_sq'):
                t = adam[k]
                assert t.is_cuda and t.dtype == torch.float32 and t.is_contiguous() and t.numel() == self.n_pol_params
            assert adam['step'].is_cuda and adam['step'].dtype == torch.int64
            o = _lib.Adam(adam['params'].data_ptr(), adam['exp_avg'].data_ptr(), adam['exp_avg_sq'].data_ptr(),
                          adam['step'].data_ptr(), float(adam['lr']), float(adam['betas'][0]), float(adam['betas'][1]),
                          float(adam['eps']), float(adam.get('max_norm') or 0.0),
                          adam['norm_out'].data_ptr() if adam.get('norm_out') is not None else None,
                          int(adam.get('expect') or 0),
                          adam['loss_out'].data_ptr() if adam.get('loss_out') is not None else None)
            if adam.get('loss_out') is not None:
                lo = adam['loss_out']
                assert lo.is_cuda and lo.dtype == torch.float32 and lo.numel() >= 1
            _lib.check(self.lib.pmbrl_rollout_bwd_adam(self.plan, _stream(), self._ws_ptr,
                                                       C.byref(self._inputs), _ptr(S), _ptr(A), _ptr(R), _ptr(gr),
                                                       _ptr(gs), _ptr(ga), _ptr(self.grad_flat), _ptr(gx0),
                                                       _ptr(agn), _ptr(self.status), C.byref(o)),
                       'pmbrl_rollout_bwd_adam')
            return self.grad_flat, gx0, agn
        _lib.check(self.lib.pmbrl_rollout_bwd(self.plan, _stream(), self._ws_ptr,
                                              C.byref(self._inputs), _ptr(S), _ptr(A), _ptr(R), _ptr(gr),
                                              _ptr(gs), _ptr(ga), _ptr(self.grad_flat), _ptr(gx0),
                                              _ptr(agn), _ptr(self.status)),
                   'pmbrl_rollout_bwd')
        return self.grad_flat, gx0, agn

    def set_replay(self, on=1):
        _lib.check(self.lib.pmbrl_plan_set_replay(self.plan, int(on)), 'set_replay')
        info = (C.c_int32 * _lib.INFO_COUNT)()
        _lib.check(self.lib.pmbrl_plan_info(self.plan, info), 'plan_info')
        self.info['replay'] = int(info[_lib.INFO_REPLAY])

    def reg_calls(self):
        info = (C.c_int32 * _lib.INFO_COUNT)()
        _lib.check(self.lib.pmbrl_plan_info(self.plan, info), 'plan_info')
        return int(info[_lib.INFO_REG_FWD_CALLS]), int(info[_lib.INFO_REG_BWD_CALLS])

    def sweep_kernels(self):
        out = {}
        for v, key in enumerate(_lib.SWEEP_VARIANTS):
            if key in ('ext', 'mm', 'mmg') and not self.info['fast']:
                continue
            names = []
            for adjoint in (0, 1):
                name = C.c_char_p()
                _lib.check(self.lib.pmbrl_plan_sweep_kernel(self.plan, v, adjoint, C.byref(name)), 'plan_sweep_kernel')
                names.append((name.value or b'').decode())
            if names[0]:
                out[key] = tuple(names)
        return out

    def replay_count(self):
        n = (C.c_int64 * 2)()
        _lib.check(self.lib.pmbrl_plan_replay_count(self.plan, n), 'replay_count')
        return int(n[0]), int(n[1])

    def set_timing(self, on=True):
        _lib.check(self.lib.pmbrl_plan_set_timing(self.plan, 1 if on else 0), 'set_timing')

    def read_timing(self):
        ms = (C.c_float * _lib.TIMER_COUNT)()
        _lib.check(self.lib.pmbrl_plan_read_timing(self.plan, ms), 'read_timing')
        return {n: float(ms[i]) for i, n in enumerate(_lib.TIMER_NAMES)}

    def weighted_sum(self, a, w, out=None):
        a = _f32c(a.reshape(-1), self.device)
        w = _f32c(w.reshape(-1), self.device)
        assert a.numel() == self.H * self.B and w.numel() == a.numel()
        if out is None:
            out = torch.empty(1, dtype=torch.float32, device=self.device)
        _lib.check(self.lib.pmbrl_weighted_sum_steps(_stream(), _ptr(a), _ptr(w), self.B, self.H,
                                                     _ptr(self.status), _ptr(out)),
                   'pmbrl_weighted_sum_steps')
        return out


def clip_adam(params, grads, exp_avg, exp_avg_sq, step, lr, betas=(0.9, 0.999), eps=1e-8,
              max_norm=None, norm_out=None):
    lib = _lib.load()
    for t in (params, grads, exp_avg, exp_avg_sq):
        assert t.is_cuda and t.dtype == torch.float32 and t.is_contiguous()
    n = params.numel()
    _lib.check(lib.pmbrl_clip_adam(_stream(), _ptr(params), _ptr(grads), _ptr(exp_avg),
                                   _ptr(exp_avg_sq), n, int(step), float(lr), float(betas[0]),
                                   float(betas[1]), float(eps),
                                   float(max_norm) if max_norm else 0.0, _ptr(norm_out)),
               'pmbrl_clip_adam')


class Graph:

    def __init__(self, fn, warmup=1):
        self.lib = _lib.load()
        self.handle = C.c_void_p()
        side = torch.cuda.Stream()
        side.wait_stream(torch.cuda.current_stream())
        with torch.cuda.stream(side):
            for _ in range(warmup):
                fn()
            side.synchronize()
            _lib.check(self.lib.pmbrl_graph_capture_begin(C.c_void_p(side.cuda_stream)), 'pmbrl_graph_capture_begin')
            try:
                fn()
            finally:
                rc = self.lib.pmbrl_graph_capture_end(C.c_void_p(side.cuda_stream), C.byref(self.handle))
            _lib.check(rc, 'pmbrl_graph_capture_end')
        torch.cuda.current_stream().wait_stream(side)
        self._keep = fn

    def replay(self):
        _lib.check(self.lib.pmbrl_graph_launch(self.handle, _stream()), 'pmbrl_graph_launch')

    def num_nodes(self):
        n = C.c_int64(0)
        _lib.check(self.lib.pmbrl_graph_num_nodes(self.handle, C.byref(n)), 'pmbrl_graph_num_nodes')
        return int(n.value)

    def __del__(self):
        try:
            if self.handle:
                self.lib.pmbrl_graph_destroy(self.handle)
                self.handle = C.c_void_p()
        except Exception:
            pass


def clip_adam_guarded(params, grads, exp_avg, exp_avg_sq, step_dev, lr, status, expect, betas=(0.9, 0.999),
                      eps=1e-8, max_norm=None, norm_out=None):
    lib = _lib.load()
    for t in (params, grads, exp_avg, exp_avg_sq):
        assert t.is_cuda and t.dtype == torch.float32 and t.is_contiguous()
    assert step_dev.is_cuda and step_dev.dtype == torch.int64 and status.is_cuda and status.dtype == torch.int32
    _lib.check(lib.pmbrl_clip_adam_guarded(_stream(), _ptr(params), _ptr(grads), _ptr(exp_avg),
                                           _ptr(exp_avg_sq), params.numel(), _ptr(step_dev), float(lr),
# ... 17 lines not shown
```

Baseline: 5.822 million.

## Stream layer weight-gradient computation concurrently with the register backward sweep

The register-resident backward kernel now publishes tagged per-step layer gradients to a workspace buffer. A weight-gradient kernel on a side stream, using CUs left idle by the backward sweep, consumes late timesteps as they appear by spinning on those tags. The remaining early steps are handled afterwards by a bounded-range variant of the existing dW kernel. This overlaps part of the dW reduction with the serial adjoint sweep. The cost is extra atomic stores, a memset of the publish buffer, spin-wait polling with a timeout failure path, and more workspace memory.

Result: faster. 6.193 million, median of 6 (+6.4%).

```diff
diff --git a/include/pmbrl.h b/include/pmbrl.h
--- a/include/pmbrl.h
+++ b/include/pmbrl.h
@@ -124,6 +124,7 @@
 int pmbrl_plan_info(const pmbrl_plan* plan, int32_t* info );
 #define PMBRL_SWEEP_REG 4
 int pmbrl_plan_sweep_kernel(const pmbrl_plan* plan, int variant, int adjoint, const char** name);
+int pmbrl_plan_dw_stream(const pmbrl_plan* plan, int32_t* out );
 
 int pmbrl_pack_mask(void* stream, const float* mask_d, int32_t B, int32_t h,
                     int32_t src_ld, uint16_t* bits_d);
diff --git a/prob_mbrl_amd/_lib.py b/prob_mbrl_amd/_lib.py
--- a/prob_mbrl_amd/_lib.py
+++ b/prob_mbrl_amd/_lib.py
@@ -87,7 +87,7 @@
 EXPORTS = [
     'pmbrl_last_error', 'pmbrl_version', 'pmbrl_build_id', 'pmbrl_plan_create',
     'pmbrl_graph_capture_begin', 'pmbrl_graph_capture_end', 'pmbrl_graph_launch', 'pmbrl_graph_num_nodes', 'pmbrl_graph_destroy',
-    'pmbrl_plan_destroy', 'pmbrl_plan_workspace_bytes', 'pmbrl_plan_info', 'pmbrl_plan_sweep_kernel',
+    'pmbrl_plan_destroy', 'pmbrl_plan_workspace_bytes', 'pmbrl_plan_info', 'pmbrl_plan_sweep_kernel', 'pmbrl_plan_dw_stream',
     'pmbrl_pack_mask', 'pmbrl_draw_masks', 'pmbrl_rollout_fwd', 'pmbrl_rollout_bwd', 'pmbrl_rollout_bwd_adam',
     'pmbrl_plan_set_loss',
     'pmbrl_weighted_sum', 'pmbrl_weighted_sum_steps', 'pmbrl_clip_adam', 'pmbrl_clip_adam_guarded', 'pmbrl_debug_linear',
@@ -147,6 +147,9 @@
     lib.pmbrl_plan_info.argtypes = [vp, C.POINTER(i32)]
     lib.pmbrl_plan_sweep_kernel.restype = C.c_int
     lib.pmbrl_plan_sweep_kernel.argtypes = [vp, C.c_int, C.c_int, C.POINTER(C.c_char_p)]
+    if hasattr(lib, 'pmbrl_plan_dw_stream'):
+        lib.pmbrl_plan_dw_stream.restype = C.c_int
+        lib.pmbrl_plan_dw_stream.argtypes = [vp, C.POINTER(i32)]
     lib.pmbrl_pack_mask.restype = C.c_int
     lib.pmbrl_pack_mask.argtypes = [vp, vp, i32, i32, i32, vp]
     lib.pmbrl_rollout_fwd.restype = C.c_int
diff --git a/prob_mbrl_amd/csrc/pmbrl.hip b/prob_mbrl_amd/csrc/pmbrl.hip
--- a/prob_mbrl_amd/csrc/pmbrl.hip
+++ b/prob_mbrl_amd/csrc/pmbrl.hip
@@ -371,6 +371,14 @@
       if (*q == ',') ++q;
     }
   }
+  if (const char* e = getenv("PMBRL_DW_STREAM")) {
+    s.dw_stream_off = !strcmp(e, "off");
+    s.dw_stream_set = e[0] >= '0' && e[0] <= '9';
+    if (s.dw_stream_set) {
+      s.dw_stream_steps = atoi(e);
+      if (const char* q = strchr(e, ',')) s.dw_stream_wgs = std::max(0, atoi(q + 1));
+    }
+  }
   return s;
 }
 
@@ -856,10 +864,37 @@
   return 0;
 }
 
-static int plan_workspace(pmbrl_plan* p) {
+static int plan_dw_stream(pmbrl_plan* p, int cus) {
+  const pmbrl_config& c = p->cfg;
+  const PlanSwitches& sw = p->sw;
+  p->st_on = 0;
+  const int n_free = cus >= 64 && cus % 8 == 0 ? 8 * (cus / 8 - (p->nwg + 7) / 8) : 0;
+  const bool fam = p->reg && !p->reg_mm && sw.reg_bwd && p->dw_layer13 == PM_REG_DW_LAYER && p->RT == 1;
+  const bool single = sweep_form(p) == SweepForm::Whole && p->mm_parts <= 1 && p->pipe_K <= 1;
+  if (!fam || !single || n_free < 1 || n_free < cus / 8 || sw.dw_stream_off || c.H >= 4095) return 0;
+  const bool large = p->nwg >= n_free && (long long)c.H * p->nwg >= 14ll * cus;
+  if (!large && !sw.dw_stream_set) return 0;
+  int steps = p->nwg <= 2 * n_free ? c.H : (int)((long long)c.H * 2 * n_free / p->nwg);
+  int wgs = n_free;
+  if (sw.dw_stream_set) {
+    steps = sw.dw_stream_steps;
+    if (sw.dw_stream_wgs > 0) wgs = std::min(wgs, sw.dw_stream_wgs);
+  }
+  steps = std::max(0, std::min(c.H, steps));
+  p->st_on = 1;
+  p->st_cut = c.H - steps;
+  p->st_wgs = wgs;
+  if (!p->pipe_stream) HIPCHK(hipStreamCreateWithFlags(&p->pipe_stream, hipStreamNonBlocking));
+  for (int k = 0; k < 2; ++k)
+    if (!p->pipe_ev[k]) HIPCHK(hipEventCreateWithFlags(&p->pipe_ev[k], hipEventDisableTiming));
+  return 0;
+}
+
+static int plan_workspace(pmbrl_plan* p, int cus) {
   const pmbrl_config& c = p->cfg;
   p->reg = pm_reg_plan_ok(p) ? 1 : 0;
   p->reg_mm = pm_reg_mm_width(p);
+  if (int rc = plan_dw_stream(p, cus)) return rc;
   size_t off = 0;
   auto take = [&](size_t bytes) {
     const size_t o = off;
@@ -912,8 +947,10 @@
     for (int l = 0; l < 2; ++l) p->off_reg_ab[n][l] = take(p->reg ? (size_t)c.H * p->nwg * 1024 : 0);
   p->off_part = take((size_t)std::max(p->dw_nsplit, p->pipe_K > 1 ? p->pipe_rows : 0) *
                      ((p->pol.n_params + 3) / 4 * 4) * sizeof(float));
+  p->pub_bytes = p->st_on ? (size_t)c.H * p->nwg * 2 * c.U * 16 * sizeof(unsigned long long) : 0;
+  p->off_pub = take(p->pub_bytes);
   p->ws_bytes = off;
-  if (p->ws_bytes >= ((size_t)1 << 32)) p->reg = p->reg_mm = 0;
+  if (p->ws_bytes >= ((size_t)1 << 32)) p->reg = p->reg_mm = p->st_on = 0;
   return 0;
 }
 
@@ -1019,7 +1056,7 @@
   if (int rc = plan_angles(p.get())) return rc;
   if (int rc = plan_dw(p.get())) return rc;
   if (int rc = plan_dw_pipe(p.get(), cus)) return rc;
-  if (int rc = plan_workspace(p.get())) return rc;
+  if (int rc = plan_workspace(p.get(), cus)) return rc;
   if (int rc = plan_attrs(p.get(), cus)) return rc;
   *out = p.release();
   return 0;
@@ -1065,7 +1102,7 @@
     HIPCHK(hipGraphLaunch(R.exec, s));
     ++R.launches;
     if (slot == 0) { p->old_pack_stale = R.aux & 1; p->abits_packed = (R.aux >> 1) & 1; }
-    else p->dw_g1_rebuilt = (R.aux >> 2) & 1;
+    else { p->dw_g1_rebuilt = (R.aux >> 2) & 1; p->dw_streamed = (R.aux >> 3) & 1; }
     return 0;
   }
   if (!same || R.seen == 0) {
@@ -1101,7 +1138,7 @@
     return body(s);
   }
   R.exec = ex;
-  R.aux = (p->old_pack_stale & 1) | ((p->abits_packed & 1) << 1) | ((p->dw_g1_rebuilt & 1) << 2);
+  R.aux = (p->old_pack_stale & 1) | ((p->abits_packed & 1) << 1) | ((p->dw_g1_rebuilt & 1) << 2) | ((p->dw_streamed & 1) << 3);
   HIPCHK(hipGraphLaunch(R.exec, s));
   ++R.launches;
   return 0;
@@ -1165,7 +1202,8 @@
   if (p->tail_buf_d) (void)hipFree(p->tail_buf_d);
   if (p->pipe_stream) {
     (void)hipStreamDestroy(p->pipe_stream);
-    for (int k = 0; k < p->pipe_K; ++k) (void)hipEventDestroy(p->pipe_ev[k]);
+    for (int k = 0; k < PM_PIPE_MAX; ++k)
+      if (p->pipe_ev[k]) (void)hipEventDestroy(p->pipe_ev[k]);
   }
   delete p;
 }
@@ -1184,6 +1222,13 @@
 }
 
 extern "C" size_t pmbrl_plan_workspace_bytes(const pmbrl_plan* p) { return p ? p->ws_bytes : 0; }
+
+extern "C" int pmbrl_plan_dw_stream(const pmbrl_plan* p, int32_t* out) {
+  if (!p || !out) return fail(-1, "null argument");
+  out[0] = p->st_on ? p->cfg.H - p->st_cut : -1;
+  out[1] = p->st_on ? p->st_wgs : 0;
+  return 0;
+}
 
 extern "C" int pmbrl_plan_info(const pmbrl_plan* p, int32_t* info) {
   if (!p || !info) return fail(-1, "null argument");
@@ -1731,8 +1776,16 @@
   return 0;
 }
 
-static DwArgs dw_call_args(const pmbrl_plan* p, const BwdCall& C, const RolloutArgs& A) {
+static DwArgs dw_call_args(const pmbrl_plan* p, const BwdCall& C, const RolloutArgs& A, bool streamed) {
   DwArgs W = p->dw_args;
+  if (streamed) {
+    W.st_on = 1;
+    W.st_cut = p->st_cut;
+    W.st_wgs = p->st_wgs;
+    W.st_pub = reinterpret_cast<const unsigned long long*>(static_cast<char*>(C.workspace) + p->off_pub);
+    W.st_tag = ((++p->pub_gen) << 12) + 1u;
+    W.st_fail = C.status ? C.status + 1 : nullptr;
+  }
   for (int l = 0; l < p->pol.nl; ++l) { W.actT[l] = A.actT[l]; W.gT[l] = A.gT[l]; }
   W.part = reinterpret_cast<float*>(static_cast<char*>(C.workspace) + p->off_part);
   W.nvalid = C.status;
@@ -1769,6 +1822,14 @@
 static int bwd_sweep_whole(pmbrl_plan* p, const BwdCall& C, RolloutArgs A, const DwArgs& W, bool reg_bwd, int K, const int* lo) {
   hipStream_t s = C.stream;
   char* ws = static_cast<char*>(C.workspace);
+  if (W.st_on) {
+    const bool rec = pm_stream_recording(s);
+    if (p->pub_ws != C.workspace || rec) {
+      HIPCHK(hipMemsetAsync(ws + p->off_pub, 0, p->pub_bytes, s));
+      p->pub_ws = rec ? nullptr : C.workspace;
+    }
+    HIPCHK(hipEventRecord(p->pipe_ev[0], s));
+  }
   if (p->mm_parts > 1) {
     A.gsync += 1024;
     A.gx_carry_out = reinterpret_cast<float*>(ws + p->off_gxc2);
@@ -1778,8 +1839,13 @@
     A.t0 = lo[k];
     A.t1 = k ? lo[k - 1] : p->cfg.H;
     A.gx_from_carry = k > 0;
-    if (reg_bwd) pm_reg_launch(p, ws, A, C.in->pol_params_d, C.in->dyn_params_d, s, false);
+    if (reg_bwd) pm_reg_launch(p, ws, A, C.in->pol_params_d, C.in->dyn_params_d, s, false, W.st_on ? (unsigned)p->off_pub : 0u, W.st_tag);
     else launch_bwd_rt(p, A, s);
+    if (W.st_on) {
+      HIPCHK(hipStreamWaitEvent(p->pipe_stream, p->pipe_ev[0], 0));
+      pm_dw_stream_launch(p, W, p->pipe_stream);
+      HIPCHK(hipEventRecord(p->pipe_ev[1], p->pipe_stream));
+    }
     if (k + 1 < K) {
       HIPCHK(hipEventRecord(p->pipe_ev[k], s));
       HIPCHK(hipStreamWaitEvent(p->pipe_stream, p->pipe_ev[k], 0));
@@ -1814,7 +1880,7 @@
 static int bwd_dw(pmbrl_plan* p, const BwdCall& C, const DwArgs& W, bool piped) {
   ScopedTimer tm(p, PMBRL_TIMER_DW, C.stream);
   if (!piped) {
-    pm_dw_launch(p, W, C.stream);
+    pm_dw_launch(p, W, C.stream, W.st_on ? p->pipe_ev[1] : nullptr);
     return 0;
   }
   HIPCHK(hipEventRecord(p->pipe_ev[p->pipe_K - 1], p->pipe_stream));
@@ -1823,6 +1889,9 @@
   return 0;
 }
 
+static bool bwd_streamed(const pmbrl_plan* p, const BwdCall& C, bool reg_bwd) {
+  return p->st_on && reg_bwd && sweep_form(p) == SweepForm::Whole && p->pipe_K <= 1 && !p->prof_bwd && !bwd_tail(p, C);
+}
 static int rollout_bwd(pmbrl_plan* p, const BwdCall& C, const RolloutArgs& A0, bool reg_bwd) {
   hipStream_t s = C.stream;
   RolloutArgs A = A0;
@@ -1836,9 +1905,11 @@
   if (p->reg && !reg_bwd) bwd_convert_family(p, C);
   float* grt = reinterpret_cast<float*>(static_cast<char*>(C.workspace) + p->off_grt);
   if (int rc = bwd_reward_adjoint(p, C, A, grt)) return rc;
-  const DwArgs W = dw_call_args(p, C, A);
   const SweepForm form = sweep_form(p);
   const bool piped = form == SweepForm::Whole && p->pipe_K > 1 && !p->prof_bwd;
+  const bool streamed = bwd_streamed(p, C, reg_bwd);
+  p->dw_streamed = streamed ? 1 : 0;
+  const DwArgs W = dw_call_args(p, C, A, streamed);
   {
     ScopedTimer tm(p, PMBRL_TIMER_BWD, s);
     static const int whole[1] = {0};
@@ -1906,6 +1977,8 @@
   K.val(p->old_pack_stale); K.val(p->abits_packed);
   const int g1_rebuilt = reg_bwd ? 1 : 0;
   K.val(g1_rebuilt);
+  const int streamed = bwd_streamed(p, C, reg_bwd) ? 1 : 0;
+  K.val(streamed);
   return K;
 }
 
diff --git a/prob_mbrl_amd/csrc/pmbrl_dw.h b/prob_mbrl_amd/csrc/pmbrl_dw.h
--- a/prob_mbrl_amd/csrc/pmbrl_dw.h
+++ b/prob_mbrl_amd/csrc/pmbrl_dw.h
@@ -42,6 +42,11 @@
   const float* rc_head;
   float rc_inv_keep;
   int rc_D, rc_U;
+  int st_on;
+  int st_cut, st_wgs;
+  const unsigned long long* st_pub;
+  unsigned st_tag;
+  int* st_fail;
 };
 
 #define PM_DWP_TM 256
diff --git a/prob_mbrl_amd/csrc/pmbrl_dw.hip b/prob_mbrl_amd/csrc/pmbrl_dw.hip
--- a/prob_mbrl_amd/csrc/pmbrl_dw.hip
+++ b/prob_mbrl_amd/csrc/pmbrl_dw.hip
@@ -70,6 +70,10 @@
                                hipFuncAttributeMaxDynamicSharedMemorySize, PM_DWL_LDS_BYTES));
     HIPCHK(hipFuncSetAttribute(reinterpret_cast<const void*>(&pm_dw_layer_rc_kernel),
                                hipFuncAttributeMaxDynamicSharedMemorySize, PM_DWL_LDS_BYTES));
+    HIPCHK(hipFuncSetAttribute(reinterpret_cast<const void*>(&pm_dw_layer_st_kernel),
+                               hipFuncAttributeMaxDynamicSharedMemorySize, PM_DWL_LDS_BYTES));
+    HIPCHK(hipFuncSetAttribute(reinterpret_cast<const void*>(&pm_dw_layer_rcb_kernel),
+                               hipFuncAttributeMaxDynamicSharedMemorySize, PM_DWL_LDS_BYTES));
   }
   if (p->dw_pre_mask) {
     HIPCHK(hipFuncSetAttribute(reinterpret_cast<const void*>(&pm_dw_narrow_pre_kernel<1>),
@@ -100,7 +104,7 @@
   if (p->dw_split) Wk.chunks_per_split = (Wk.chunks_per_split + 1) & ~1;
   return Wk;
 }
-void pm_dw_launch(const pmbrl_plan* p, const DwArgs& W, hipStream_t s) {
+void pm_dw_launch(const pmbrl_plan* p, const DwArgs& W, hipStream_t s, hipEvent_t after) {
   const dim3 rows(W.nsplit), units((W.nsplit + 7) / 8 * 8 * p->n_dw_units);
   if (p->n_dw_blocks == 0) {}
   else if (p->dw_split) hipLaunchKernelGGL(pm_dw_kernel_s, rows, dim3(PM_DW_NT), 0, s, W);
@@ -118,12 +122,21 @@
     hipLaunchKernelGGL(pm_dw_wide_kernel, units, dim3(PM_DW_NT), PM_DWW_LDS_BYTES, s, W, p->dw_units_d, p->n_dw_units);
   const bool rebuild = W.rc_abits != nullptr;
   assert(!rebuild || (W.RT == 1 && p->dw_layer13 == PM_REG_DW_LAYER));
-  if (p->dw_layer13 >= 0 && rebuild)
+  assert(!W.st_on || rebuild);
+  if (after) (void)hipStreamWaitEvent(s, after, 0);
+  if (W.st_on && W.st_cut == 0) return;
+  if (p->dw_layer13 >= 0 && rebuild && W.st_on)
+    hipLaunchKernelGGL(pm_dw_layer_rcb_kernel, rows, dim3(PM_DW_NT), PM_DWL_LDS_BYTES, s, W, p->dw_layer13);
+  else if (p->dw_layer13 >= 0 && rebuild)
     hipLaunchKernelGGL(pm_dw_layer_rc_kernel, rows, dim3(PM_DW_NT), PM_DWL_LDS_BYTES, s, W, p->dw_layer13);
   else if (p->dw_layer13 >= 0)
     hipLaunchKernelGGL(pm_dw_layer_kernel, rows, dim3(PM_DW_NT), PM_DWL_LDS_BYTES, s, W, p->dw_layer13);
 }
 void pm_dw_launch_range(const pmbrl_plan* p, const DwArgs& W, int k, hipStream_t s) { pm_dw_launch(p, dw_range_args(p, W, k), s); }
+void pm_dw_stream_launch(const pmbrl_plan* p, const DwArgs& W, hipStream_t s) {
+  assert(W.st_on && W.rc_abits && W.RT == 1 && p->dw_layer13 == PM_REG_DW_LAYER);
+  hipLaunchKernelGGL(pm_dw_layer_st_kernel, dim3(W.st_wgs), dim3(PM_DW_NT), PM_DWL_LDS_BYTES, s, W, p->dw_layer13);
+}
 void pm_dw_blocks_launch(const DwArgs& W, hipStream_t s) {
   hipLaunchKernelGGL(pm_dw_kernel, dim3(W.nsplit), dim3(PM_DW_NT), 0, s, W);
 }
diff --git a/prob_mbrl_amd/csrc/pmbrl_dw_kernels.h b/prob_mbrl_amd/csrc/pmbrl_dw_kernels.h
--- a/prob_mbrl_amd/csrc/pmbrl_dw_kernels.h
+++ b/prob_mbrl_amd/csrc/pmbrl_dw_kernels.h
@@ -48,6 +48,37 @@
   return r.zero;
 }
 __device__ __forceinline__ void pm_dw_put(float* q, float v, bool add) { *q = add ? *q + v : v; }
+
+struct DwStream {
+  int steps;
+  int rows;
+  int nc;
+  bool any;
+};
+__device__ __forceinline__ DwStream pm_dw_stream(const DwArgs& A) {
+  long long nv = 0x7fffffffll;
+  if (A.nvalid) nv = max(0, __builtin_amdgcn_readfirstlane(*A.nvalid));
+  const long long n_chunks = min((long long)A.n_chunks, nv * A.chunks_per_step);
+  DwStream S;
+  S.steps = (int)(n_chunks / A.chunks_per_step);
+  S.rows = (int)((n_chunks + A.chunks_per_split - 1) / A.chunks_per_split);
+  S.nc = min(A.st_wgs, S.rows);
+  S.any = A.st_cut < S.steps;
+  return S;
+}
+__device__ __forceinline__ bool pm_dw_range_st(const DwArgs& A, int row, DwRange& r) {
+  const DwStream S = pm_dw_stream(A);
+  r.add = r.zero = false;
+  if (row >= S.rows) return false;
+  const int c_end = min(A.st_cut, S.steps) * A.chunks_per_step;
+  const int per = ((c_end + S.rows - 1) / S.rows + 1) & ~1;
+  r.add = S.any && row < S.nc;
+  r.c_lo = row * per;
+  r.c_hi = min(c_end, r.c_lo + per);
+  if (r.c_lo < r.c_hi) return true;
+  r.zero = !r.add;
+  return r.zero;
+}
 
 template <int NI, int NJ>
 __device__ __forceinline__ void pm_dw_block(const DwArgs& A, const DwBlock& blk, int c_lo, int c_hi,
@@ -940,14 +971,106 @@
       }
   }
 };
-template <bool RC>
+typedef __attribute__((address_space(1))) const unsigned long long pm_dw_gu64;
+struct PmDwRcSt : PmDwRc {
+  unsigned long long gr[2][2][2];
+  const unsigned long long* gp;
+  unsigned want;
+  int gblk;
+  bool gsecond, dead;
+
+  __device__ __forceinline__ void init_st(const DwArgs& A) {
+    gblk = 2 * A.rc_U * 16;
+    dead = false;
+  }
+  __device__ __forceinline__ void load() {
+#pragma unroll
+    for (int h = 0; h < 2; ++h) {
+      pm_dw_gu64* q = (pm_dw_gu64*)gp + ((h == 1 && gsecond) ? gblk : 0);
+#pragma unroll
+      for (int s = 0; s < 2; ++s) {
+        gr[h][s][0] = __hip_atomic_load(q + hoff_m[s], __ATOMIC_RELAXED, __HIP_MEMORY_SCOPE_AGENT);
+        gr[h][s][1] = __hip_atomic_load(q + hoff_l[s], __ATOMIC_RELAXED, __HIP_MEMORY_SCOPE_AGENT);
+      }
+    }
+  }
+  __device__ __forceinline__ void fetch_st(const DwArgs& A, int c, bool second, int t) {
+    gp = A.st_pub + (size_t)c * gblk;
+    want = A.st_tag + (unsigned)t;
+    gsecond = second;
+    load();
+#pragma unroll
+    for (int h = 0; h < 2; ++h) {
+      const unsigned* ap = A.rc_abits + (size_t)(c + h) * (PR_NW * 64);
+#pragma unroll
+      for (int i = 0; i < 2; ++i) abw[h][i] = (h == 0 || second) ? ap[ab_off[i]] : 0u;
+    }
+  }
+  __device__ __forceinline__ void settle(const DwArgs& A, int lane) {
+    for (int spins = 0;;) {
+      bool here = true;
+#pragma unroll
+      for (int h = 0; h < 2; ++h)
+#pragma unroll
+        for (int s = 0; s < 2; ++s) {
+          const bool live = (h == 0 || gsecond) && hok[s];
+          here = here && (!live || ((unsigned)(gr[h][s][0] >> 32) == want && (unsigned)(gr[h][s][1] >> 32) == want));
+        }
+      if (__all(here) || dead) break;
+      for (;;) {
+        if (++spins > (1 << 19)) {
+          dead = true;
+          if (lane == 0 && A.st_fail) atomicMax(A.st_fail, 1);
+          break;
+        }
+        __builtin_amdgcn_s_sleep(32);
+        const unsigned long long g1 = __hip_atomic_load((pm_dw_gu64*)gp, __ATOMIC_RELAXED, __HIP_MEMORY_SCOPE_AGENT);
+        if ((unsigned)(g1 >> 32) == want) break;
+      }
+      if (dead) break;
+      load();
+    }
+#pragma unroll
+    for (int h = 0; h < 2; ++h)
+#pragma unroll
+      for (int s = 0; s < 2; ++s) {
+        const bool live = (h == 0 || gsecond) && hok[s];
+        hgm[h][s] = live ? __uint_as_float((unsigned)gr[h][s][0]) : 0.f;
+        hgl[h][s] = live ? __uint_as_float((unsigned)gr[h][s][1]) : 0.f;
+      }
+  }
+};
+template <bool RC, int ST = 0>
 __device__ __forceinline__ void pm_dw_layer_body(const DwArgs& A, int l) {
+  static_assert(RC || ST == 0, "the streamed form rebuilds its operand");
   extern __shared__ __attribute__((aligned(16))) unsigned short dww_lds[];
   const int tid = threadIdx.x, lane = tid & 63;
   const int wid = __builtin_amdgcn_readfirstlane(tid >> 6);
   const int row = blockIdx.x;
   DwRange R;
-  if (!pm_dw_range(A, row, R)) return;
+  int st_steps = 0, k_lo = 0, k_hi = 0;
+  if constexpr (ST == 1) {
+    const DwStream S = pm_dw_stream(A);
+    if (!S.any || row >= S.nc) return;
+    st_steps = S.steps;
+    k_lo = (int)((long long)row * A.chunks_per_step / S.nc);
+    k_hi = (int)((long long)(row + 1) * A.chunks_per_step / S.nc);
+    R.add = false;
+    R.zero = k_lo >= k_hi;
+    R.c_lo = R.c_hi = 0;
+    if (A.st_cut == 0) {
+      const int O_ = A.dim[l + 1], K_ = A.dim[l];
+      for (int r = S.nc + row; r < S.rows; r += S.nc) {
+        float* pz = A.part + (size_t)r * A.part_stride;
+        for (int e = tid; e < O_ * K_; e += PM_DW_NT) pz[A.w_off[l] + e] = 0.f;
+        for (int e = tid; e < O_; e += PM_DW_NT) pz[A.b_off[l] + e] = 0.f;
+      }
+    }
+  } else if constexpr (ST == 2) {
+    if (!pm_dw_range_st(A, row, R)) return;
+  } else {
+    if (!pm_dw_range(A, row, R)) return;
+  }
   const int Fo16 = A.nt[l + 1] * 16, Fi16 = A.nt[l] * 16;
   const int O = A.dim[l + 1], K = A.dim[l];
   float* part = A.part + (size_t)row * A.part_stride;
@@ -962,7 +1085,8 @@
   const size_t gblk = (size_t)Fo16 * A.Rw, ablk = (size_t)Fi16 * A.Rw;
   f32x4 rb[PM_DWL_Q];
   std::conditional_t<RC, PmDwNone, PmDwFetched> cl;
-  std::conditional_t<RC, PmDwRc, PmDwNone> rc;
+  std::conditional_t<RC, std::conditional_t<ST == 1, PmDwRcSt, PmDwRc>, PmDwNone> rc;
+  if constexpr (ST == 1) rc.init_st(A);
   if constexpr (RC) rc.init(A, l, wid, lane);
   else {
 #pragma unroll
@@ -996,9 +1120,9 @@
       offB[j] = (unsigned)((kq >> 2) * (int)ablk + fb * 16 + (kq & 3) * 4);
     }
   }
-  auto fetch = [&](int c) {
-    const bool second = c + 1 < R.c_hi;
-    if constexpr (RC) rc.fetch(A, l, c, second);
+  auto fetch = [&](int c, bool second, int t) {
+    if constexpr (ST == 1) rc.fetch_st(A, c, second, t);
+    else if constexpr (RC) rc.fetch(A, l, c, second);
     if (second && pow2) {
       const int b = A.RT >= 2 ? c >> rt_sh : c, rt = A.RT >= 2 ? (c & (A.RT - 1)) : 0;
       const float* pg = gbase + (size_t)b * gblk + rt * 16;
@@ -1038,6 +1162,7 @@
         if constexpr (!RC) cl.bs[j] += (cl.ra[j][0] + cl.ra[j][1]) + (cl.ra[j][2] + cl.ra[j][3]);
       }
     }
+    if constexpr (ST == 1) rc.settle(A, lane);
     if constexpr (RC) rc.stage(sa, A.rc_inv_keep, lane);
   };
   f32x4 acc[2][PM_DWL_NT];
@@ -1070,16 +1195,34 @@
       if (two) acc[1][j] = pm_mfma_bf<false>(ah[1], bh, acc[1][j]);
     }
   };
-  fetch(R.c_lo);
-  stage(0);
-  __syncthreads();
-  int st = 0;
-  for (int c = R.c_lo; c < R.c_hi; c += 2, st ^= 1) {
-    const bool more = c + 2 < R.c_hi;
-    if (more) fetch(c + 2);
-    mfmas(st);
-    if (more) stage(st ^ 1);
+  if constexpr (ST == 1) {
+    int t = st_steps - 1, k = k_lo;
+    fetch(t * A.chunks_per_step + k, k + 1 < k_hi, t);
+    stage(0);
     __syncthreads();
+    for (int st = 0;; st ^= 1) {
+      int tn = t, kn = k + 2;
+      if (kn >= k_hi) { kn = k_lo; tn = t - 1; }
+      const bool more = tn >= A.st_cut;
+      if (more) fetch(tn * A.chunks_per_step + kn, kn + 1 < k_hi, tn);
+      mfmas(st);
+      if (more) stage(st ^ 1);
+      __syncthreads();
+      if (!more) break;
+      t = tn; k = kn;
+    }
+  } else {
+    fetch(R.c_lo, R.c_lo + 1 < R.c_hi, 0);
+    stage(0);
+    __syncthreads();
+    int st = 0;
+    for (int c = R.c_lo; c < R.c_hi; c += 2, st ^= 1) {
+      const bool more = c + 2 < R.c_hi;
+      if (more) fetch(c + 2, c + 3 < R.c_hi, 0);
+      mfmas(st);
+      if (more) stage(st ^ 1);
+      __syncthreads();
+    }
   }
   {
     constexpr int LDE = PM_DWL_F + 4;
@@ -1135,3 +1278,5 @@
 }
 __global__ __launch_bounds__(PM_DW_NT, 2) void pm_dw_layer_kernel(const DwArgs A, int l) { pm_dw_layer_body<false>(A, l); }
 __global__ __launch_bounds__(PM_DW_NT, 2) void pm_dw_layer_rc_kernel(const DwArgs A, int l) { pm_dw_layer_body<true>(A, l); }
+__global__ __launch_bounds__(PM_DW_NT, 2) void pm_dw_layer_st_kernel(const DwArgs A, int l) { pm_dw_layer_body<true, 1>(A, l); }
+__global__ __launch_bounds__(PM_DW_NT, 2) void pm_dw_layer_rcb_kernel(const DwArgs A, int l) { pm_dw_layer_body<true, 2>(A, l); }
diff --git a/prob_mbrl_amd/csrc/pmbrl_host.h b/prob_mbrl_amd/csrc/pmbrl_host.h
--- a/prob_mbrl_amd/csrc/pmbrl_host.h
+++ b/prob_mbrl_amd/csrc/pmbrl_host.h
@@ -36,6 +36,8 @@
   int replay;
   bool dw_pipe_off, dw_pipe_ranges;
   std::vector<int> dw_pipe;
+  bool dw_stream_off, dw_stream_set;
+  int dw_stream_steps, dw_stream_wgs;
 };
 
 #define PM_PIPE_MAX 8
@@ -66,6 +68,11 @@
   int pipe_K, pipe_lo[PM_PIPE_MAX], pipe_rows, pipe_grid;
   hipStream_t pipe_stream;
   hipEvent_t pipe_ev[PM_PIPE_MAX];
+  int st_on, st_cut, st_wgs;
+  size_t off_pub, pub_bytes;
+  const void* pub_ws;
+  mutable unsigned pub_gen;
+  int dw_streamed;
   int dw_wave_first[PM_DW_NW + 1];
   size_t off_actT[PM_MAXL], off_gT[PM_MAXL], off_Tp, off_Td, off_xt, off_rt, off_part, off_mmfac,
       off_gxc, off_gxc2, off_gsync, off_xch, xch_bytes, off_grt, off_Jx, off_Ja, off_gmm_c, off_gmm_k, ws_bytes;
@@ -179,7 +186,8 @@
 int build_dw_blocks(int nl, const int* nt, std::vector<DwBlock>& blocks, int* wave_first, int tn_max = PM_DW_TN,
                     const bool* skip = nullptr);
 int pm_dw_set_attr(const pmbrl_plan* p);
-void pm_dw_launch(const pmbrl_plan* p, const DwArgs& W, hipStream_t s);
+void pm_dw_launch(const pmbrl_plan* p, const DwArgs& W, hipStream_t s, hipEvent_t after = nullptr);
+void pm_dw_stream_launch(const pmbrl_plan* p, const DwArgs& W, hipStream_t s);
 void pm_dw_launch_range(const pmbrl_plan* p, const DwArgs& W, int k, hipStream_t s);
 void pm_dw_blocks_launch(const DwArgs& W, hipStream_t s);
 #define PM_NORM_MAXB 8192
@@ -213,7 +221,7 @@
 #define PM_REG_DW_LAYER 1
 void pm_reg_dw_rebuild_args(const pmbrl_plan* p, char* ws, DwArgs& W);
 void pm_reg_launch(const pmbrl_plan* p, char* ws, const RolloutArgs& A, const float* pol_params, const float* dyn_params,
-                   hipStream_t s, bool fwd);
+                   hipStream_t s, bool fwd, unsigned pub = 0, unsigned pub_tag = 0);
 PmInstTable pm_fast_f32_instances();
 PmInstTable pm_fast_split1_instances();
 PmInstTable pm_fast_split2_instances();
diff --git a/prob_mbrl_amd/csrc/pmbrl_reg.h b/prob_mbrl_amd/csrc/pmbrl_reg.h
--- a/prob_mbrl_amd/csrc/pmbrl_reg.h
+++ b/prob_mbrl_amd/csrc/pmbrl_reg.h
@@ -72,6 +72,7 @@
   long long* prof;
   RegMM mm;
   int wg0;
+  unsigned pub, pub_tag;
 };
 typedef __attribute__((address_space(4))) const RegMM* pr_mm_kptr;
 __device__ __forceinline__ pr_mm_kptr pr_mm_args() {
@@ -1258,6 +1259,21 @@
           __builtin_amdgcn_raw_buffer_store_b32(__float_as_uint(pl_[s]), srd, ((U + j) * 16 + row) * 4, pr_uni(so_g2), 0);
         }
       }
+      if constexpr (MMD == 0 && !TREE) {
+        if (A.pub) {
+          typedef PM_GLOBAL_ unsigned long long gu64;
+          const unsigned long long tg = (unsigned long long)(A.pub_tag + (unsigned)t) << 32;
+          gu64* const pb = (gu64*)((PM_GLOBAL_ char*)A.ws + A.pub) + (size_t)(t * A.nwg + wg) * (size_t)(2 * U * 16);
+#pragma unroll
+          for (int s = 0; s < 2; ++s) {
+            const int j = 2 * g + s - D;
+            if (j >= 0 && j < U) {
+              __hip_atomic_store(pb + j * 16 + row, tg | __float_as_uint(pm_[s]), __ATOMIC_RELAXED, __HIP_MEMORY_SCOPE_AGENT);
+              __hip_atomic_store(pb + (U + j) * 16 + row, tg | __float_as_uint(pl_[s]), __ATOMIC_RELAXED, __HIP_MEMORY_SCOPE_AGENT);
+            }
+          }
+        }
+      }
     } else if (wid == 3) {
       for (int k = 2 * U * 16 + lane; k < 256; k += 64) __builtin_amdgcn_raw_buffer_store_b32(0u, srd, k * 4, pr_uni(so_g2), 0);
     }
diff --git a/prob_mbrl_amd/csrc/pmbrl_reg.hip b/prob_mbrl_amd/csrc/pmbrl_reg.hip
--- a/prob_mbrl_amd/csrc/pmbrl_reg.hip
+++ b/prob_mbrl_amd/csrc/pmbrl_reg.hip
@@ -168,10 +168,11 @@
 }
 
 void pm_reg_launch(const pmbrl_plan* p, char* ws, const RolloutArgs& A, const float* pol_params, const float* dyn_params,
-                   hipStream_t s, bool fwd) {
+                   hipStream_t s, bool fwd, unsigned pub, unsigned pub_tag) {
   ++p->reg_calls[fwd ? 0 : 1];
   RegArgs R;
   reg_args(p, ws, A, reinterpret_cast<const float*>(ws + p->off_reg_pack), pol_params, dyn_params, R);
+  if (!fwd && !p->reg_mm) { R.pub = pub; R.pub_tag = pub_tag; }
   if (p->sw.reg_debug)
     fprintf(stderr, "pm_reg_launch %s: off_mmfac %zu off_reg_pack %zu gT %zu %zu %zu actT %zu %zu %zu abits %zu %zu %zu %zu ws_bytes %zu\n", fwd ? "fwd" : "bwd",
             p->off_mmfac, p->off_reg_pack, p->off_gT[0], p->off_gT[1], p->off_gT[2], p->off_actT[0], p->off_actT[1], p->off_actT[2],
diff --git a/prob_mbrl_amd/engine.py b/prob_mbrl_amd/engine.py
--- a/prob_mbrl_amd/engine.py
+++ b/prob_mbrl_amd/engine.py
@@ -645,6 +645,13 @@
                 out[key] = tuple(names)
         return out
 
+    def dw_stream(self):
+        if not hasattr(self.lib, 'pmbrl_plan_dw_stream'):
+            return None
+        out = (C.c_int32 * 2)()
+        _lib.check(self.lib.pmbrl_plan_dw_stream(self.plan, out), 'plan_dw_stream')
+        return None if out[0] < 0 else (int(out[0]), int(out[1]))
+
     def replay_count(self):
         n = (C.c_int64 * 2)()
         _lib.check(self.lib.pmbrl_plan_replay_count(self.plan, n), 'replay_count')
```
